# timweiland/GaussianMarkovRandomFields.jl

Hardware: AMD Instinct MI355X
Metric: factor+solve(64 RHS) throughput (higher is better)
Workload: dtype f64; 1 GPU; cfg2: 1000x1000-node jittered P1 mesh, 2-D Matern nu=1 (alpha=2), refactorize + 64-RHS solve + logdet per step, inputs resident in HBM; n=1000000, nnz_Q=18960020, nnz_L=178441686, nnz_L_stored=193749782, nrhs=64, parallelism=1 GPU, ordering=own geometric nested dissection

## Files before the change

### gaussianmarkovrandomfields.jl_amd/csrc/device.cpp

```cpp
#include "device.h"

#include <algorithm>
#include <atomic>
#include <chrono>
#include <cstdio>
#include <climits>
#include <cstdlib>
#include <cstring>
#include <exception>
#include <functional>
#include <stdexcept>
#include <thread>
#include <type_traits>

#include "kernels.h"

namespace gmrfx {

void hip_check(hipError_t e, const char *what) {
    if (e != hipSuccess) throw std::runtime_error(std::string("HIP error in ") + what + ": " + hipGetErrorString(e));
}
#define HC(x) hip_check((x), #x)

static constexpr size_t kPairSlackBytes = 16;
static constexpr size_t kChunkSlack = 16 * 320;
template <class T> T *Device::dalloc(size_t count) {
    void *p = nullptr;
    const size_t bytes = std::max<size_t>(count, 1) * sizeof(T) + kPairSlackBytes;
    HC(hipMalloc(&p, bytes));
    allocs_.push_back(p);
    bytes_total += (double)bytes;
    return (T *)p;
}

template <class T> static void regrow(DevBuf<T> &buf, size_t count, double *ledger) {
    DevBuf<T> fresh;
    fresh.alloc(count, ledger);
    if (buf) HC(hipDeviceSynchronize());
    buf = std::move(fresh);
}

Device::~Device() {
    if (stream) { (void)hipStreamSynchronize(stream); }
    for (void *p : allocs_) (void)hipFree(p);
}

void Device::set_external_stream(hipStream_t s, bool use, bool async) {
    HC(hipSetDevice(device));
    HC(hipStreamSynchronize(stream));
    stream = use ? s : own_stream_;
    async_phases_ = use && async;
}

void Device::init(const Symbolic &S, int dev) {
    int count = 0;
    hipError_t e = hipGetDeviceCount(&count);
    if (e != hipSuccess || count <= 0) throw std::runtime_error("no HIP device available (libgmrfx has no CPU fallback)");
    if (dev < 0) HC(hipGetDevice(&dev));
    if (dev >= count) throw std::runtime_error("HIP device ordinal out of range");
    device = dev;
    HC(hipSetDevice(device));
    {
        int lo = 0, hi = 0;
        HC(hipDeviceGetStreamPriorityRange(&lo, &hi));
        own_stream_.create(hipStreamNonBlocking, hi);
        stream = own_stream_;
        stream2.create(hipStreamNonBlocking, lo);
        stream3.create(hipStreamNonBlocking, hi);
    }
    env_ = read_env_knobs();
    inv_cap_ = env_.inv_cap;
    ev_fact_.create(hipEventDisableTiming);
    ev_inv_.create(hipEventDisableTiming);
    for (auto &ev : ev_) ev.create();
    for (auto &l : ev_lane_) for (auto &ev : l) ev.create();
    h_info_.alloc(2);
    h_info_[0] = INT_MAX;
    h_info_[1] = 0;
    ev_ready_.create(hipEventDisableTiming);
    ev_ready2_.create(hipEventDisableTiming);
    ev_done1_.create(hipEventDisableTiming);
    upload(S);
}

void Device::upload(const Symbolic &S) {
    S_ = &S;
    const DevicePlan P = build_device_plan(S, PlanOptions{env_.syrk_xcd});
    auto up = [&](const auto &host) {
        using T = typename std::decay_t<decltype(host)>::value_type;
        using D = std::conditional_t<std::is_same<T, i64>::value, long long, T>;
        static_assert(sizeof(D) == sizeof(T), "a device array holds the same bytes as its host vector");
        D *p = dalloc<D>(host.size());
        if (!host.empty()) HC(hipMemcpyAsync(p, host.data(), host.size() * sizeof(T), hipMemcpyHostToDevice, stream));
        return p;
    };
    levels_ = P.levels; swlevels_ = P.swlevels; sel_max_cols_ = P.sel_max_cols; sel_max_trail_ = P.sel_max_trail;
    inv_maxc_ = P.inv_maxc; inv_nact_ = P.inv_nact; inv_lvl_first_ = P.inv_lvl_first; inv_lvl_maxc_ = P.inv_lvl_maxc; inv_lvl_nact_ = P.inv_lvl_nact;
    fc_levelptr_ = P.fc_levelptr; fc_maxtrail_ = P.fc_maxtrail;
    std::copy_n(P.wave_first, kWaveClasses, wave_first_); std::copy_n(P.wave_count, kWaveClasses, wave_count_); std::copy_n(P.nsub_cls, 3, nsub_cls_);
    bottom_top_level_ = P.bottom_top_level; fused_gate_level_ = P.fused_gate_level; first_multiblock_level_ = P.first_multiblock_level;
    syrk_flops = P.syrk_flops; sum_trail_ = P.sum_trail; l_size_ = P.l_size; nq_ = P.nq; nswt_ = P.nswt; nswc_ = P.nswc;

    ds_.n = (int)S.n;
    ds_.nsuper = S.nsuper;
    ds_.sfirst = up(S.sfirst); ds_.rowptr = up(S.rowptr); ds_.rows = up(S.rows); ds_.rel = up(S.rel);
    ds_.panelptr = up(S.panelptr); ds_.ld = up(S.ld); ds_.cbptr = up(S.cbptr);
    d_zbptr_ = up(S.zbptr);
    d_selrec_ = up(P.selrec);
    ds_.childptr = up(S.childptr); ds_.children = up(S.children); ds_.sparent = up(S.sparent);
    ds_.qptr = up(S.qptr); ds_.qsrc = up(P.qsrc); ds_.qdst = up(P.qdst); ds_.qcol = up(P.qcol); ds_.qcolptr = up(P.qcolptr);
    d_nzp_ = dalloc<double>((size_t)std::max<long long>(nq_, 1));
    ev_nzp_.create(hipEventDisableTiming);
    ev_nzp0_.create(hipEventDisableTiming);
    ds_.wptr = up(S.wptr);
    ds_.edge = up(P.edge); ds_.etile = up(P.etile); ds_.erow = up(P.erow);
    ds_.diagoff = up(S.diagoff); ds_.perm = up(S.perm);
    d_iperm_ = up(S.iperm);
    if (S.shard_plan) {
        d_owncol_ = up(P.owncol);
        ds_.foreign_parent = up(P.foreign_parent);
        d_fchild_ = up(P.fchild);
    }
    ds_.lrow = up(S.lrow);
    d_sw_levellist_ = up(S.sw_levellist);
    if (nswc_ > 0) {
        d_swc_fwd_ = up(S.swc_fwd); d_swc_bwd_ = up(S.swc_bwd);
        d_swc_listf_ = up(P.swc_listf); d_swc_listb_ = up(P.swc_listb);
        d_dtile_ = dalloc<double>((size_t)nswc_ * 256);
    }
    d_swt_ = up(P.swt);
    d_wave_order_ = up(P.wave_order);
    d_levellist_ = up(S.levellist); d_levellist2_ = up(P.levellist2);
    d_sub_first_ = up(S.sub_first); d_sub_last_ = up(S.sub_last);
    d_sel_levellist_ = up(S.sel_levellist);
    d_frec_ = up(P.frec); d_sel_frec_ = up(P.sel_frec); d_frec2_ = up(P.frec2);
    d_invlist_ = up(P.invlist);
    for (const auto &off : P.inv_toff) d_inv_toff_.push_back(up(off));
    d_invT_ = dalloc<double>((size_t)std::max<long long>(P.inv_tsize, 1));
    if (!P.inv_lvl_list.empty()) d_inv_lvl_list_ = up(P.inv_lvl_list);
    for (const auto &off : P.inv_lvl_toff) d_inv_lvl_toff_.push_back(up(off));
    d_syrk_recs_ = up(P.syrk_recs); d_fwd_recs_ = up(P.fwd_recs); d_arec_ = up(P.arec);
    ev_syrk_.resize(2 * (size_t)S.nlevels);
    for (auto &e : ev_syrk_) e.create();

    static_assert(kPairSlackBytes >= sizeof(double), "pair loads read one element past the end");
    d_L_ = dalloc<double>((size_t)l_size_ + kChunkSlack);
    d_cb_ = dalloc<double>((size_t)S.cb_arena);
    d_nz_ = dalloc<double>((size_t)S.nnz_in);
    d_info_ = dalloc<int>(2);
    d_part_ = dalloc<double>(1024 + 8);
    HC(hipMemsetAsync(d_L_, 0, ((size_t)l_size_ + kChunkSlack) * sizeof(double) + kPairSlackBytes, stream));
    HC(hipStreamSynchronize(stream));
}

void Device::clone_from(const Device &o, const Symbolic &S) {
    init(S, o.device);
    inv_cap_ = o.inv_cap_;
    inv_cap_decided_ = o.inv_cap_decided_;
    ms_inv_decide = o.ms_inv_decide;
    if (o.factorized) {
        HC(hipMemcpyAsync(d_L_, o.d_L_, (size_t)l_size_ * sizeof(double), hipMemcpyDeviceToDevice, stream));
        HC(hipMemcpyAsync(d_info_, o.d_info_, sizeof(int), hipMemcpyDeviceToDevice, stream));
        HC(hipStreamSynchronize(stream));
        factorized = true;
        inverse_pending = true;
    }
}

static bool host_ptr_is_pinned(const void *p) {
    hipPointerAttribute_t a;
    if (hipPointerGetAttributes(&a, p) != hipSuccess) { (void)hipGetLastError(); return false; }
    return a.type == hipMemoryTypeHost || a.type == hipMemoryTypeDevice || a.type == hipMemoryTypeManaged;
}
static int host_io_threads() {
    static const int nt = [] {
        const unsigned hc = std::thread::hardware_concurrency();
        return (int)std::min<unsigned>(8, std::max<unsigned>(1, hc / 2));
    }();
    return nt;
}
static constexpr long long kIoSliceBytes = 16ll << 20;
static constexpr int kIoRing = 8;

static void parallel_memcpy(double *dst, const double *src, long long count) {
    const int T = (int)std::min<long long>(host_io_threads(), std::max<long long>(1, count >> 18));
    if (T <= 1) { std::memcpy(dst, src, (size_t)count * sizeof(double)); return; }
    std::vector<std::thread> th;
    const long long per = (count + T - 1) / T;
    for (int t = 1; t < T; t++) {
        const long long a = t * per, e = std::min(count, a + per);
        if (a < e) th.emplace_back([=] { std::memcpy(dst + a, src + a, (size_t)(e - a) * sizeof(double)); });
    }
    std::memcpy(dst, src, (size_t)std::min(per, count) * sizeof(double));
    for (auto &x : th) x.join();
}

HostIoPlan host_io_plan(long long n, long long nrhs, long long slice_bytes) {
    HostIoPlan p;
    const long long slice_doubles = std::max<long long>(1, slice_bytes / (long long)sizeof(double));
    n = std::max<long long>(n, 1);
    if (n <= slice_doubles) {
        p.cols_per = slice_doubles / n; p.ppc = 1; p.rows_per = n;
        p.slot_doubles = p.cols_per * n;
        p.nsl = (nrhs + p.cols_per - 1) / p.cols_per;
    } else {
        p.cols_per = 1; p.ppc = (n + slice_doubles - 1) / slice_doubles; p.rows_per = (n + p.ppc - 1) / p.ppc;
        p.slot_doubles = p.rows_per;
        p.nsl = nrhs * p.ppc;
    }
    p.reserve = std::min<long long>(p.nsl, kIoRing) * p.slot_doubles;
    return p;
}
HostIoPlan host_io_plan_dir(long long n, long long nrhs, int download) { return host_io_plan(n, nrhs, download ? kIoSliceBytes / 2 : kIoSliceBytes); }
static inline void host_io_slice(const HostIoPlan &p, long long k, long long n, long long nrhs, long long &j0, long long &nc, long long &r0, long long &nr) {
    if (p.ppc == 1) { j0 = k * p.cols_per; nc = std::min(p.cols_per, nrhs - j0); r0 = 0; nr = n; }
    else { j0 = k / p.ppc; nc = 1; r0 = (k % p.ppc) * p.rows_per; nr = std::max<long long>(0, std::min(p.rows_per, n - r0)); }
}

void Device::host_io_reserve(long long count) {
    if (!stream_io_) {
        stream_io_.create(hipStreamNonBlocking);
        ev_up_.create(hipEventDisableTiming);
        ev_x_.create(hipEventDisableTiming);
    }
    if (count <= h_stage_.cap()) return;
    if (h_stage_) HC(hipStreamSynchronize(stream_io_));
    h_stage_.alloc(count);
}

void Device::host_upload_values(const double *nzval) {
    const long long cnt = S_->nnz_in;
    if (host_ptr_is_pinned(nzval)) {
        HC(hipMemcpyAsync(d_nz_, nzval, (size_t)cnt * sizeof(double), hipMemcpyDefault, stream));
        return;
    }
    if (!h_nzstage_) h_nzstage_.alloc(cnt);
    HC(hipStreamSynchronize(stream));
    parallel_memcpy(h_nzstage_, nzval, cnt);
    HC(hipMemcpyAsync(d_nz_, h_nzstage_, (size_t)cnt * sizeof(double), hipMemcpyHostToDevice, stream));
}

void Device::host_upload(const double *B, long long ldb, long long nrhs, double *d_dst) {
    const long long n = S_->n;
    host_io_reserve(0);
    if (host_ptr_is_pinned(B)) {
        if (ldb == n) HC(hipMemcpyAsync(d_dst, B, (size_t)(n * nrhs) * sizeof(double), hipMemcpyDefault, stream_io_));
        else HC(hipMemcpy2DAsync(d_dst, n * sizeof(double), B, ldb * sizeof(double), n * sizeof(double), nrhs, hipMemcpyDefault, stream_io_));
        HC(hipEventRecord(ev_up_, stream_io_));
        return;
    }
    const HostIoPlan pl = host_io_plan(n, nrhs, kIoSliceBytes);
    const long long slot_doubles = pl.slot_doubles, nsl = pl.nsl;
// ... 21 lines not shown
                double *st = h_stage_ + slot * slot_doubles;
                for (long long j = 0; j < nc; j++)
                    std::memcpy(st + j * nr, B + (j0 + j) * ldb + r0, (size_t)nr * sizeof(double));
                if (nc * nr > 0) HC(hipMemcpyAsync(d_dst + j0 * n + r0, st, (size_t)(nc * nr) * sizeof(double), hipMemcpyHostToDevice, stream_io_));
                HC(hipEventRecord(ev_ring_[slot], stream_io_));
                posted[(size_t)k].store(1, std::memory_order_release);
            }
        } catch (...) {
            if (!failed.exchange(true)) err = std::current_exception();
        }
    };
    for (int t = 1; t < T; t++) th.emplace_back(work, t);
    work(0);
    for (auto &x : th) x.join();
    if (err) std::rethrow_exception(err);
    HC(hipEventRecord(ev_up_, stream_io_));
}

void Device::host_download(const double *d_src, long long nrhs, double *X, long long ldx, hipStream_t after) {
    const long long n = S_->n;
    host_io_reserve(0);
    HC(hipStreamSynchronize(after));
    if (host_ptr_is_pinned(X)) {
        if (ldx == n) HC(hipMemcpyAsync(X, d_src, (size_t)(n * nrhs) * sizeof(double), hipMemcpyDefault, stream_io_));
        else HC(hipMemcpy2DAsync(X, ldx * sizeof(double), d_src, n * sizeof(double), n * sizeof(double), nrhs, hipMemcpyDefault, stream_io_));
        HC(hipStreamSynchronize(stream_io_));
        return;
    }
    const HostIoPlan pl = host_io_plan(n, nrhs, kIoSliceBytes / 2);
    const long long slot_doubles = pl.slot_doubles, nsl = pl.nsl;
    host_io_reserve(pl.reserve);
    while ((int)ev_ring_.size() < kIoRing) { Event e; e.create(hipEventDisableTiming); ev_ring_.push_back(std::move(e)); }
    std::vector<std::atomic<int>> done((size_t)nsl);
    for (auto &a : done) a.store(0);
    const int T = (int)std::min<long long>(std::min<long long>(host_io_threads(), kIoRing), nsl);
    std::vector<std::thread> th;
    std::exception_ptr err;
    std::atomic<bool> failed{false};
    const int dev = device;
    auto work = [&](int t) {
        try {
            HC(hipSetDevice(dev));
            for (long long k = t; k < nsl && !failed.load(); k += T) {
                long long j0, nc, r0, nr;
                host_io_slice(pl, k, n, nrhs, j0, nc, r0, nr);
                const int slot = (int)(k % kIoRing);
                if ((slot + 1) * slot_doubles > h_stage_.cap() || nc * nr > slot_doubles) throw std::runtime_error("host_download: slice leaves the staging ring");
                if (k >= kIoRing)
                    while (!done[(size_t)(k - kIoRing)].load(std::memory_order_acquire)) { if (failed.load()) return; std::this_thread::yield(); }
                double *st = h_stage_ + slot * slot_doubles;
                if (nc * nr > 0) HC(hipMemcpyAsync(st, d_src + j0 * n + r0, (size_t)(nc * nr) * sizeof(double), hipMemcpyDeviceToHost, stream_io_));
                HC(hipEventRecord(ev_ring_[slot], stream_io_));
                HC(hipEventSynchronize(ev_ring_[slot]));
                for (long long j = 0; j < nc; j++)
                    std::memcpy(X + (j0 + j) * ldx + r0, st + j * nr, (size_t)nr * sizeof(double));
                done[(size_t)k].store(1, std::memory_order_release);
            }
        } catch (...) {
            if (!failed.exchange(true)) err = std::current_exception();
        }
    };
    for (int t = 1; t < T; t++) th.emplace_back(work, t);
    work(0);
    for (auto &x : th) x.join();
    if (err) std::rethrow_exception(err);
}

static const int kClsRows[4] = {48, 64, 96, 128};
static const int OBK = 4;
static const FrontArg kNoFront{0, 0, 0, 0, 0, 0, 0};

bool Device::factor_small_fronts(const LevelInfo &L) {
    const int nf = L.nbig();
    int ncls_used = 0, widest = -1;
    for (int k = 0; k < 4; k++) if (L.ncls[k] > 0) { ncls_used++; widest = k; }
    const bool split_small = L.nsmall > 0 && (nf > 0 || ncls_used > 1);
    if (split_small) {
        HC(hipEventRecord(ev_ready_, stream));
        HC(hipStreamWaitEvent(stream3, ev_ready_, 0));
    }
    for (int k = 0, off = 0; k < 4; off += L.ncls[k], k++) {
        hipStream_t st_small = !split_small ? stream : (nf > 0 || k != widest) ? stream3 : stream;
        launch_factor_small(st_small, ds_, d_levellist_ + L.first + off, L.ncls[k], kClsRows[k], nz_src_, d_L_, d_cb_, d_info_);
    }
    return split_small;
}

struct Device::PanelChain {
    hipStream_t st;
    const FrontView *views;
    int half;
    FrontArg f1;
    int of(int a) const { return half < 0 ? a : half == 0 ? (a + 1) / 2 : a / 2; }
    int count(const LevelInfo &L, int b) const { return of(L.wider_than(b * NB)); }
    const FrontArg &arg(int active) const { return active == 1 ? f1 : kNoFront; }
};

void Device::panel_block(const PanelChain &ch, const LevelInfo &L, int b) {
    const int n = ch.count(L, b), kb = b * NB;
    if (n <= 0) return;
    hipStream_t st = ch.st;
    const FrontView *hl = ch.views;
    if (b == 0 && n > 1) {
        const int cut[5] = {0, ch.of(L.wider[0]), ch.of(L.wider[1]), ch.of(L.wider[2]), n};
        const int wcls[4] = {64, 48, 32, 16};
        for (int q = 0; q < 4; q++)
            if (cut[q + 1] > cut[q])
                launch_potrf64(st, ds_, hl + cut[q], cut[q + 1] - cut[q], kb, d_L_, d_info_, kNoFront, std::min(wcls[q], L.max_cols));
    } else
        launch_potrf64(st, ds_, hl, n, kb, d_L_, d_info_, ch.arg(n), std::min(NB, L.max_cols - kb));
    {
        constexpr int narrow_min = 256;
        const int cut32 = b == 0 ? ch.of(L.wider[1]) : n;
        const int nnarrow = n - cut32;
        if (b == 0 && narrow_min > 0 && nnarrow >= narrow_min) {
            if (cut32 > 0) launch_trsm(st, ds_, hl, cut32, kb, 0, L.max_rows - kb - 1, d_L_, nullptr, nullptr, kNoFront);
            launch_trsm_narrow(st, hl + cut32, nnarrow, kb, L.max_rows - kb - 1, d_L_);
        } else
            launch_trsm(st, ds_, hl, n, kb, 0, L.max_rows - kb - 1, d_L_, nullptr, nullptr, ch.arg(n));
    }
    const int J1 = (b / OBK + 1) * OBK;
    const int nnext = ch.count(L, b + 1), nouter = ch.count(L, J1);
    if (b + 1 < J1 && nnext > 0)
        launch_gemm_nt(st, ds_, hl, nnext, kb, NB, kb + NB, J1 * NB, L.max_rows - kb - NB,
                       std::min(J1 * NB, L.max_cols) - kb - NB, d_L_, ch.arg(nnext));
    if (b + 1 == J1 && nouter > 0)
        launch_gemm_nt(st, ds_, hl, nouter, (J1 - OBK) * NB, OBK * NB, J1 * NB, INT_MAX,
                       L.max_rows - J1 * NB, L.max_cols - J1 * NB, d_L_, ch.arg(nouter));
}

bool Device::factor_panel_chains(const LevelInfo &L) {
    const int nf = L.nbig(), nblk = L.nblk(), base = L.first + L.nsmall;
    const bool two = nf >= 2 && nblk >= 4 && !sharded();
    if (two) {
        HC(hipEventRecord(ev_ready2_, stream));
        HC(hipStreamWaitEvent(stream3, ev_ready2_, 0));
    }
    auto front_at = [&](int pos) {
        if (pos >= nf) return kNoFront;
        const i32 s = S_->levellist[base + pos];
        return FrontArg{1, (int)s, S_->ncols(s), S_->nrows(s), (int)S_->ld[s], (int)S_->sfirst[s], (long long)S_->panelptr[s]};
    };
    const PanelChain ch[2] = {{stream, two ? d_frec2_ + base : d_frec_ + base, two ? 0 : -1, front_at(0)},
                              {stream3, d_frec2_ + base + (nf + 1) / 2, 1, front_at(1)}};
    for (int b = 0; b < nblk; b++)
        for (int h = 0; h < (two ? 2 : 1); h++) panel_block(ch[h], L, b);
    if (two) {
        HC(hipEventRecord(ev_done1_, stream3));
        HC(hipStreamWaitEvent(stream, ev_done1_, 0));
    }
    return two;
}

void Device::factor_contribution_blocks(const LevelInfo &L, int slot) {
    const int *list = d_levellist_ + L.first + L.nsmall;
    const int nf = L.nbig();
    HC(hipEventRecord(ev_syrk_[2 * slot], stream));
    const bool huge = env_.syrk_xcd && !sharded() && L.max_trail >= 4096 && L.max_cols >= 1024;
    if (env_.syrk_xcd) launch_syrk_cb_recs(stream, ds_, d_syrk_recs_ + L.syrk_off, L.syrk_split, L.syrk_per, d_L_, d_cb_, huge ? 1 : 0, L.max_cols >= env_.syrk_piped_min);
    else launch_syrk_cb(stream, ds_, list, nf, L.max_trail, d_L_, d_cb_);
    if (huge) launch_syrk_big(stream, ds_, list, nf, L.max_trail, d_L_, d_cb_);
    HC(hipEventRecord(ev_syrk_[2 * slot + 1], stream));
}

void Device::factor_levels(int lo, int hi, bool record_level_events) {
    if (lo == 0) {
        const int big = INT_MAX;
        HC(hipMemcpyAsync(d_info_, &big, sizeof(int), hipMemcpyHostToDevice, stream));
        syrk_launches = 0;
        for (int k = 0, off = 0; k < 3; off += nsub_cls_[k], k++)
            launch_subtree(stream, ds_, 0, d_sub_first_ + off, d_sub_last_ + off, nsub_cls_[k], kClsRows[k], nz_src_, d_L_, d_cb_,
                           d_info_, nullptr, nullptr, 0, 0);
    }
    if (lo == 0) {
        HC(hipEventRecord(ev_nzp0_, stream));
        HC(hipStreamWaitEvent(stream3, ev_nzp0_, 0));
        launch_gather_values(stream3, nz_src_, ds_.qsrc, d_nzp_, nq_);
        HC(hipEventRecord(ev_nzp_, stream3));
        nzp_pending_ = true;
    }
    int nsy = (int)syrk_launches;
    for (int lev = lo; lev < hi; lev++) {
        const LevelInfo &L = levels_[lev];
        if (env_.level_mark) { launch_level_mark(stream, 3, lev); level_event(stream, 0, lev); }
        const int nf = L.nbig();
        const bool split_small = factor_small_fronts(L);
        if (nf > 0 && nzp_pending_) { HC(hipStreamWaitEvent(stream, ev_nzp_, 0)); nzp_pending_ = false; }
        launch_assemble(stream, ds_, d_levellist_ + L.first + L.nsmall, d_arec_ + L.first + L.nsmall, d_nzp_, nf, L.max_cols, L.max_rows, nz_src_, d_L_, d_cb_);
        const bool two = factor_panel_chains(L);
        if (nf > 0 && L.max_trail > 0) factor_contribution_blocks(L, nsy++);
        if (split_small && !two) {
            HC(hipEventRecord(ev_done1_, stream3));
            HC(hipStreamWaitEvent(stream, ev_done1_, 0));
        }
        if (record_level_events) HC(hipEventRecord(ev_flevel_[lev], stream));
    }
    syrk_launches = nsy;
    if (lo == 0 && nzp_pending_) { HC(hipStreamWaitEvent(stream, ev_nzp_, 0)); nzp_pending_ = false; }
    if (env_.level_mark) level_event(stream, 0, hi);
}

void Device::start_inverse_async() {
    if (!inverse_pending) return;
    if (!fact_event_valid_) HC(hipEventRecord(ev_fact_, stream));
    fact_event_valid_ = false;
    HC(hipStreamWaitEvent(stream2, ev_fact_, 0));
    invert_diag_blocks(stream2, NB, inv_cap_);
    HC(hipEventRecord(ev_inv_, stream2));
    inverse_pending = false;
    inverse_full_ = inv_maxc_ <= inv_cap_;
}
void Device::wait_inverse(hipStream_t st) { HC(hipStreamWaitEvent(st, ev_inv_, 0)); }

void Device::decide_inverse_cap() {
    if (inv_cap_decided_ || sharded() || *h_info_ != INT_MAX) return;
    inv_cap_decided_ = true;
    const int nf = inv_nact_.empty() ? 0 : inv_nact_[0];
    if (nf <= 0 || inv_cap_ <= NB) return;
    const auto t0 = std::chrono::steady_clock::now();
    const size_t cnt = (size_t)nf * (size_t)((inv_maxc_ + 255) / 256);
    if (!d_pivgrowth_) d_pivgrowth_ = dalloc<double>(cnt);
    launch_pivot_growth(stream, ds_, d_invlist_, nf, inv_maxc_, d_L_, d_pivgrowth_);
    std::vector<double> r(cnt);
    HC(hipMemcpyAsync(r.data(), d_pivgrowth_, cnt * sizeof(double), hipMemcpyDeviceToHost, stream));
    HC(hipStreamSynchronize(stream));
    ms_inv_decide = std::chrono::duration<double, std::milli>(std::chrono::steady_clock::now() - t0).count();
    for (double v : r)
        if (!(v <= kInvGrowthMax)) {
            inv_cap_ = NB;
            break;
        }
}

void Device::invert_diag_blocks(hipStream_t stream, int b_from, int b_to) {
    int stage = 0;
    for (int B = NB; B < std::min(inv_maxc_, b_to); B *= 2, stage++) {
        if (B < b_from) continue;
        const int na = inv_nact_[stage];
        if (na <= 0) break;
        launch_inv_stage(stream, ds_, d_invlist_, na, B, inv_maxc_, 1, d_L_, d_invT_, d_inv_toff_[stage]);
        launch_inv_stage(stream, ds_, d_invlist_, na, B, inv_maxc_, 2, d_L_, d_invT_, d_inv_toff_[stage]);
    }
}

void Device::invert_level(hipStream_t st, int lev) {
    if (inv_lvl_first_.empty() || inv_lvl_maxc_[lev] <= NB) return;
    int stage = 0;
    for (int B = NB; B < std::min(inv_lvl_maxc_[lev], inv_cap_); B *= 2, stage++) {
        const int na = inv_lvl_nact_[lev][stage];
        if (na <= 0) break;
        launch_inv_stage(st, ds_, d_inv_lvl_list_ + inv_lvl_first_[lev], na, B, inv_lvl_maxc_[lev], 1, d_L_, d_invT_, d_inv_lvl_toff_[stage] + inv_lvl_first_[lev]);
        launch_inv_stage(st, ds_, d_inv_lvl_list_ + inv_lvl_first_[lev], na, B, inv_lvl_maxc_[lev], 2, d_L_, d_invT_, d_inv_lvl_toff_[stage] + inv_lvl_first_[lev]);
    }
}

void Device::refactorize_solve(const double *nzval, bool nz_on_device, const double *B, long long ldb, long long nrhs, double *X, long long ldx_out,
                               bool b_on_device) {
    HC(hipSetDevice(device));
    if (sharded()) throw std::invalid_argument("sharded handle: use the phase entry points (gmrfx/shard.py)");
    if (nrhs <= 0 || stream != own_stream_ || !inv_cap_decided_) {
        refactorize(nzval, nz_on_device);
        if (nrhs > 0) solve(B, ldb, nrhs, X, ldx_out, b_on_device, 0);
        return;
    }
    const long long n = S_->n;
    const int nl = (int)levels_.size();
    const double *src = nzval;
    if (!nz_on_device) {
        host_upload_values(nzval);
        src = d_nz_;
    }
    ensure_rhs_capacity(nrhs);
    const double *dB = B;
    double *dXo = X;
    long long ldin = ldb, ldout = ldx_out;
    if (!b_on_device) {
        ensure_io(n * nrhs);
        dB = d_io_; dXo = d_io_; ldin = n; ldout = n;
    }
    while ((int)ev_flevel_.size() < nl + 1) { Event e; e.create(hipEventDisableTiming); ev_flevel_.push_back(std::move(e)); }
    if (!b_on_device) {
        host_upload(B, ldb, nrhs, d_io_);
        HC(hipStreamWaitEvent(stream, ev_up_, 0));
    }
    begin_factor(src);
    HC(hipEventRecord(ev_ready_, stream));
    factor_levels(0, nl, true);
    enqueue_factor_tail();
    const int PW = pass_width(nrhs);
    const int nr = (int)std::min<long long>(PW, nrhs), ldx = nr;
    const Event *ev = ev_lane_[0];
    const SweepLane ln0 = lane(0), side{stream2, ln0.X, ln0.X2, ln0.W};
    HC(hipStreamWaitEvent(side.st, ev_ready_, 0));
    if (!b_on_device) HC(hipStreamWaitEvent(side.st, ev_up_, 0));
    HC(hipEventRecord(ev[0], side.st));
    launch_permute(side.st, d_iperm_, (int)n, const_cast<double *>(dB), ldin, side.X, nr, ldx, 0);
    HC(hipEventRecord(ev[1], side.st));
    forward(side, nr, ldx, 0, nl, true);
    HC(hipEventRecord(ev_inv_, side.st));
    HC(hipEventRecord(ev[2], side.st));
    inverse_pending = false;
    inverse_full_ = inv_maxc_ <= inv_cap_;
    enqueue_logdet(stream2, false);
    HC(hipStreamWaitEvent(stream, ev[2], 0));
    backward(ln0, nr, ldx, true, nl, 0);
    HC(hipEventRecord(ev[3], stream));
    launch_permute(stream, d_iperm_, (int)n, dXo, ldout, ln0.X, nr, ldx, 1);
    HC(hipEventRecord(ev[4], stream));
    for (long long j0 = PW; j0 < nrhs; j0 += PW)
        sweep_pass(ln0, nullptr, dB + j0 * ldin, ldin, dXo + j0 * ldout, ldout, (int)std::min<long long>(PW, nrhs - j0), 0, nullptr);
    HC(hipEventRecord(ev_lane_[1][0], stream));
    if (!b_on_device) host_download(d_io_, nrhs, X, ldx_out, stream);
    HC(hipStreamSynchronize(stream));
    finish_factor();
    float a = 0, b = 0, c = 0, d = 0, tail = 0;
    HC(hipEventElapsedTime(&a, ev[0], ev[1]));
    HC(hipEventElapsedTime(&b, ev_[1], ev[2]));
    HC(hipEventElapsedTime(&c, ev[2], ev[3]));
    HC(hipEventElapsedTime(&d, ev[3], ev[4]));
    HC(hipEventElapsedTime(&tail, ev_[1], ev_lane_[1][0]));
    ms_perm = a + d; ms_fwd = std::max(b, 0.0f); ms_bwd = b >= 0 ? c : c + b;
    ms_solve = tail;
    last_nrhs = nrhs;
}

void Device::begin_factor(const double *d_src) {
    nz_src_ = d_src;
    nz_held_ = (d_src == d_nz_);
    factor_serial_++;
    HC(hipEventRecord(ev_[0], stream));
}
void Device::enqueue_factor_tail() {
    HC(hipEventRecord(ev_[1], stream));
    HC(hipEventRecord(ev_fact_, stream));
    fact_event_valid_ = true;
    HC(hipMemcpyAsync(h_info_, d_info_, sizeof(int), hipMemcpyDeviceToHost, stream));
}
void Device::finish_factor() {
    info_cached_ = true;
    HC(hipGetLastError());
    decide_inverse_cap();
    float ms = 0;
    HC(hipEventElapsedTime(&ms, ev_[0], ev_[1]));
    ms_factor = ms;
    syrk_times_pending_ = true;
    factorized = true;
    selinv_valid = false;
}

void Device::refactorize(const double *nzval, bool on_device) {
    HC(hipSetDevice(device));
    if (sharded()) throw std::invalid_argument("sharded handle: use gmrfx_refactorize_phase (two phases with an exchange in between)");
    const double *src = nzval;
    if (!on_device) {
        HC(hipMemcpyAsync(d_nz_, nzval, (size_t)S_->nnz_in * sizeof(double), hipMemcpyHostToDevice, stream));
        src = d_nz_;
    }
    begin_factor(src);
    factor_levels(0, (int)levels_.size(), false);
    enqueue_factor_tail();
    inverse_pending = true;
    HC(hipStreamSynchronize(stream));
    finish_factor();
}

void Device::refactorize_phase(const double *d_nzval, int phase) {
    HC(hipSetDevice(device));
    if (!sharded()) throw std::invalid_argument("gmrfx_refactorize_phase needs a sharded handle (shard_world > 1, or shard_min_top > 0)");
    const int nl = (int)levels_.size();
    const int split = std::min<int>(S_->shard_level, nl);
    info_cached_ = false;
    fact_event_valid_ = false;
    factor_serial_++;
    HC(hipEventRecord(ev_[0], stream));
    if (phase == 0) {
        nz_src_ = d_nzval;
        nz_held_ = false;
        factorized = false;
        factor_levels(0, split, false);
    } else {
        const int lev = split + phase - 1;
        if (lev >= nl) throw std::invalid_argument("refactorize phase beyond the last level");
        factor_levels(lev, lev + 1, false);
    }
    HC(hipEventRecord(ev_[1], stream));
    if (!async_phases_) {
        HC(hipStreamSynchronize(stream));
        HC(hipGetLastError());
        float ms = 0;
        HC(hipEventElapsedTime(&ms, ev_[0], ev_[1]));
        ms_factor = phase == 0 ? ms : ms_factor + ms;
    }
    selinv_begun_ = false;
    if (split + phase >= nl) { factorized = true; selinv_valid = false; inverse_pending = true; }
}

void Device::dist_front_phase(const double *d_nzval, int front, int what, int block) {
    HC(hipSetDevice(device));
    if (front < 0 || front >= S_->nsuper || !S_->is_dist(front)) throw std::invalid_argument("not a distributed front of this handle");
    const i32 R = front;
    const int g = S_->group_size(R), me = S_->group_pos(R, S_->shard_rank);
    if (me < 0) return;
    const int c = S_->ncols(R), r = S_->nrows(R);
    const int nob = S_->panel_blocks(R);
    const FrontArg fa{1, (int)R, c, r, (int)S_->ld[R], (int)S_->sfirst[R], (long long)S_->panelptr[R]};
    const bool compact = S_->compact_here(R);
    const long long ldR = S_->ld[R], ppl = S_->panelptr[R];
    auto blk_pp = [&](int b) -> long long { return compact ? ppl - 256LL * (b - b / g) * ldR : ppl; };
    auto a_pp = [&](int b) -> long long {
        if (!compact) return kNoPpa;
        return b % g == me ? blk_pp(b) : ppl + S_->compact_window(R, b & 1) - 256LL * b * ldR;
    };
    if (!d_dist_list_) {
        d_dist_list_ = dalloc<int>(S_->dist_fronts.size());
        HC(hipMemcpyAsync(d_dist_list_, S_->dist_fronts.data(), S_->dist_fronts.size() * sizeof(int), hipMemcpyHostToDevice, stream));
    }
    const int *list = d_dist_list_ + S_->dist_index[R];
    if (what == 0) {
        if (!d_nzval) throw std::invalid_argument("d_nzval is null");
        launch_assemble_cyclic(stream, ds_, list, c, d_nzval, d_L_, d_cb_, g, me, compact);
    } else if (what == 1) {
        if (block < 0 || block >= nob) throw std::invalid_argument("distributed front: block out of range");
        if (block % g != me) return;
        FrontArg fb = fa;
        fb.pp = blk_pp(block);
        const int b0 = block * OBK, b1 = std::min(b0 + OBK, (c + NB - 1) / NB);
        for (int b = b0; b < b1; b++) {
            const int kb = b * NB;
            launch_potrf64(stream, ds_, nullptr, 1, kb, d_L_, d_info_, fb);
            launch_trsm(stream, ds_, nullptr, 1, kb, 0, r - kb - 1, d_L_, nullptr, nullptr, fb);
            if (b + 1 < b1)
                launch_gemm_nt(stream, ds_, nullptr, 1, kb, NB, kb + NB, b1 * NB, r - kb - NB, std::min(b1 * NB, c) - kb - NB, d_L_, fb);
        }
    } else if (what == 2 || what == 4 || what == 5) {
        if (block < 0 || block >= nob) throw std::invalid_argument("distributed front: block out of range");
        const int k0 = block * 256, K = std::min(256, c - k0);
        const int jlo = what == 5 ? block + 2 : block + 1, jhi = what == 4 ? std::min(block + 2, nob) : nob;
        for (int j = jlo; j < jhi; j++) {
            if (j % g != me) continue;
            const int c0 = j * 256;
            FrontArg fj = fa;
            fj.pp = blk_pp(j);
            fj.ppa = a_pp(block);
            launch_gemm_nt(stream, ds_, nullptr, 1, k0, K, c0, c0 + 256, r - c0, std::min(256, c - c0), d_L_, fj);
        }
    } else if (what == 3) {
        if (r > c) launch_syrk_cb_cyclic(stream, ds_, list, r - c, d_L_, d_cb_, g, me, nob);
    } else throw std::invalid_argument("distributed front phase must be 0 (assemble), 1 (factor block), 2 / 4 / 5 (apply block: all / next / rest) or 3 (contribution block)");
    if (!async_phases_) HC(hipStreamSynchronize(stream));
    HC(hipGetLastError());
}

void Device::set_prior(const double *prior_nzval, const long long *map, long long cnt) {
    HC(hipSetDevice(device));
    const long long nnz = S_->nnz_in;
    for (long long k = 0; k < cnt; k++)
        if (map[k] < 0 || map[k] >= nnz) throw std::invalid_argument("Hessian index map points outside the stored pattern of Q");
    if (!d_prior_) d_prior_ = dalloc<double>((size_t)nnz);
    HC(hipMemcpyAsync(d_prior_, prior_nzval, (size_t)nnz * sizeof(double), hipMemcpyHostToDevice, stream));
    if (cnt > hmap_cap_ || !d_hmap_ || !d_h_) {
        hmap_cap_ = 0;
        regrow(d_hmap_, (size_t)cnt, &bytes_total);
        regrow(d_h_, (size_t)cnt, &bytes_total);
        hmap_cap_ = cnt;
    }
    hmap_cnt_ = cnt;
    if (cnt > 0) HC(hipMemcpyAsync(d_hmap_, map, (size_t)cnt * sizeof(long long), hipMemcpyHostToDevice, stream));
    HC(hipStreamSynchronize(stream));
}
void Device::newton_values(const double *h, bool on_device) {
    if (!d_prior_) throw std::invalid_argument("gmrfx_set_prior has not been called");
    const double *dh = h;
    if (!on_device && hmap_cnt_ > 0) {
        HC(hipMemcpyAsync(d_h_, h, (size_t)hmap_cnt_ * sizeof(double), hipMemcpyHostToDevice, stream));
        dh = d_h_;
    }
    launch_newton_update(stream, d_prior_, d_nz_, S_->nnz_in, d_hmap_, dh, hmap_cnt_);
}
void Device::refactorize_update(const double *h, bool on_device) {
    HC(hipSetDevice(device));
    newton_values(h, on_device);
    refactorize(d_nz_, true);
}

void Device::refactorize_update_solve(const double *h, bool h_on_device, const double *B, long long ldb, long long nrhs, double *X, long long ldx,
                                      bool b_on_device) {
    HC(hipSetDevice(device));
    newton_values(h, h_on_device);
    refactorize_solve(d_nz_, true, B, ldb, nrhs, X, ldx, b_on_device);
}

double Device::syrk_ms() {
    if (syrk_times_pending_) {
        HC(hipSetDevice(device));
        ms_syrk = 0;
        for (long long k = 0; k < syrk_launches; k++) {
            float t = 0;
            HC(hipEventElapsedTime(&t, ev_syrk_[2 * k], ev_syrk_[2 * k + 1]));
            ms_syrk += t;
        }
        syrk_times_pending_ = false;
    }
    return ms_syrk;
}

long long Device::fail_col() {
    int v = INT_MAX;
    if (info_cached_) v = *h_info_;
    else {
        HC(hipStreamSynchronize(stream));
        HC(hipMemcpy(&v, d_info_, sizeof(int), hipMemcpyDeviceToHost));
    }
    return v == INT_MAX ? -1 : v;
}

void Device::ensure_rhs_capacity(long long nrhs) {
    const long long chunk = std::min<long long>(nrhs, 64);
    if (chunk > rhs_cap_) {
        d_X_ = dalloc<double>((size_t)S_->n * 64);
        d_X2_ = dalloc<double>((size_t)S_->n * 64);
        d_W_ = dalloc<double>((size_t)std::max<long long>(sum_trail_, 1) * 64);
        rhs_cap_ = 64;
    }
    if (pass_width(nrhs) < nrhs && !d_Xb_ && !sharded()) {
        d_Xb_ = dalloc<double>((size_t)S_->n * 64);
        d_X2b_ = dalloc<double>((size_t)S_->n * 64);
        d_Wb_ = dalloc<double>((size_t)std::max<long long>(sum_trail_, 1) * 64);
    }
}

void Device::ensure_io(long long need) {
    if (need <= io_cap_) return;
    const long long cap = std::max(need, 2 * io_cap_);
    regrow(d_io_, (size_t)cap, &bytes_total);
    io_cap_ = cap;
}

void Device::sweep_tasks(const SweepLane &ln, int phase, int nr, int ldx, bool follows_factor) {
    if (nr > env_.wave_max_nr) {
        constexpr int pad_kb = 16;
        const size_t extra = (follows_factor && phase == 1) ? (size_t)pad_kb * 1024 : 0;
        ensure_dtile(ln.st);
        launch_sweep_chunks(ln.st, ds_, phase, d_swt_, nswt_, d_swc_fwd_, d_swc_bwd_, d_swc_listf_, d_swc_listb_, d_dtile_, d_L_, ln.X,
                            phase == 1 ? ln.W : nullptr, nr, ldx, extra);
        return;
    }
    ensure_rdiag(ln.st);
    if (nr <= 4) {
        launch_wave_tasks(ln.st, ds_, phase, d_swt_, d_wave_order_ + nswt_, nswt_, kWaveRows[kWaveClasses - 1], d_L_, d_rdiag_, d_rdiag_ + S_->n, ln.X,
                          ln.W, nr, ldx);
        return;
    }
    for (int k = kWaveClasses - 1; k >= 0; k--)
        launch_wave_tasks(ln.st, ds_, phase, d_swt_, d_wave_order_ + wave_first_[k], wave_count_[k], kWaveRows[k], d_L_, d_rdiag_,
                          d_rdiag_ + S_->n, ln.X, ln.W, nr, ldx);
}

void Device::ensure_rdiag(hipStream_t st) {
    if (env_.wave_max_nr <= 0 || nswt_ <= 0) return;
    if (!d_rdiag_) { d_rdiag_ = dalloc<double>((size_t)S_->n + 2); rdiag_for_ = 0; }
    if (rdiag_for_ == factor_serial_) return;
    launch_rdiag(st, d_L_, ds_.diagoff, (int)S_->n, d_rdiag_);
    HC(hipMemsetAsync(d_rdiag_ + S_->n, 0, 2 * sizeof(double), st));
    rdiag_for_ = factor_serial_;
}

void Device::ensure_dtile(hipStream_t st) {
    if (nswc_ <= 0 || dtile_for_ == factor_serial_) return;
    launch_pack_diag(st, d_swc_bwd_, nswc_, d_L_, d_dtile_);
    dtile_for_ = factor_serial_;
}

SweepKnobs Device::sweep_knobs() const {
    return SweepKnobs{inv_cap_, env_.fwd_front_min, env_.bwd_front_min, env_.syrk_xcd, kNarrowPassMax, kNarrowPassMaxBwd,
                      kFrontMaxCols, kWaveSplitCols, kWaveSplitRows};
}

void Device::forward(const SweepLane &ln, int nr, int ldx, int lo, int hi, bool follows_factor) {
    const SweepKnobs knobs = sweep_knobs();
    if (env_.level_mark && lo == 0) { launch_level_mark(ln.st, 1, -1); level_event(ln.st, 1, 0); }
    if (follows_factor) {
        HC(hipStreamWaitEvent(ln.st, ev_flevel_[fused_gate_level_], 0));
        if (nr <= env_.wave_max_nr && nswt_ > 0) rdiag_for_ = 0;
        dtile_for_ = 0;
    }
    if (lo == 0) sweep_tasks(ln, 1, nr, ldx, follows_factor);
    if (lo == 0)
        for (int k = 0, off = 0; k < 3; off += nsub_cls_[k], k++)
            launch_subtree(ln.st, ds_, 1, d_sub_first_ + off, d_sub_last_ + off, nsub_cls_[k], kClsRows[k], nullptr, d_L_, nullptr,
                           nullptr, ln.X, ln.W, nr, ldx);
    for (int lev = lo; lev < hi; lev++) {
        const LevelInfo &L = swlevels_[lev];
        if (env_.level_mark) { launch_level_mark(ln.st, 1, lev); level_event(ln.st, 1, 1 + lev); }
        if (follows_factor) {
            if (lev > fused_gate_level_) HC(hipStreamWaitEvent(ln.st, ev_flevel_[lev], 0));
            invert_level(ln.st, lev);
        } else if (lev == std::max(lo, first_multiblock_level_)) wait_inverse(ln.st);
        for (int k = 0, off = 0; k < 4; off += L.ncls[k], k++)
            launch_fwd_small(ln.st, ds_, d_sw_levellist_ + L.first + off, L.ncls[k], kClsRows[k], d_L_, ln.X, ln.W, nr, ldx);
        const int *list = d_sw_levellist_ + L.first + L.nsmall;
        const FwdLevelPlan p = plan_forward_level(L, nr, knobs);
        if (p.ntail > 0) {
            launch_fwd_front(ln.st, ds_, list + p.nf, p.ntail, d_L_, ln.X, ln.X2, ln.W, nr, ldx);
            if (p.nf == 0) continue;
        }
        launch_fwd_assemble(ln.st, ds_, list, p.nf, L.max_cols, ln.X, ln.W, nr, ldx);
        for (int j = 0; j < p.nbk; j++) {
            launch_xmul(ln.st, ds_, list, p.xmul_fronts(j), L.max_cols, 0, d_L_, ln.X, ln.X2, nr, ldx, j, inv_cap_);
            if (j + 1 < p.nbk) launch_fwd_own_update(ln.st, ds_, list, p.own_fronts(j), L.max_cols, d_L_, ln.X2, ln.X, nr, ldx, j, inv_cap_);
        }
        if (p.wave) launch_fwd_update_wave(ln.st, ds_, d_fwd_recs_ + L.fwd_off, L.fwd_split, L.fwd_per, d_L_, ln.X2, ln.W, nr, ldx, p.cmin, p.wave_split_k);
        if (p.update == FwdLevelPlan::kRecords)
            launch_fwd_update_recs(ln.st, ds_, d_fwd_recs_ + L.fwd_off, L.fwd_split, L.fwd_per, d_L_, ln.X2, ln.W, nr, ldx, p.cmin);
        else if (p.update == FwdLevelPlan::kGrid)
            launch_fwd_update(ln.st, ds_, list, p.nf, L.max_trail, d_L_, ln.X2, ln.W, nr, ldx, p.cmin);
    }
    if (env_.level_mark) level_event(ln.st, 1, 1 + hi);
}

void Device::backward(const SweepLane &ln, int nr, int ldx, bool y_in_x2, int hi, int lo) {
    const SweepKnobs knobs = sweep_knobs();
    double *const Xt = y_in_x2 ? ln.X2 : ln.X, *const Xx = y_in_x2 ? ln.X : ln.X2;
    wait_inverse(ln.st);
    for (int l = hi - 1; l >= lo; l--) {
        const LevelInfo &L = swlevels_[l];
        if (env_.level_mark) { launch_level_mark(ln.st, 2, l); level_event(ln.st, 2, (int)levels_.size() - 1 - l); }
        const int *list = d_sw_levellist_ + L.first + L.nsmall;
        for (int k = 0, off = 0; k < 4; off += L.ncls[k], k++)
            launch_bwd_small(ln.st, ds_, d_sw_levellist_ + L.first + off, L.ncls[k], kClsRows[k], d_L_, ln.X, nr, ldx);
        const BwdLevelPlan p = plan_backward_level(L, nr, knobs);
        if (p.ntail > 0) {
            launch_bwd_front(ln.st, ds_, list + p.nf, p.ntail, d_L_, ln.X, Xt, ln.X, nr, ldx);
            if (p.nf == 0) continue;
        }
        if (p.wave) launch_bwd_wave(ln.st, ds_, list, p.nf, L.max_cols, d_L_, ln.X, Xt, nr, ldx, p.mmin, p.wave_split_k);
        if (p.gemm) launch_bwd_gemm(ln.st, ds_, list, p.nf, L.max_cols, d_L_, ln.X, Xt, nr, ldx, -1, 1 << 30, p.mmin);
        for (int j = p.nbk - 1; j >= 0; j--) {
            if (j + 1 < p.nbk) launch_bwd_gemm(ln.st, ds_, list, p.own_fronts(j), L.max_cols, d_L_, ln.X, Xt, nr, ldx, j, inv_cap_);
            launch_xmul(ln.st, ds_, list, p.xmul_fronts(j), L.max_cols, 1, d_L_, Xt, Xx, nr, ldx, j, inv_cap_);
            if (!y_in_x2) launch_copy_own(ln.st, ds_, list, p.xmul_fronts(j), L.max_cols, ln.X2, ln.X, nr, ldx, j, inv_cap_);
        }
    }
    if (env_.level_mark && lo == 0) { launch_level_mark(ln.st, 2, -1); level_event(ln.st, 2, (int)levels_.size()); }
    if (lo == 0)
        for (int k = 0, off = 0; k < 3; off += nsub_cls_[k], k++)
            launch_subtree(ln.st, ds_, 2, d_sub_first_ + off, d_sub_last_ + off, nsub_cls_[k], kClsRows[k], nullptr, d_L_, nullptr,
                           nullptr, ln.X, nullptr, nr, ldx);
    if (lo == 0) sweep_tasks(ln, 2, nr, ldx, false);
    if (env_.level_mark && lo == 0) level_event(ln.st, 2, (int)levels_.size() + 1);
}

void Device::level_event(hipStream_t st, int phase, int slot) {
    auto &v = ev_level_[phase];
    while ((int)v.size() <= slot) { Event e; e.create(); v.push_back(std::move(e)); }
    HC(hipEventRecord(v[slot], st));
    level_slots_[phase] = std::max(level_slots_[phase], slot + 1);
}
int Device::level_times(int phase, double *out, int cap) {
    HC(hipSetDevice(device));
    const int nl = (int)levels_.size();
    if (!env_.level_mark || phase < 0 || phase > 2 || level_slots_[phase] < (phase == 0 ? nl + 1 : nl + 2)) return 0;
    HC(hipDeviceSynchronize());
    auto &v = ev_level_[phase];
    auto dt = [&](int a, int b) { float ms = 0; HC(hipEventElapsedTime(&ms, v[a], v[b])); return (double)ms; };
    for (int k = 0; k <= nl && k < cap; k++) {
        if (phase == 0) out[k] = k == 0 ? 0.0 : dt(k - 1, k);
        else if (phase == 1) out[k] = dt(k, k + 1);
        else out[k] = k == 0 ? dt(nl, nl + 1) : dt(nl - k, nl - k + 1);
    }
    return std::min(nl + 1, cap);
}

void Device::solve_phase(const double *d_B, long long ldb, long long nrhs, double *d_Xout, long long ldx_out, int phase) {
    HC(hipSetDevice(device));
    if (!sharded()) throw std::invalid_argument("gmrfx_solve_phase needs a sharded handle (shard_world > 1, or shard_min_top > 0)");
    if (nrhs <= 0 || nrhs > 64) throw std::invalid_argument("sharded solves take 1..64 right-hand sides per call");
    const int nr = (int)nrhs, ldx = nr, nl = (int)levels_.size();
    const int split = std::min<int>(S_->shard_level, nl);
    const long long n = S_->n;
    HC(hipEventRecord(ev_[0], stream));
    if (phase == 0 || phase == 10) ensure_rhs_capacity(nrhs);
    const SweepLane ln = lane(0);
    if (phase == 0) {
        start_inverse_async();
        ensure_rdiag(stream);
        ensure_dtile(stream);
        launch_permute(stream, d_iperm_, (int)n, const_cast<double *>(d_B), ldb, ln.X, nr, ldx, 0);
        forward(ln, nr, ldx, 0, split, false);
    } else if (phase >= 100 && phase < 100 + (nl - split)) {
        const int lev = split + phase - 100;
        forward(ln, nr, ldx, lev, lev + 1, false);
    } else if (phase >= 200 && phase < 200 + (nl - split)) {
        const int lev = split + phase - 200;
        backward(ln, nr, ldx, true, lev + 1, lev);
    } else if (phase == 2) {
        backward(ln, nr, ldx, true, split, 0);
    } else if (phase == 10) {
        start_inverse_async();
        ensure_rdiag(stream);
        ensure_dtile(stream);
        launch_permute(stream, nullptr, (int)n, const_cast<double *>(d_B), ldb, ln.X, nr, ldx, 0);
    } else if (phase >= 300 && phase < 300 + (nl - split)) {
        const int lev = split + phase - 300;
        backward(ln, nr, ldx, false, lev + 1, lev);
    } else if (phase == 12) {
        backward(ln, nr, ldx, false, split, 0);
    } else if (phase == 3) {
        launch_permute(stream, d_iperm_, (int)n, d_Xout, ldx_out, ln.X, nr, ldx, 1);
    } else throw std::invalid_argument("solve phase must be 0, 2, 3, 10, 12, 100 + k, 200 + k or 300 + k (k = top level)");
    HC(hipEventRecord(ev_[1], stream));
    if (!async_phases_) {
        HC(hipStreamSynchronize(stream));
        HC(hipGetLastError());
        float ms = 0;
        HC(hipEventElapsedTime(&ms, ev_[0], ev_[1]));
        ms_solve = (phase == 0 || phase == 10) ? ms : ms_solve + ms;
    }
    last_nrhs = nrhs;
}

void Device::sweep_pass(const SweepLane &ln, const Event *ev, const double *dB, long long ldin, double *dXo, long long ldout, int nr, int mode,
                        const MemberLayout *ml) {
    const int n = (int)S_->n, ldx = nr, nl = (int)levels_.size();
    auto mark = [&](int k) { if (ev) HC(hipEventRecord(ev[k], ln.st)); };
    mark(0);
    if (ml) launch_batch_permute(ln.st, mode == 0 ? d_iperm_ : nullptr, n, (int)ml->n_member, const_cast<double *>(dB), ldin, ml->sin, ln.X, nr, ldx, 0);
    else launch_permute(ln.st, mode == 0 ? d_iperm_ : nullptr, n, const_cast<double *>(dB), ldin, ln.X, nr, ldx, 0);
    mark(1);
    if (mode == 0) forward(ln, nr, ldx, 0, nl, false);
    mark(2);
    backward(ln, nr, ldx, mode == 0, nl, 0);
    mark(3);
    if (ml) launch_batch_permute(ln.st, d_iperm_, n, (int)ml->n_member, dXo, ldout, ml->sout, ln.X, nr, ldx, 1);
    else launch_permute(ln.st, d_iperm_, n, dXo, ldout, ln.X, nr, ldx, 1);
    mark(4);
}

void Device::solve(const double *B, long long ldb, long long nrhs, double *X, long long ldx_out, bool on_device, int mode,
                   const MemberLayout *ml) {
    HC(hipSetDevice(device));
    if (sharded()) throw std::invalid_argument("sharded handle: use gmrfx_solve_phase (phases with exchanges in between, gmrfx/shard.py)");
    if (ml && !on_device) throw std::invalid_argument("member-strided solves take device arrays");
    if (nrhs <= 0) return;
    const long long n = S_->n;
    ensure_rhs_capacity(nrhs);
    start_inverse_async();
    ensure_rdiag(stream);
    ensure_dtile(stream);
    const double *dB = B;
    double *dXo = X;
    long long ldin = ldb, ldout = ldx_out;
    if (!on_device) {
        const long long need = n * nrhs;
        ensure_io(need);
        if (ldb == n) HC(hipMemcpyAsync(d_io_, B, (size_t)need * sizeof(double), hipMemcpyHostToDevice, stream));
        else HC(hipMemcpy2DAsync(d_io_, n * sizeof(double), B, ldb * sizeof(double), n * sizeof(double), nrhs, hipMemcpyHostToDevice, stream));
        dB = d_io_; dXo = d_io_; ldin = n; ldout = n;
    }
    double t_perm = 0, t_fwd = 0, t_bwd = 0;
    const int PW = pass_width(nrhs);
    const bool two = nrhs > PW && d_Xb_ != nullptr;
    const SweepLane lanes[2] = {lane(0), lane(1)};
    if (two) {
        HC(hipEventRecord(ev_ready_, stream));
        HC(hipStreamWaitEvent(stream3, ev_ready_, 0));
    }
    bool busy[2] = {false, false};
    auto collect = [&](int ln) {
        if (!busy[ln]) return;
        HC(hipEventSynchronize(ev_lane_[ln][4]));
        float a, b, c, d;
        HC(hipEventElapsedTime(&a, ev_lane_[ln][0], ev_lane_[ln][1]));
        HC(hipEventElapsedTime(&b, ev_lane_[ln][1], ev_lane_[ln][2]));
        HC(hipEventElapsedTime(&c, ev_lane_[ln][2], ev_lane_[ln][3]));
        HC(hipEventElapsedTime(&d, ev_lane_[ln][3], ev_lane_[ln][4]));
        t_perm += a + d; t_fwd += b; t_bwd += c;
        busy[ln] = false;
    };
    HC(hipEventRecord(ev_[0], stream));
    int pass = 0;
    for (long long j0 = 0; j0 < nrhs; j0 += PW, pass++) {
        const int ln = two ? (pass & 1) : 0;
        collect(ln);
        sweep_pass(lanes[ln], ev_lane_[ln], dB + j0 * ldin, ldin, dXo + j0 * ldout, ldout, (int)std::min<long long>(PW, nrhs - j0), mode, ml);
        busy[ln] = true;
    }
    if (two) {
        HC(hipEventRecord(ev_done1_, stream3));
        HC(hipStreamWaitEvent(stream, ev_done1_, 0));
    }
    HC(hipEventRecord(ev_[1], stream));
    collect(0);
    collect(1);
    HC(hipStreamSynchronize(stream));
    float wall = 0;
    HC(hipEventElapsedTime(&wall, ev_[0], ev_[1]));
    HC(hipGetLastError());
    if (!on_device) {
        const long long need = n * nrhs;
        if (ldx_out == n) HC(hipMemcpyAsync(X, d_io_, (size_t)need * sizeof(double), hipMemcpyDeviceToHost, stream));
        else HC(hipMemcpy2DAsync(X, ldx_out * sizeof(double), d_io_, n * sizeof(double), n * sizeof(double), nrhs, hipMemcpyDeviceToHost, stream));
        HC(hipStreamSynchronize(stream));
    }
    ms_perm = t_perm; ms_fwd = t_fwd; ms_bwd = t_bwd;
    if (mode == 0) ms_solve = two ? wall : t_perm + t_fwd + t_bwd; else ms_bsolve = two ? wall : t_perm + t_bwd;
    last_nrhs = nrhs;
}

void Device::enqueue_logdet(hipStream_t st, bool timed) {
    if (!h_logdet_) {
        h_logdet_.alloc(1);
        ev_logdet_.create(hipEventDisableTiming);
    }
    const int nparts = (int)std::min<long long>(1024, std::max<long long>(1, (S_->n + 255) / 256));
    if (timed) HC(hipEventRecord(ev_[0], st));
    launch_logdet(st, d_L_, ds_.diagoff, d_owncol_, (int)S_->n, d_part_, nparts, d_part_ + 1024);
    if (timed) HC(hipEventRecord(ev_[1], st));
    HC(hipMemcpyAsync(h_logdet_, d_part_ + 1024, sizeof(double), hipMemcpyDeviceToHost, st));
    HC(hipEventRecord(ev_logdet_, st));
    logdet_for_ = factor_serial_;
}
double Device::logdet() {
    HC(hipSetDevice(device));
    if (logdet_for_ != factor_serial_ || !h_logdet_) {
        enqueue_logdet(stream, true);
        HC(hipEventSynchronize(ev_logdet_));
        float ms; HC(hipEventElapsedTime(&ms, ev_[0], ev_[1])); ms_logdet = ms;
    } else HC(hipEventSynchronize(ev_logdet_));
    return *h_logdet_;
}

void Device::prepare_quadform(long long nvec) {
    const Symbolic &S = *S_;
    if (!d_in_colptr_) {
        d_in_colptr_ = dalloc<long long>(S.in_colptr.size());
        d_in_row_ = dalloc<int>(std::max<size_t>(S.in_row.size(), 1));
        HC(hipMemcpyAsync(d_in_colptr_, S.in_colptr.data(), S.in_colptr.size() * sizeof(long long), hipMemcpyHostToDevice, stream));
        HC(hipMemcpyAsync(d_in_row_, S.in_row.data(), S.in_row.size() * sizeof(int), hipMemcpyHostToDevice, stream));
        HC(hipStreamSynchronize(stream));
    }
    const int nblk = quadform_blocks((int)S.n);
    if (nvec > qf_cap_) {
        const long long cap = std::max<long long>(nvec, 2 * qf_cap_);
        qf_cap_ = 0;
        regrow(d_qf_part_, (size_t)cap * nblk, &bytes_total);
        regrow(d_qf_out_, (size_t)cap, &bytes_total);
        qf_cap_ = cap;
    }
}

void Device::refactorize_logpdf(const double *d_nz, const double *d_X, long long ldx, long long nvec, const double *d_mu, double *quad_out,
                                double *logdet_out) {
    HC(hipSetDevice(device));
    const Symbolic &S = *S_;
    if (sharded()) throw std::invalid_argument("sharded handle: use the phase entry points (gmrfx/shard.py)");
    if (nvec < 0 || nvec > 65535) throw std::invalid_argument("refactorize_logpdf: 0..65535 vectors per call");
    if (nvec > 0 && ldx < S.n) throw std::invalid_argument("refactorize_logpdf: ldx < n");
    if (stream != own_stream_) throw std::invalid_argument("refactorize_logpdf: not on a caller's stream");
    if (nvec > 0) {
        prepare_quadform(nvec);
        h_qf_.grow(nvec, 16);
        HC(hipEventRecord(ev_ready_, stream));
        HC(hipStreamWaitEvent(stream2, ev_ready_, 0));
        launch_quadform(stream2, (int)S.n, d_in_colptr_, d_in_row_, d_nz, S.in_use, d_X, ldx, (int)nvec, d_mu, d_qf_part_, d_qf_out_);
        HC(hipMemcpyAsync(h_qf_, d_qf_out_, (size_t)nvec * sizeof(double), hipMemcpyDeviceToHost, stream2));
        ev_qf_.ensure(hipEventDisableTiming);
        HC(hipEventRecord(ev_qf_, stream2));
    }
    begin_factor(d_nz);
    factor_levels(0, (int)levels_.size(), false);
    enqueue_factor_tail();
    inverse_pending = true;
    enqueue_logdet(stream, false);
    if (nvec > 0) HC(hipStreamWaitEvent(stream, ev_qf_, 0));
    HC(hipStreamSynchronize(stream));
    finish_factor();
    for (long long k = 0; k < nvec; k++) quad_out[k] = h_qf_[k];
    if (logdet_out) *logdet_out = *h_logdet_;
}

void Device::quadform(const double *d_nz, const double *d_X, long long ldx, long long nvec, const double *d_mu, double *out_host) {
    HC(hipSetDevice(device));
    const Symbolic &S = *S_;
    if (nvec <= 0) return;
    if (nvec > 65535) throw std::invalid_argument("quadform: at most 65535 vectors per call");
    if (ldx < S.n) throw std::invalid_argument("quadform: ldx < n");
    if (!d_nz) {
        if (!nz_held_) throw std::invalid_argument("quadform: the handle does not hold Q's values (last refactorisation read a caller device buffer): pass them");
        d_nz = d_nz_;
    }
    prepare_quadform(nvec);
    HC(hipEventRecord(ev_[0], stream));
    launch_quadform(stream, (int)S.n, d_in_colptr_, d_in_row_, d_nz, S.in_use, d_X, ldx, (int)nvec, d_mu, d_qf_part_, d_qf_out_);
    HC(hipEventRecord(ev_[1], stream));
    HC(hipMemcpyAsync(out_host, d_qf_out_, (size_t)nvec * sizeof(double), hipMemcpyDeviceToHost, stream));
    HC(hipStreamSynchronize(stream));
    float ms; HC(hipEventElapsedTime(&ms, ev_[0], ev_[1])); ms_quadform = ms;
}

void Device::selinv_begin() {
    const Symbolic &S = *S_;
    start_inverse_async();
    wait_inverse(stream);
    if (!inverse_full_) {
        invert_diag_blocks(stream, inv_cap_, 1 << 30);
        inverse_full_ = true;
    }
    if (!d_Z_) d_Z_ = dalloc<double>((size_t)l_size_);
    if (!d_yoff_) {
        std::vector<long long> yoff(S.nsuper, 0);
        long long mx = 0;
        for (i32 l = 0; l < S.nlevels; l++) {
            long long off = 0;
            const i64 lf = S.sel_levelptr[l], cnt = S.sel_levelptr[l + 1] - lf;
            for (i64 k = 0; k < cnt; k++) {
                i32 s = S.sel_levellist[lf + k];
                yoff[s] = off;
                off += k < S.sel_level_nsmall[l] ? (long long)S.nrows(s) * NB : 2LL * (S.nrows(s) - S.ncols(s)) * S.ncols(s);
            }
            mx = std::max(mx, off);
        }
        if (mx > tmp_cap_) { regrow(d_tmp_, (size_t)mx, &bytes_total); tmp_cap_ = mx; }
        d_yoff_ = dalloc<long long>(std::max<size_t>(yoff.size(), 1));
        HC(hipMemcpyAsync(d_yoff_, yoff.data(), yoff.size() * sizeof(long long), hipMemcpyHostToDevice, stream));
        HC(hipStreamSynchronize(stream));
    }
    HC(hipMemsetAsync(d_Z_, 0, (size_t)l_size_ * sizeof(double) + kPairSlackBytes, stream));
}

void Device::selinv_levels(int hi, int lo) {
    const Symbolic &S = *S_;
    DevSym dsz = ds_;
    dsz.cbptr = d_zbptr_;
    for (int l = hi - 1; l >= lo; l--) {
        const int sfirst = (int)S.sel_levelptr[l], scount = (int)(S.sel_levelptr[l + 1] - S.sel_levelptr[l]);
        const int snsmall = S.sel_level_nsmall[l];
        const int *list = d_sel_levellist_ + sfirst + snsmall;
        const int nf = scount - snsmall;
        if (env_.level_mark) launch_level_mark(stream, 4, l);
        launch_sel_gather(stream, d_selrec_, dsz, list, nf, sel_max_trail_[l], d_Z_, d_cb_);
        for (int phase = 0; phase < 3; phase++)
            launch_sel_dense(stream, dsz, list, nf, phase, sel_max_cols_[l], sel_max_trail_[l], d_L_, d_Z_, d_cb_, d_tmp_,
                             d_tmp_, d_yoff_);
        if (snsmall > 0) {
            const int *sl = d_sel_levellist_ + sfirst;
            launch_sel_gather(stream, d_selrec_, dsz, sl, snsmall, 128, d_Z_, d_cb_);
            launch_trsm(stream, dsz, d_sel_frec_ + sfirst, snsmall, 0, 1, 128, d_L_, d_tmp_, d_yoff_, FrontArg{0, 0, 0, 0, 0, 0, 0});
            launch_sel_symm(stream, dsz, sl, snsmall, 0, 128, d_Z_, d_cb_, d_tmp_, d_yoff_);
            launch_sel_diag(stream, dsz, sl, snsmall, 0, d_L_, d_Z_, d_tmp_, d_yoff_);
        }
    }
}

void Device::selinv_compute() {
    HC(hipSetDevice(device));
    if (selinv_valid) return;
    if (sharded()) throw std::invalid_argument("sharded handle: the selected inversion runs in phases with exchanges in between (gmrfx_selinv_phase, gmrfx/shard.py)");
    selinv_begin();
    HC(hipEventRecord(ev_[0], stream));
    selinv_levels((int)levels_.size(), 0);
    HC(hipEventRecord(ev_[1], stream));
    HC(hipStreamSynchronize(stream));
    HC(hipGetLastError());
    float ms; HC(hipEventElapsedTime(&ms, ev_[0], ev_[1])); ms_selinv = ms;
    selinv_valid = true;
}

void Device::selinv_phase(int what, int hi, int lo) {
    HC(hipSetDevice(device));
    if (!sharded()) throw std::invalid_argument("gmrfx_selinv_phase needs a sharded handle (shard_world > 1, or shard_min_top > 0)");
    const int nl = (int)levels_.size();
    if (what != 0 && !selinv_begun_)
        throw std::invalid_argument("selinv phase 1, 2 or 3 before phase 0 (begin) since the last refactorisation");
    if (what == 0) {
        if (!factorized) throw std::invalid_argument("selinv phase 0 before the factorisation has finished");
        selinv_valid = false;
        selinv_begin();
        selinv_begun_ = true;
        ms_selinv = 0;
    } else if (what == 1) {
        if (hi < 0 || hi >= nl) throw std::invalid_argument("selinv phase: level out of range");
        DevSym dsz = ds_;
        dsz.cbptr = d_zbptr_;
        const int a = fc_levelptr_[hi], b = fc_levelptr_[hi + 1];
        launch_sel_gather(stream, d_selrec_, dsz, d_fchild_ + a, b - a, fc_maxtrail_[hi], d_Z_, d_cb_);
    } else if (what == 2) {
        if (lo < 0 || hi > nl || lo > hi) throw std::invalid_argument("selinv phase: level range out of bounds");
        HC(hipEventRecord(ev_[0], stream));
        selinv_levels(hi, lo);
        HC(hipEventRecord(ev_[1], stream));
        if (!async_phases_) {
            HC(hipStreamSynchronize(stream));
            float ms; HC(hipEventElapsedTime(&ms, ev_[0], ev_[1])); ms_selinv += ms;
        }
    } else if (what == 3) {
        selinv_valid = true;
    } else throw std::invalid_argument("selinv phase must be 0 (begin), 1 (gather for other ranks), 2 (own levels) or 3 (end)");
    if (!async_phases_) HC(hipStreamSynchronize(stream));
    HC(hipGetLastError());
}

void Device::selinv_diag(double *out_host) {
    HC(hipSetDevice(device));
    const long long n = S_->n;
    if (n > io_cap_) { regrow(d_io_, (size_t)n, &bytes_total); io_cap_ = n; }
    launch_gather_diag(stream, d_Z_, ds_.diagoff, ds_.perm, (int)n, d_io_);
    HC(hipMemcpyAsync(out_host, d_io_, (size_t)n * sizeof(double), hipMemcpyDeviceToHost, stream));
    HC(hipStreamSynchronize(stream));
}

void Device::gather_z(const long long *offsets_host, long long cnt, double *out_host) {
    HC(hipSetDevice(device));
    if (cnt <= 0) return;
    DevBuf<long long> d_off;
    DevBuf<double> d_out;
    d_off.alloc((size_t)cnt);
    d_out.alloc((size_t)cnt);
    HC(hipMemcpyAsync(d_off, offsets_host, (size_t)cnt * sizeof(long long), hipMemcpyHostToDevice, stream));
    launch_gather(stream, d_Z_, d_off, cnt, d_out);
    HC(hipMemcpyAsync(out_host, d_out, (size_t)cnt * sizeof(double), hipMemcpyDeviceToHost, stream));
    HC(hipStreamSynchronize(stream));
}

// ... 18 lines not shown
}

long long Device::rowdiag_plan_create(const long long *segptr_host, long long nseg, const long long *off_host, const int *p_host,
                                      const int *q_host, long long nvals) {
    HC(hipSetDevice(device));
    if (nseg > 0x7fffffffLL) throw std::invalid_argument("too many rows");
    RowDiagPlan P;
    P.nseg = nseg; P.cnt = nseg > 0 ? segptr_host[nseg] : 0; P.nvals = nvals;
    P.seg.alloc((size_t)nseg + 1);
    P.off.alloc((size_t)P.cnt);
    P.p.alloc((size_t)P.cnt);
    P.q.alloc((size_t)P.cnt);
    P.vals.alloc((size_t)nvals);
    P.out.alloc((size_t)nseg);
    HC(hipMemcpyAsync(P.seg, segptr_host, (size_t)(nseg + 1) * sizeof(long long), hipMemcpyHostToDevice, stream));
    HC(hipMemcpyAsync(P.off, off_host, (size_t)P.cnt * sizeof(long long), hipMemcpyHostToDevice, stream));
    HC(hipMemcpyAsync(P.p, p_host, (size_t)P.cnt * sizeof(int), hipMemcpyHostToDevice, stream));
    HC(hipMemcpyAsync(P.q, q_host, (size_t)P.cnt * sizeof(int), hipMemcpyHostToDevice, stream));
    HC(hipStreamSynchronize(stream));
    for (size_t k = 0; k < rd_plans_.size(); k++)
        if (!rd_plans_[k].seg) { rd_plans_[k] = std::move(P); return (long long)k; }
    rd_plans_.push_back(std::move(P));
    return (long long)rd_plans_.size() - 1;
}

void Device::rowdiag_plan_apply(long long id, const double *values_host, double *out_host) {
    HC(hipSetDevice(device));
    if (id < 0 || id >= (long long)rd_plans_.size() || !rd_plans_[id].seg) throw std::invalid_argument("unknown row-diag plan");
    const RowDiagPlan &P = rd_plans_[id];
    if (P.nseg <= 0) return;
    HC(hipMemcpyAsync(P.vals, values_host, (size_t)P.nvals * sizeof(double), hipMemcpyHostToDevice, stream));
    launch_seg_wsum_pairs(stream, d_Z_, P.seg, P.nseg, P.off, P.p, P.q, P.vals, P.out);
    HC(hipMemcpyAsync(out_host, P.out, (size_t)P.nseg * sizeof(double), hipMemcpyDeviceToHost, stream));
    HC(hipStreamSynchronize(stream));
}

void Device::rowdiag_plan_free(long long id) {
    if (id < 0 || id >= (long long)rd_plans_.size() || !rd_plans_[id].seg) return;
    rd_plans_[id] = RowDiagPlan{};
}

void Device::dense_apply(const double *d_D, const double *d_T, double *d_R, long long n1, long long n2) {
    HC(hipSetDevice(device));
    launch_dense_apply(stream, d_D, d_T, d_R, (int)n1, n2);
    HC(hipGetLastError());
    HC(hipStreamSynchronize(stream));
}
void Device::transpose(const double *d_src, double *d_dst, long long rows, long long cols) {
    HC(hipSetDevice(device));
    launch_transpose(stream, d_src, d_dst, rows, cols);
    HC(hipGetLastError());
    HC(hipStreamSynchronize(stream));
}

void Device::copy_factor(double *out_host) {
    HC(hipSetDevice(device));
    HC(hipMemcpy(out_host, d_L_, (size_t)l_size_ * sizeof(double), hipMemcpyDeviceToHost));
}

void Device::set_batch(int nbatch, long long n_member, long long nnz_member) {
    HC(hipSetDevice(device));
    const Symbolic &S = *S_;
    if (nbatch < 1 || n_member * nbatch != S.n || nnz_member * nbatch != S.nnz_in) throw std::invalid_argument("set_batch: sizes do not match the forest");
    nbatch_ = nbatch; nmember_ = n_member; nnz_member_ = nnz_member;
    d_bpsum_ = dalloc<double>((size_t)nbatch * batch_diag_parts((int)n_member));
    d_bpbad_ = dalloc<int>((size_t)nbatch * batch_diag_parts((int)n_member));
    d_bdiag_ = dalloc<double>(2 * (size_t)nbatch);
    h_bdiag_.alloc(2 * (long long)nbatch);
    ev_bdiag_.create(hipEventDisableTiming);
    d_bin_colptr_ = dalloc<long long>((size_t)n_member + 1);
    d_bin_row_ = dalloc<int>((size_t)std::max<long long>(nnz_member, 1));
    HC(hipMemcpyAsync(d_bin_colptr_, S.in_colptr.data(), ((size_t)n_member + 1) * sizeof(long long), hipMemcpyHostToDevice, stream));
    if (nnz_member > 0) HC(hipMemcpyAsync(d_bin_row_, S.in_row.data(), (size_t)nnz_member * sizeof(int), hipMemcpyHostToDevice, stream));
    HC(hipStreamSynchronize(stream));
}

void Device::enqueue_batch_diag(hipStream_t st) {
    double *ld = d_bdiag_;
    long long *info = reinterpret_cast<long long *>(d_bdiag_ + nbatch_);
    launch_batch_diag(st, d_L_, ds_.diagoff, (int)nmember_, nbatch_, d_bpsum_, d_bpbad_, ld, info);
    HC(hipMemcpyAsync(h_bdiag_, d_bdiag_, 2 * (size_t)nbatch_ * sizeof(double), hipMemcpyDeviceToHost, st));
    HC(hipEventRecord(ev_bdiag_, st));
    bdiag_for_ = factor_serial_;
}

void Device::batch_diag(double *logdet_out, long long *info_out) {
    HC(hipSetDevice(device));
    if (!h_bdiag_) throw std::invalid_argument("not a batched handle");
    if (bdiag_for_ != factor_serial_) enqueue_batch_diag(stream);
    HC(hipEventSynchronize(ev_bdiag_));
    HC(hipGetLastError());
    read_batch_diag(logdet_out, info_out);
}
void Device::read_batch_diag(double *logdet_out, long long *info_out) const {
    const long long *hi = reinterpret_cast<const long long *>(h_bdiag_ + nbatch_);
    for (int k = 0; k < nbatch_; k++) {
        if (logdet_out) logdet_out[k] = h_bdiag_[k];
        if (info_out) info_out[k] = hi[k];
    }
}

void Device::prepare_batch_quadform(long long npairs) {
    const long long nblk = batch_quadform_blocks((int)nmember_);
    if (npairs > bqf_cap_) {
        const long long cap = std::max<long long>(npairs, 2 * bqf_cap_);
        bqf_cap_ = 0;
        regrow(d_bqf_part_, (size_t)(cap * nblk), &bytes_total);
        regrow(d_bqf_out_, (size_t)cap, &bytes_total);
        bqf_cap_ = cap;
    }
    h_bqf_.grow(npairs, 64);
}

void Device::enqueue_batch_quadform(hipStream_t st, const double *d_nz, const double *d_X, long long ldx, long long sx, long long nvec,
                                    const double *d_mu) {
    launch_batch_quadform(st, (int)nmember_, d_bin_colptr_, d_bin_row_, d_nz, nnz_member_, S_->in_use, d_X, ldx, sx, (int)nvec, nbatch_, d_mu,
                          d_bqf_part_, d_bqf_out_);
    HC(hipMemcpyAsync(h_bqf_, d_bqf_out_, (size_t)(nvec * nbatch_) * sizeof(double), hipMemcpyDeviceToHost, st));
}

void Device::batch_quadform(const double *d_nz, const double *d_X, long long ldx, long long sx, long long nvec, const double *d_mu,
                            double *quad_out) {
    HC(hipSetDevice(device));
    if (!h_bdiag_) throw std::invalid_argument("not a batched handle");
    if (nvec <= 0) return;
    if (!d_nz) {
        if (!nz_held_) throw std::invalid_argument("batch_quadform: the handle does not hold Q's values (last refactorisation read a caller device buffer): pass them");
        d_nz = d_nz_;
    }
    prepare_batch_quadform(nvec * nbatch_);
    HC(hipEventRecord(ev_[0], stream));
    enqueue_batch_quadform(stream, d_nz, d_X, ldx, sx, nvec, d_mu);
    HC(hipEventRecord(ev_[1], stream));
    HC(hipStreamSynchronize(stream));
    HC(hipGetLastError());
    float ms; HC(hipEventElapsedTime(&ms, ev_[0], ev_[1])); ms_quadform = ms;
    for (long long k = 0; k < nvec * nbatch_; k++) quad_out[k] = h_bqf_[k];
}

void Device::batch_refactorize_logpdf(const double *d_nz, const double *d_X, long long ldx, long long sx, long long nvec, const double *d_mu,
                                      double *quad_out, double *logdet_out, long long *info_out) {
    HC(hipSetDevice(device));
    if (!h_bdiag_) throw std::invalid_argument("not a batched handle");
    if (stream != own_stream_) throw std::invalid_argument("batch_refactorize_logpdf: not on a caller's stream");
    if (nvec > 0) {
        prepare_batch_quadform(nvec * nbatch_);
        HC(hipEventRecord(ev_ready_, stream));
        HC(hipStreamWaitEvent(stream2, ev_ready_, 0));
        enqueue_batch_quadform(stream2, d_nz, d_X, ldx, sx, nvec, d_mu);
        ev_qf_.ensure(hipEventDisableTiming);
        HC(hipEventRecord(ev_qf_, stream2));
    }
    begin_factor(d_nz);
    factor_levels(0, (int)levels_.size(), false);
    enqueue_factor_tail();
    inverse_pending = true;
    enqueue_batch_diag(stream);
    if (nvec > 0) HC(hipStreamWaitEvent(stream, ev_qf_, 0));
    HC(hipStreamSynchronize(stream));
    finish_factor();
    for (long long k = 0; k < nvec * nbatch_; k++) quad_out[k] = h_bqf_[k];
    read_batch_diag(logdet_out, info_out);
}

}
```

### gaussianmarkovrandomfields.jl_amd/csrc/device.h

```cpp
#pragma once
#include <hip/hip_runtime.h>

#include <functional>
#include <string>
#include <vector>

#include "device_plan.h"
#include "rbmc_plan.h"
#include "resource.h"

namespace gmrfx {

struct DevSym {
    int n, nsuper;
    const int *sfirst;
    const long long *rowptr;
    const int *rows;
    const int *rel;
    const long long *panelptr;
    const int *ld;
    const long long *cbptr;
    const long long *childptr;
    const int *children;
    const int *sparent;
    const long long *qptr;
    const int *qsrc;
    const int *qdst;
    const int *qcol;
    const int *qcolptr;
    const int *erow;
    const long long *wptr;
    const long long *diagoff;
    const int *perm;
    const EdgeRec *edge;
    const int *etile;
    const int *lrow;
    const unsigned char *foreign_parent;
};

struct ConHost {
    int m = 0;
    std::vector<long long> rowptr;
    std::vector<int> col;
    std::vector<double> val, e;
    double logdet_AAt = 0;
};

constexpr long long kNoPpa = (long long)0x8000000000000000ull;
struct FrontArg { int on, s, c, r, ld, first; long long pp; long long ppa = kNoPpa; };
struct SweepLane { hipStream_t st; double *X, *X2, *W; };
constexpr size_t kTableMinBytes = 8;
class Device {
public:
    Device() = default;
    ~Device();
    Device(const Device &) = delete;
    Device &operator=(const Device &) = delete;

    void init(const Symbolic &S, int device);
    void clone_from(const Device &o, const Symbolic &S);

    void refactorize(const double *nzval, bool on_device);
    void refactorize_solve(const double *nzval, bool nz_on_device, const double *B, long long ldb, long long nrhs, double *X, long long ldx,
                           bool b_on_device);
    void refactorize_logpdf(const double *d_nz, const double *d_X, long long ldx, long long nvec, const double *d_mu, double *quad_out,
                            double *logdet_out);
    void refactorize_update_solve(const double *h, bool h_on_device, const double *B, long long ldb, long long nrhs, double *X, long long ldx,
                                  bool b_on_device);
    void set_prior(const double *prior_nzval, const long long *map, long long cnt);
    void refactorize_update(const double *h, bool on_device);
    void refactorize_phase(const double *d_nzval, int phase);
    void solve_phase(const double *d_B, long long ldb, long long nrhs, double *d_X, long long ldx, int phase);
    double *rhs_x() { return d_X_; }
    double *rhs_w() { return d_W_; }
    void ensure_rhs(long long nrhs) { ensure_rhs_capacity(nrhs); }
    static int pass_width(long long) { return 64; }
    double *cb_arena() { return d_cb_; }
    double *factor_panels() { return d_L_; }
    bool sharded() const { return S_ && S_->shard_plan; }
    struct MemberLayout { long long n_member, sin, sout; };
    void solve(const double *B, long long ldb, long long nrhs, double *X, long long ldx, bool on_device, int mode,
               const MemberLayout *ml = nullptr);
    void set_batch(int nbatch, long long n_member, long long nnz_member);
    bool batched() const { return (bool)h_bdiag_; }
    void batch_diag(double *logdet_out, long long *info_out);
    void batch_quadform(const double *d_nz, const double *d_X, long long ldx, long long sx, long long nvec, const double *d_mu, double *quad_out);
    void batch_refactorize_logpdf(const double *d_nz, const double *d_X, long long ldx, long long sx, long long nvec, const double *d_mu,
                                  double *quad_out, double *logdet_out, long long *info_out);
    double logdet();
    void quadform(const double *d_nz, const double *d_X, long long ldx, long long nvec, const double *d_mu, double *out_host);
    void selinv_compute();
    void selinv_phase(int what, int hi, int lo);
    void selinv_diag(double *out_host);
    void gather_z(const long long *offsets_host, long long cnt, double *out_host);
    void weighted_z_sums(const long long *segptr_host, long long nseg, const long long *off_host, const double *w_host, double *out_host);
    long long rowdiag_plan_create(const long long *segptr_host, long long nseg, const long long *off_host, const int *p_host,
                                  const int *q_host, long long nvals);
    void rowdiag_plan_apply(long long id, const double *values_host, double *out_host);
    void rowdiag_plan_free(long long id);
    void copy_factor(double *out_host);
    void dense_apply(const double *d_D, const double *d_T, double *d_R, long long n1, long long n2);
    void transpose(const double *d_src, double *d_dst, long long rows, long long cols);
    long long fail_col();
    void con_set(const ConHost &c);
    int con_m() const { return con_.m; }
    bool con_prepare();
    double con_logdet_w() const { return con_.logdet_w; }
    double con_ms() const { return con_.ms; }
    void con_get(double *At_host, long long ld, double *W_host);
    void con_correct(double *d_X, long long ldx, long long nvec, const double *d_mu);
    double ms_con_correct = 0;
    void con_residual(double *out_host);
    const std::vector<double> &con_linv() const { return con_.h_linv; }
    void con_var(double *out_host);
    void bcon_set(const ConHost &c);
    int bcon_m() const { return bcon_.m; }
    bool bcon_prepare();
    const std::vector<double> &bcon_logdet_w() const { return bcon_.h_logdet; }
    const std::vector<long long> &bcon_cinfo() const { return bcon_.h_cinfo; }
    double bcon_ms() const { return bcon_.ms; }
    void bcon_get(int member, double *At_host, long long ld, double *W_host);
    void bcon_correct(double *d_X, long long ldx, long long sx, long long nvec, const double *d_mu);
    void bcon_quad(const double *d_x, double *quad_host);
    void bcon_var(double *out_host);

    void rbmc_var(const RbmcSym &sym, const RbmcPlan *plan, const double *d_nz, const double *Z, long long ldz, bool z_on_device, long long k,
                  double *out, bool out_on_device);
    double ms_rbmc = 0, ms_rbmc_bsolve = 0;

    bool factorized = false, selinv_valid = false;
    bool inverse_pending = false;
    double ms_factor = 0, ms_solve = 0, ms_fwd = 0, ms_bwd = 0, ms_perm = 0, ms_bsolve = 0, ms_logdet = 0, ms_selinv = 0;
    long long last_nrhs = 0;
    double ms_quadform = 0;
    double ms_inv_decide = 0;
    int inv_cap() const { return inv_cap_; }
    bool syrk_times_pending_ = false;
    double syrk_ms();
    double ms_syrk = 0, syrk_flops = 0;
    long long syrk_launches = 0;
    double bytes_total = 0;
    int device = 0;
    hipStream_t stream = nullptr;
    Stream own_stream_;
    bool async_phases_ = false;
    Stream stream2;
    Stream stream3;

private:
    void upload(const Symbolic &S);
    void ensure_rhs_capacity(long long nrhs);
    void factor_levels(int lo, int hi, bool record_level_events);
    struct PanelChain;
    bool factor_small_fronts(const LevelInfo &L);
    bool factor_panel_chains(const LevelInfo &L);
    void panel_block(const PanelChain &ch, const LevelInfo &L, int b);
    void factor_contribution_blocks(const LevelInfo &L, int slot);
    SweepKnobs sweep_knobs() const;
    void forward(const SweepLane &ln, int nr, int ldx, int lo, int hi, bool follows_factor);
    void backward(const SweepLane &ln, int nr, int ldx, bool y_in_x2, int hi, int lo);
    void sweep_pass(const SweepLane &ln, const Event *ev, const double *dB, long long ldin, double *dXo, long long ldout, int nr, int mode,
                    const MemberLayout *ml);
    SweepLane lane(int k) const { return k == 0 ? SweepLane{stream, d_X_, d_X2_, d_W_} : SweepLane{stream3, d_Xb_, d_X2b_, d_Wb_}; }
    void begin_factor(const double *d_src);
    void enqueue_factor_tail();
    void finish_factor();
    void newton_values(const double *h, bool on_device);
    void ensure_io(long long need);
    void read_batch_diag(double *logdet_out, long long *info_out) const;
    Stream stream_io_;
    Event ev_fact_, ev_inv_;
    template <class T> T *dalloc(size_t count);
    std::vector<void *> allocs_;

    const Symbolic *S_ = nullptr;
    const SelRec *d_selrec_ = nullptr;
    DevSym ds_{};
    std::vector<LevelInfo> levels_;
    std::vector<LevelInfo> swlevels_;
    int *d_sw_levellist_ = nullptr;
    SweepTask *d_swt_ = nullptr;
    int nswt_ = 0;
    const unsigned char *d_owncol_ = nullptr;
    const long long *d_zbptr_ = nullptr;
    const int *d_iperm_ = nullptr;
    int *d_levellist_ = nullptr;
    FwdTile *d_fwd_recs_ = nullptr;
    double *d_nzp_ = nullptr;
    long long nq_ = 0;
    Event ev_nzp_, ev_nzp0_;
    AsmRec *d_arec_ = nullptr;
    SyrkTile *d_syrk_recs_ = nullptr;
    EnvKnobs env_;
    FrontView *d_frec_ = nullptr, *d_frec2_ = nullptr, *d_sel_frec_ = nullptr;
    int *d_levellist2_ = nullptr;
    const int *d_wave_order_ = nullptr;
    int wave_first_[kWaveClasses] = {0, 0}, wave_count_[kWaveClasses] = {0, 0};
    void sweep_tasks(const SweepLane &ln, int phase, int nr, int ldx, bool follows_factor);
public:
    void set_external_stream(hipStream_t s, bool use, bool async);
    int level_times(int phase, double *out, int cap);
    void dist_front_phase(const double *d_nzval, int front, int what, int block);
private:
    void ensure_rdiag(hipStream_t st);
    bool nzp_pending_ = false;
    void ensure_dtile(hipStream_t st);
    Symbolic::SwChunk *d_swc_fwd_ = nullptr, *d_swc_bwd_ = nullptr;
    int *d_swc_listf_ = nullptr, *d_swc_listb_ = nullptr;
    double *d_dtile_ = nullptr;
    int nswc_ = 0;
    unsigned long long dtile_for_ = 0;
    double *d_rdiag_ = nullptr;
    unsigned long long factor_serial_ = 1, rdiag_for_ = 0;
    std::vector<int> sel_max_cols_, sel_max_trail_;
    int *d_dist_list_ = nullptr;
    bool selinv_begun_ = false;
    std::vector<Event> ev_level_[3];
    int level_slots_[3] = {0, 0, 0};
    void level_event(hipStream_t st, int phase, int slot);
    int *d_sub_first_ = nullptr, *d_sub_last_ = nullptr, *d_sel_levellist_ = nullptr;
    int nsub_cls_[3] = {0, 0, 0};
    double *d_L_ = nullptr, *d_Z_ = nullptr, *d_cb_ = nullptr, *d_nz_ = nullptr;
    const double *nz_src_ = nullptr;
    double *d_prior_ = nullptr;
    DevBuf<double> d_h_;
    DevBuf<long long> d_hmap_;
    long long hmap_cnt_ = 0, hmap_cap_ = 0;
    double *d_X_ = nullptr, *d_X2_ = nullptr, *d_W_ = nullptr, *d_part_ = nullptr;
    DevBuf<double> d_io_, d_tmp_;
    int *d_invlist_ = nullptr;
    std::vector<int> inv_nact_;
    std::vector<long long *> d_inv_toff_;
    double *d_invT_ = nullptr;
    int inv_maxc_ = 0;
    int inv_cap_ = EnvKnobs{}.inv_cap;
    static constexpr double kInvGrowthMax = 1e4;
    bool inv_cap_decided_ = false;
    double *d_pivgrowth_ = nullptr;
    void decide_inverse_cap();
    bool inverse_full_ = false;
    std::vector<Event> ev_flevel_;
    int bottom_top_level_ = 0, fused_gate_level_ = 0;
    int *d_inv_lvl_list_ = nullptr;
    std::vector<int> inv_lvl_first_, inv_lvl_maxc_;
    std::vector<std::vector<int>> inv_lvl_nact_;
    std::vector<long long *> d_inv_lvl_toff_;
    void invert_level(hipStream_t st, int lev);
    bool fact_event_valid_ = false;
    PinnedBuf<int> h_info_;
    PinnedBuf<double> h_qf_;
    Event ev_qf_;
    void prepare_quadform(long long nvec);
    PinnedBuf<double> h_logdet_;
    unsigned long long logdet_for_ = 0;
    Event ev_logdet_;
    void enqueue_logdet(hipStream_t st, bool timed);
    bool info_cached_ = false;
    void invert_diag_blocks(hipStream_t st, int b_from, int b_to);
    void start_inverse_async();
    void wait_inverse(hipStream_t st);
    int first_multiblock_level_ = 0;
    long long rhs_cap_ = 0, io_cap_ = 0, tmp_cap_ = 0;
    long long *d_yoff_ = nullptr;
    int *d_fchild_ = nullptr;
    std::vector<int> fc_levelptr_, fc_maxtrail_;
    void selinv_begin();
    void selinv_levels(int hi, int lo);
    double *d_Xb_ = nullptr, *d_X2b_ = nullptr, *d_Wb_ = nullptr;
    Event ev_lane_[2][5];
    Event ev_ready_, ev_ready2_, ev_done1_;
    int *d_info_ = nullptr;
    PinnedBuf<double> h_stage_, h_nzstage_;
    void host_upload_values(const double *nzval);
    Event ev_up_, ev_x_;
    std::vector<Event> ev_ring_;
    void host_io_reserve(long long count);
    void host_upload(const double *B, long long ldb, long long nrhs, double *d_dst);
    void host_download(const double *d_src, long long nrhs, double *X, long long ldx, hipStream_t after);
    struct RowDiagPlan { long long nseg = 0, cnt = 0, nvals = 0; DevBuf<long long> seg, off; DevBuf<int> p, q; DevBuf<double> vals, out; };
    std::vector<RowDiagPlan> rd_plans_;
    long long *d_in_colptr_ = nullptr;
    int *d_in_row_ = nullptr;
    DevBuf<double> d_qf_part_, d_qf_out_;
    long long qf_cap_ = 0;
    bool nz_held_ = false;
    Event ev_[8];
    std::vector<Event> ev_syrk_;
    long long l_size_ = 0, sum_trail_ = 0;
    int nbatch_ = 1;
    long long nmember_ = 0, nnz_member_ = 0;
    double *d_bpsum_ = nullptr, *d_bdiag_ = nullptr;
    PinnedBuf<double> h_bdiag_;
    int *d_bpbad_ = nullptr;
    unsigned long long bdiag_for_ = 0;
    Event ev_bdiag_;
    long long *d_bin_colptr_ = nullptr;
    int *d_bin_row_ = nullptr;
    DevBuf<double> d_bqf_part_, d_bqf_out_;
    PinnedBuf<double> h_bqf_;
    long long bqf_cap_ = 0;
    void enqueue_batch_diag(hipStream_t st);
    struct ConRows {
        int m = 0, maxchunks = 0;
        long long nnz = 0, maxlen = 0, totchunks = 0, colcap = 0;
        DevBuf<long long> rowptr;
        DevBuf<int> col, choff;
        DevBuf<double> val, e, R, part;
    };
    ConRows con_rows_upload(const ConHost &c);
    void con_reserve_cols(ConRows &a, long long cols, int members);
    struct ConDev : ConRows {
        DevBuf<double> At, B, Linv, amu, sig;
        std::vector<double> h_w, h_linv;
        double logdet_w = 0, ms = 0;
        unsigned long long serial = 0;
    } con_;
    struct BConDev : ConRows {
        long long piece = 0;
        DevBuf<long long> cinfo;
        DevBuf<double> At, B, W, Linv, amu, sig, stat;
        std::vector<double> h_logdet;
        std::vector<long long> h_cinfo;
        double ms = 0;
        bool ok = false;
        unsigned long long serial = 0;
    } bcon_;
    Event con_ev_[2], bcon_ev_[2], rb_ev_[2];
    struct RbmcSymDev {
        DevBuf<long long> rp;
        DevBuf<int> col, pos, dpos;
        DevBuf<double> Xc, Xt, mean, m2, base, out;
    };
    struct RbmcPlanDev {
        DevBuf<long long> bptr, eptr;
        DevBuf<int> rows, ns, loc, order[kRbmcClasses];
        DevBuf<unsigned char> owner;
        int cnt[kRbmcClasses] = {};
        DevBuf<double> scrM, scrR;
        int enclosure = -2;
        unsigned long long serial = 0;
    };
    struct RbmcState { RbmcSymDev sym; RbmcPlanDev plan; } rb_;
    void rbmc_upload_sym(const RbmcSym &sym);
    void rbmc_upload_plan(const RbmcPlan &plan);
    void con_drop();
    void prepare_batch_quadform(long long npairs);
    void enqueue_batch_quadform(hipStream_t st, const double *d_nz, const double *d_X, long long ldx, long long sx, long long nvec,
                                const double *d_mu);
};

void hip_check(hipError_t e, const char *what);

struct HostIoPlan { long long cols_per = 1, ppc = 1, rows_per = 0, slot_doubles = 0, nsl = 0, reserve = 0; };
HostIoPlan host_io_plan(long long n, long long nrhs, long long slice_bytes);
HostIoPlan host_io_plan_dir(long long n, long long nrhs, int download);

}
```

### gaussianmarkovrandomfields.jl_amd/csrc/device_plan.cpp

```cpp
#include "device_plan.h"

#include <algorithm>
#include <climits>
#include <cstdlib>
#include <stdexcept>
#include <string>

namespace gmrfx {

static std::vector<FrontView> front_views(const Symbolic &S, const std::vector<i32> &lst) {
    std::vector<FrontView> v(lst.size());
    for (size_t k = 0; k < lst.size(); k++) {
        const i32 s = lst[k];
        v[k] = FrontView{(int)s, S.ncols(s), S.nrows(s), (int)S.ld[s], (int)S.sfirst[s], 0, (long long)S.panelptr[s]};
    }
    return v;
}

static std::vector<int> even_odd_levellist(const Symbolic &S) {
    std::vector<int> l2(S.levellist.begin(), S.levellist.end());
    for (i32 l = 0; l < S.nlevels; l++) {
        const i64 f = S.levelptr[l] + S.level_nsmall[l], e = S.levelptr[l + 1];
        i64 w = f;
        for (i64 k = f; k < e; k += 2) l2[w++] = S.levellist[k];
// ... 300 lines not shown
        std::vector<int> &ord = P.wave_order;
        for (int k = 0; k < kWaveClasses; k++) {
            P.wave_first[k] = (int)ord.size();
            for (int t = 0; t < P.nswt; t++) {
                const int rows = tk[t].nt + tk[t].mroot;
                if (rows <= kWaveRows[k] && (k == 0 || rows > kWaveRows[k - 1])) ord.push_back(t);
            }
            P.wave_count[k] = (int)ord.size() - P.wave_first[k];
        }
        if ((int)ord.size() != P.nswt) throw std::runtime_error("internal: a sweep task exceeds the largest wave-task class");
        for (int t = 0; t < P.nswt; t++) ord.push_back(t);
    }
    P.levellist2 = even_odd_levellist(S);
    for (int k = 0; k < 3; k++) P.nsub_cls[k] = S.nsub_cls[k];
    P.frec = front_views(S, S.levellist);
    P.sel_frec = front_views(S, S.sel_levellist);
    P.frec2 = front_views(S, P.levellist2);

    P.sel_max_cols.assign(S.nlevels, 0);
    P.sel_max_trail.assign(S.nlevels, 0);
    for (i32 l = 0; l < S.nlevels; l++)
        for (i64 k = S.sel_levelptr[l] + S.sel_level_nsmall[l]; k < S.sel_levelptr[l + 1]; k++) {
            const i32 s = S.sel_levellist[k];
            P.sel_max_cols[l] = std::max(P.sel_max_cols[l], (int)S.ncols(s));
            P.sel_max_trail[l] = std::max(P.sel_max_trail[l], (int)(S.nrows(s) - S.ncols(s)));
        }
    P.levels = level_infos(S, S.levelptr, S.levellist, S.level_nsmall, S.level_ncls, &P.syrk_flops);
    P.swlevels = level_infos(S, S.sw_levelptr, S.sw_levellist, S.sw_level_nsmall, S.sw_level_ncls, nullptr);

    {
        std::vector<int> &il = P.invlist;
        for (i32 s = 0; s < ns; s++) {
            const bool mine = !S.shard_plan || S.owner[s] == S.shard_rank;
            if (S.ncols(s) > NB && mine) il.push_back(s);
        }
        std::sort(il.begin(), il.end(), [&](int a, int b) { return S.ncols(a) != S.ncols(b) ? S.ncols(a) > S.ncols(b) : a < b; });
        P.inv_maxc = il.empty() ? 0 : S.ncols(il[0]);
        for (int B = NB; B < P.inv_maxc; B *= 2) {
            long long acc = 0;
            P.inv_toff.push_back(stage_offsets(S, il, B, &acc));
            P.inv_nact.push_back((int)P.inv_toff.back().size());
            P.inv_tsize = std::max(P.inv_tsize, acc);
        }
        std::vector<int> &cat = P.inv_lvl_list;
        P.inv_lvl_first.assign(S.nlevels + 1, 0); P.inv_lvl_maxc.assign(S.nlevels, 0); P.inv_lvl_nact.assign(S.nlevels, {});
        std::vector<std::vector<int>> per(S.nlevels);
        for (int s : il) per[S.level[s]].push_back(s);
        for (i32 l = 0; l < S.nlevels; l++) {
            P.inv_lvl_first[l] = (int)cat.size();
            P.inv_lvl_maxc[l] = per[l].empty() ? 0 : S.ncols(per[l][0]);
            cat.insert(cat.end(), per[l].begin(), per[l].end());
        }
        P.inv_lvl_first[S.nlevels] = (int)cat.size();
        for (int B = NB; !cat.empty() && B < P.inv_maxc; B *= 2) {
            std::vector<long long> off(cat.size(), 0);
            for (i32 l = 0; l < S.nlevels; l++) {
                long long acc = 0;
                const std::vector<long long> lo = stage_offsets(S, per[l], B, &acc);
                std::copy(lo.begin(), lo.end(), off.begin() + P.inv_lvl_first[l]);
                P.inv_lvl_nact[l].push_back((int)lo.size());
            }
            P.inv_lvl_toff.push_back(off);
        }
    }
    {
        int &btl = P.bottom_top_level;
        for (size_t t = 0; t < S.swt_last.size(); t++) btl = std::max<int>(btl, S.level[S.swt_last[t]]);
        for (i32 s = 0; s < ns; s++) if (S.in_subtree[s]) btl = std::max<int>(btl, S.level[s]);
        btl = std::min<int>(btl, std::max<int>(S.nlevels - 1, 0));
        int gate = S.nlevels - 1;
        while (gate > 0 && P.levels[gate - 1].count <= 32) gate--;
        P.fused_gate_level = std::min<int>(std::max(gate, btl), std::max<int>(S.nlevels - 1, 0));
    }

    std::vector<double> cost;
    constexpr int SQ = 8;
    for (i32 l = 0; l < S.nlevels; l++) {
        LevelInfo &L = P.levels[l];
        cost.clear();
        L.syrk_off = (long long)P.syrk_recs.size();
        for (int k = L.nsmall; o.syrk_xcd && k < L.count; k++) {
            const i32 s = S.levellist[L.first + k];
            const int c = S.ncols(s), m = S.nrows(s) - c;
            const int T = (m + 63) / 64, nT = (m + 31) / 32;
            const i64 ch0 = S.childptr[s];
            const int nch = (int)(S.childptr[s + 1] - ch0);
            for (int I = 0; I < T; I += SQ)
                for (int J = 0; J <= I; J += SQ)
                    for (int bi = I; bi < std::min(I + SQ, T); bi++)
                        for (int bj = J; bj < std::min(J + SQ, bi + 1); bj++) {
                            cost.push_back((double)(c + 48) * (bi == bj ? 3 : 4));
                            SyrkTile t{};
                            t.pa = (long long)S.panelptr[s] + c;
                            t.cb = (long long)S.cbptr[s];
                            t.ch0 = (long long)ch0;
                            t.c = c; t.m = m; t.ld = (int)S.ld[s]; t.nch = nch;
                            t.bi = bi; t.bj = bj;
                            for (int q = 0; q < std::min(nch, 2); q++) {
                                const EdgeRec &e = P.edge[ch0 + q];
                                const int *et = P.etile.data() + e.tptr;
                                t.reloff[q] = e.reloff; t.cboff[q] = e.cboff; t.md[q] = e.md;
                                t.a0[q] = et[2 * bi]; t.a1[q] = et[std::min(2 * bi + 2, nT)];
                                t.b0[q] = et[2 * bj]; t.b1[q] = et[std::min(2 * bj + 2, nT)];
                            }
                            P.syrk_recs.push_back(t);
                        }
        }
        cut_xcd_runs(cost, L.syrk_split, &L.syrk_per, "contribution-block");
    }
    if (P.syrk_recs.empty()) P.syrk_recs.push_back(SyrkTile{});
    for (i32 l = 0; l < S.nlevels; l++) {
        LevelInfo &L = P.swlevels[l];
        cost.clear();
        L.fwd_off = (long long)P.fwd_recs.size();
        for (int k = L.nsmall; o.syrk_xcd && k < L.count; k++) {
            const i32 s = S.sw_levellist[L.first + k];
            const int c = S.ncols(s), r = S.nrows(s), m = r - c;
            const i64 ch0 = S.childptr[s];
            const int nch = (int)(S.childptr[s + 1] - ch0);
            for (int T = 0; T * 32 < m; T++) {
                FwdTile t{};
                t.pp = (long long)S.panelptr[s]; t.xoff = S.sfirst[s]; t.woff = S.wptr[s]; t.ch0 = (long long)ch0;
                t.c = c; t.r = r; t.ld = (int)S.ld[s]; t.i0 = c + 32 * T; t.nch = nch; t.tile = T;
                for (int q = 0; q < std::min(nch, 2); q++) {
                    const EdgeRec &e = P.edge[ch0 + q];
                    t.md[q] = e.md; t.reloff[q] = e.reloff; t.cwoff[q] = e.woff;
                    t.a0[q] = P.etile[(size_t)e.tptr + T]; t.a1[q] = P.etile[(size_t)e.tptr + T + 1];
                }
                P.fwd_recs.push_back(t);
                cost.push_back((double)(c + 64));
            }
        }
        cut_xcd_runs(cost, L.fwd_split, &L.fwd_per, "update-vector");
    }
    if (P.fwd_recs.empty()) P.fwd_recs.push_back(FwdTile{});
    P.arec.resize(S.levellist.size());
    for (size_t k = 0; k < S.levellist.size(); k++) {
        const i32 s = S.levellist[k];
        AsmRec a{};
        a.pp = (long long)S.panelptr[s];
        a.ch0 = (long long)S.childptr[s];
        a.c = S.ncols(s); a.ld = (int)S.ld[s]; a.first = (int)S.sfirst[s];
        a.nch = (int)(S.childptr[s + 1] - S.childptr[s]);
        for (int q = 0; q < std::min(a.nch, 2); q++) {
            const EdgeRec &e = P.edge[a.ch0 + q];
            a.reloff[q] = e.reloff; a.cboff[q] = e.cboff; a.eoff[q] = e.eoff; a.md[q] = e.md;
        }
        P.arec[k] = a;
    }
    if (P.arec.empty()) P.arec.push_back(AsmRec{});

    P.first_multiblock_level = S.nlevels;
    for (i32 l = 0; l < S.nlevels; l++) if (P.swlevels[l].max_cols > NB) { P.first_multiblock_level = l; break; }
    P.l_size = S.panelptr[ns];
    return P;
}

}
```

### gaussianmarkovrandomfields.jl_amd/csrc/device_plan.h

```cpp
#pragma once
#include <algorithm>
#include <utility>
#include <vector>

#include "symbolic.h"

namespace gmrfx {

constexpr int NB = 64;
constexpr int kChunkNc = 16;
constexpr int kChunkSpareRow = 288;
constexpr int kWaveClasses = 2;
constexpr int kWaveRows[kWaveClasses] = {160, 288};

struct EdgeRec {
    int d, md;
    int tptr;
    int nown;
    long long reloff;
    long long woff;
    long long cboff;
    long long eoff;
};

// ... 27 lines not shown
    long long pa;
    long long cb;
    long long ch0;
    int c, m, ld, nch;
    int bi, bj, pad0, pad1;
    long long reloff[2], cboff[2];
    int md[2];
    int a0[2], a1[2], b0[2], b1[2];
};
static_assert(sizeof(SyrkTile) == 128, "SyrkTile is one 128-byte record");

struct FwdTile {
    long long pp;
    long long xoff;
    long long woff;
    long long ch0;
    int c, r, ld, i0;
    int nch, tile;
    int md[2], a0[2], a1[2];
    int pad[4];
    long long reloff[2], cwoff[2];
};
static_assert(sizeof(FwdTile) == 128, "FwdTile is one 128-byte record");

struct SelRec {
    long long rel;
    long long zp;
    long long zbp;
    long long out;
    int m, cp, mp, ldp;
    int p, foreign, pad[2];
};
static_assert(sizeof(SelRec) == 64, "SelRec is 64 bytes");

struct LevelInfo {
    int first;
    int count;
    int nsmall;
    int ncls[4];
    int max_rows;
    int max_cols;
    int max_trail = 0;
    int min_trail = 0;
    int wider[3] = {0, 0, 0};
    long long syrk_off = 0;
    SyrkSplit syrk_split{};
    int syrk_per = 0;
    long long fwd_off = 0;
    SyrkSplit fwd_split{};
    int fwd_per = 0;

    int nbig() const { return count - nsmall; }
    int nblk() const { return (max_cols + NB - 1) / NB; }
    int wider_than(int cols) const { const size_t k = (size_t)cols / NB; return k < wider_blk_.size() ? wider_blk_[k] : 0; }
    void set_block_counts(std::vector<int> counts) { wider_blk_ = std::move(counts); }
private:
    std::vector<int> wider_blk_;
};

constexpr int kSyrkPipedMinCols = 128;
struct EnvKnobs {
    int inv_cap = 2048;
    int wave_max_nr = 16;
    bool level_mark = false;
    int fwd_front_min = 384;
    int bwd_front_min = 192;
    bool syrk_xcd = true;
    int syrk_piped_min = kSyrkPipedMinCols;
};
EnvKnobs read_env_knobs();

constexpr int kFwdWaveCols = 1024;
constexpr int kBwdWaveRows = 4096;

struct SweepKnobs {
    int inv_cap;
    int fwd_front_min, bwd_front_min;
    bool tile_records;
    int narrow_pass_max, narrow_pass_max_bwd;
    int front_max_cols;
    int wave_split_cols, wave_split_rows;
};

struct LevelBlocks {
    const LevelInfo *L;
    int inv_cap;
    int ntail;
    int nf;
    int nbk;
    int xmul_fronts(int j) const { return std::min(nf, L->wider_than(j * inv_cap)); }
    int own_fronts(int j) const { return std::min(nf, L->wider_than((j + 1) * inv_cap)); }
};
struct FwdLevelPlan : LevelBlocks {
    int cmin;
    bool wave;
    bool wave_split_k;
    enum Update { kNone, kRecords, kGrid } update;
};
struct BwdLevelPlan : LevelBlocks {
    int mmin;
    bool wave;
    bool wave_split_k;
    bool gemm;
};
FwdLevelPlan plan_forward_level(const LevelInfo &L, int nr, const SweepKnobs &k);
BwdLevelPlan plan_backward_level(const LevelInfo &L, int nr, const SweepKnobs &k);

constexpr int ASM_CW = 4;
constexpr int FWD_RB = 32;
constexpr int kAsmLdsWaveMaxRows = 1280, kAsmLdsWgMaxRows = 16384;
constexpr int kAsmHbmWgMaxGroups = 2200;
constexpr int kTrsmSplitMaxTiles = 128;
constexpr int kGemmBigKStep = 16, kGemmBigMinK = 256, kGemmBigMinM = 4096, kGemmBigMinN = 512;
constexpr int kGemmSmallTileMax = 256;
constexpr int kFwdUpdate16MaxTiles = 128;
constexpr int kBwdGemmWide8Min = 384, kBwdGemm8Max = 768;
constexpr int kPermuteNarrowMaxNr = 8;
constexpr int kNarrowPassMax = 32, kNarrowPassMaxBwd = 16;
constexpr int kWaveSplitCols = 128, kWaveSplitRows = 256;
constexpr int kFrontMaxCols = 128;

inline int cdiv(int a, int b) { return (a + b - 1) / b; }
inline unsigned odd(int v) { return (unsigned)(v | 1); }
inline int asm_ldmax(int max_rows) { return (max_rows + 1) & ~1; }

enum KernelVariant {
    kNoLaunch,
    kAssembleLdsWave, kAssembleLdsWg, kAssembleHbmWg, kAssembleHbmWave,
    kTrsmSplit, kTrsmWhole,
    kGemmNtBig, kGemmNt32, kGemmNt64,
    kFwdUpdate16, kFwdUpdate32,
    kBwdGemm16x8, kBwdGemm32x8, kBwdGemm32x4,
    kPermuteNarrow, kPermuteTiles,
    kWaveWhole, kWaveSplitK,
    kFwdOwnUpdate,
    kVariantCount
};
struct Launch {
    KernelVariant variant = kNoLaunch;
    unsigned gx = 0, gy = 1, gz = 1, block = 0;
    size_t lds = 0;
    bool raised_lds = false;
};
Launch choose_assemble(int nfronts, int max_cols, int max_rows);
Launch choose_assemble_hbm(int nfronts, int max_cols);
Launch choose_trsm(int nactive, int max_rows_below);
Launch choose_gemm_nt(int nactive, int K, int maxM, int maxN);
Launch choose_fwd_update(int nfronts, int max_trail);
Launch choose_fwd_update_wave(int per_xcd, int nr, bool split_k);
Launch choose_fwd_own_update(int nfronts, int max_cols, int blk, int cap);
Launch choose_bwd_gemm(int nfronts, int max_cols, int blk, int cap);
Launch choose_bwd_wave(int nfronts, int max_cols, int nr, bool split_k);
Launch choose_permute(int n, int nr);

struct PlanOptions {
    bool syrk_xcd = true;
    int chunk_nc = kChunkNc, chunk_spare_row = kChunkSpareRow;
};

struct DevicePlan {
    std::vector<SelRec> selrec;
    std::vector<int> qsrc, qdst, qcol, qcolptr;
    std::vector<EdgeRec> edge;
    std::vector<int> etile, erow;
    std::vector<unsigned char> owncol, foreign_parent;
    std::vector<int> fchild;
    std::vector<SweepTask> swt;
    std::vector<int> swc_listf, swc_listb;
    std::vector<int> wave_order;
    std::vector<int> levellist2;
    std::vector<FrontView> frec, frec2, sel_frec;
    std::vector<int> invlist;
    std::vector<std::vector<long long>> inv_toff;
    std::vector<int> inv_lvl_list;
    std::vector<std::vector<long long>> inv_lvl_toff;
    std::vector<SyrkTile> syrk_recs;
    std::vector<FwdTile> fwd_recs;
    std::vector<AsmRec> arec;
    std::vector<LevelInfo> levels, swlevels;
    std::vector<int> sel_max_cols, sel_max_trail;
    int inv_maxc = 0;
    long long inv_tsize = 0;
    std::vector<int> inv_nact, inv_lvl_first, inv_lvl_maxc;
    std::vector<std::vector<int>> inv_lvl_nact;
    std::vector<int> fc_levelptr, fc_maxtrail;
    int wave_first[kWaveClasses] = {}, wave_count[kWaveClasses] = {};
    int nsub_cls[3] = {};
    int bottom_top_level = 0, fused_gate_level = 0, first_multiblock_level = 0;
    double syrk_flops = 0;
    long long sum_trail = 0, l_size = 0, nq = 0;
    int nswt = 0, nswc = 0;
};

DevicePlan build_device_plan(const Symbolic &S, const PlanOptions &o);

}
```

### gaussianmarkovrandomfields.jl_amd/csrc/gmrfx_api.cpp

```cpp
#include "../../include/gmrfx.h"

#include <algorithm>
#include <chrono>
#include <climits>
#include <cmath>
#include <cstdlib>
#include <cstring>
#include <memory>
#include <stdexcept>
#include <string>
#include <system_error>
#include <thread>
#include <vector>

#include "device.h"
#include "symbolic.h"

using namespace gmrfx;

struct gmrfx_handle {
    Symbolic S;
    std::unique_ptr<Device> D;
    gmrfx_opts opts{};
    std::string err;
// ... 119 lines not shown
    if (so.coords && so.coord_dim != 2 && so.coord_dim != 3) throw std::invalid_argument("coord_dim must be 2 or 3");
    if (const char *e = std::getenv("GMRFX_SMALL_ROWS")) so.small_front_rows = std::atoi(e);
    if (const char *e = std::getenv("GMRFX_SUBTREE_MAX")) so.subtree_max = std::atoi(e);
    if (const char *e = std::getenv("GMRFX_SWEEP_TASK_ROWS")) so.sweep_task_rows = std::atoi(e);
    if (const char *e = std::getenv("GMRFX_MERGE_WIDE")) so.merge_wide = std::atoi(e);
    if (const char *e = std::getenv("GMRFX_TOP_BY_DEPTH")) so.top_by_depth = std::atoi(e);
    if (o.shard_world > 1 || (o.shard_world == 1 && o.shard_min_top > 0)) {
        so.shard_min_top = std::max(0, o.shard_min_top);
        if (o.shard_rank < 0 || o.shard_rank >= o.shard_world) throw std::invalid_argument("shard_rank out of range");
        so.shard_rank = o.shard_rank;
        so.shard_world = o.shard_world;
        if (const char *e = std::getenv("GMRFX_DIST_MIN")) so.dist_min_cols = std::atoi(e);
        so.subtree_max = 0;
    }
}

extern "C" int32_t gmrfx_create(int64_t n, const int64_t *colptr, const int64_t *rowval, int32_t index_base,
                                const int64_t *perm, const gmrfx_opts *opts, gmrfx_handle **out) {
    if (!out) { g_create_err = "out is null"; return GMRFX_ERR_INVALID_ARG; }
    *out = nullptr;
    if (!colptr || !rowval) { g_create_err = "colptr/rowval is null"; return GMRFX_ERR_INVALID_ARG; }
    std::unique_ptr<gmrfx_handle> h(new gmrfx_handle());
    if (!read_opts(opts, h->opts)) return GMRFX_ERR_INVALID_ARG;
    if (int32_t e = create_guarded(true, [&]() -> int32_t {
            SymOptions so;
            sym_options(h->opts, so);
            analyze(n, colptr, rowval, index_base, perm, so, h->S);
            h->opts.coords = nullptr;
            h->n_member = h->S.n; h->nnz_member = h->S.nnz_in;
            return GMRFX_OK;
        })) return e;
    if (int32_t e = attach_device(h.get(), false)) return e;
    *out = h.release();
    return GMRFX_OK;
}

extern "C" void gmrfx_destroy(gmrfx_handle *h) { delete h; }

extern "C" int32_t gmrfx_clone(const gmrfx_handle *h, gmrfx_handle **out) {
    if (!h || !out) return GMRFX_ERR_INVALID_ARG;
    *out = nullptr;
    std::unique_ptr<gmrfx_handle> c(new gmrfx_handle());
    try {
        c->S = h->S;
        c->opts = h->opts;
        c->nbatch = h->nbatch; c->n_member = h->n_member; c->nnz_member = h->nnz_member;
        if (h->D) {
            c->D.reset(new Device());
            c->D->clone_from(*h->D, c->S);
            if (h->D->batched()) c->D->set_batch((int)c->nbatch, c->n_member, c->nnz_member);
        }
        c->con = h->con;
        if (c->D && c->con.m > 0) c->D->con_set(c->con);
        c->bcon = h->bcon;
        if (c->D && c->bcon.m > 0) c->D->bcon_set(c->bcon);
    } catch (const std::exception &e) {
        g_create_err = e.what();
        return GMRFX_ERR_HIP;
    }
    *out = c.release();
    return GMRFX_OK;
}

static int32_t refactorize_impl(gmrfx_handle *h, const double *nz, int64_t *info, bool dev) {
    return guarded(h, [&]() -> int32_t {
        if (int32_t e = need_device(h, false)) return e;
        if (!nz) throw std::invalid_argument("nzval is null");
        h->D->refactorize(nz, dev);
        return pivot_status(h, info);
    });
}
extern "C" int32_t gmrfx_refactorize(gmrfx_handle *h, const double *nzval, int64_t *info) { return refactorize_impl(h, nzval, info, false); }

static int32_t refactorize_solve_impl(gmrfx_handle *h, const double *nz, const double *B, int64_t ldb, int64_t nrhs, double *X, int64_t ldx,
                                      int64_t *info, bool dev) {
    return guarded(h, [&]() -> int32_t {
        if (int32_t e = need_device(h, false)) return e;
        if (!nz) throw std::invalid_argument("nzval is null");
        check_rhs(h, B, ldb, X, ldx, nrhs, "B/X");
        h->D->refactorize_solve(nz, dev, B, ldb, nrhs, X, ldx, dev);
        return pivot_status(h, info);
    });
}
extern "C" int32_t gmrfx_refactorize_solve(gmrfx_handle *h, const double *nzval, const double *B, int64_t ldb, int64_t nrhs, double *X,
                                           int64_t ldx, int64_t *info) { return refactorize_solve_impl(h, nzval, B, ldb, nrhs, X, ldx, info, false); }
extern "C" int32_t gmrfx_refactorize_solve_dev(gmrfx_handle *h, const double *d_nzval, const double *d_B, int64_t ldb, int64_t nrhs, double *d_X,
                                               int64_t ldx, int64_t *info) { return refactorize_solve_impl(h, d_nzval, d_B, ldb, nrhs, d_X, ldx, info, true); }

extern "C" int32_t gmrfx_set_prior(gmrfx_handle *h, const double *prior_nzval, const int64_t *map, int64_t cnt, int32_t index_base) {
    return guarded(h, [&]() -> int32_t {
        if (int32_t e = need_device(h, false)) return e;
        if (!prior_nzval || (cnt > 0 && !map) || cnt < 0) throw std::invalid_argument("prior_nzval / map is null");
        std::vector<long long> m((size_t)cnt);
        for (int64_t k = 0; k < cnt; k++) m[k] = map[k] - index_base;
        h->D->set_prior(prior_nzval, m.data(), cnt);
        return GMRFX_OK;
    });
}
static int32_t refactorize_update_impl(gmrfx_handle *h, const double *hv, int64_t *info, bool dev) {
    return guarded(h, [&]() -> int32_t {
        if (int32_t e = need_device(h, false)) return e;
        h->D->refactorize_update(hv, dev);
        return pivot_status(h, info);
    });
}
extern "C" int32_t gmrfx_refactorize_logpdf_dev(gmrfx_handle *h, const double *d_nzval, const double *d_X, int64_t ldx, int64_t nvec,
                                                const double *d_mu, double *quad, double *logdet, int64_t *info) {
    return guarded(h, [&]() -> int32_t {
        if (int32_t e = need_device(h, false)) return e;
        if (!d_nzval) throw std::invalid_argument("nzval is null");
        if (nvec > 0 && (!d_X || !quad)) throw std::invalid_argument("X / quad is null");
        h->D->refactorize_logpdf(d_nzval, d_X, ldx, nvec, d_mu, quad, logdet);
        return pivot_status(h, info);
    });
}
static int32_t refactorize_update_solve_impl(gmrfx_handle *h, const double *hv, const double *B, int64_t ldb, int64_t nrhs, double *X, int64_t ldx,
                                             int64_t *info, bool dev) {
    return guarded(h, [&]() -> int32_t {
        if (int32_t e = need_device(h, false)) return e;
        check_rhs(h, B, ldb, X, ldx, nrhs, "B/X");
        h->D->refactorize_update_solve(hv, dev, B, ldb, nrhs, X, ldx, dev);
        return pivot_status(h, info);
    });
}
extern "C" int32_t gmrfx_refactorize_update_solve(gmrfx_handle *h, const double *hvals, const double *B, int64_t ldb, int64_t nrhs, double *X,
                                                  int64_t ldx, int64_t *info) { return refactorize_update_solve_impl(h, hvals, B, ldb, nrhs, X, ldx, info, false); }
extern "C" int32_t gmrfx_refactorize_update_solve_dev(gmrfx_handle *h, const double *d_hvals, const double *d_B, int64_t ldb, int64_t nrhs,
                                                      double *d_X, int64_t ldx, int64_t *info) { return refactorize_update_solve_impl(h, d_hvals, d_B, ldb, nrhs, d_X, ldx, info, true); }
extern "C" int32_t gmrfx_refactorize_update(gmrfx_handle *h, const double *hvals, int64_t *info) { return refactorize_update_impl(h, hvals, info, false); }
extern "C" int32_t gmrfx_refactorize_update_dev(gmrfx_handle *h, const double *d_hvals, int64_t *info) { return refactorize_update_impl(h, d_hvals, info, true); }

extern "C" int32_t gmrfx_refactorize_phase(gmrfx_handle *h, const double *d_nzval, int32_t phase) {
    return guarded(h, [&]() -> int32_t {
        if (int32_t e = need_device(h, false)) return e;
        if (phase == 0 && !d_nzval) throw std::invalid_argument("d_nzval is null");
        if (phase < 0 || phase > h->S.nlevels - h->S.shard_level) throw std::invalid_argument("phase must be 0 (own subtrees) or 1 + k (top level k)");
        h->D->refactorize_phase(d_nzval, phase);
        return GMRFX_OK;
    });
}
extern "C" int32_t gmrfx_level_times(gmrfx_handle *h, int32_t which, double *ms, int64_t cap, int64_t *count) {
    return guarded(h, [&]() -> int32_t {
        if (int32_t e = need_device(h, false)) return e;
        if (!ms || !count) throw std::invalid_argument("null output");
        *count = h->D->level_times(which, ms, (int)cap);
        return GMRFX_OK;
    });
}
extern "C" int32_t gmrfx_host_io_plan(int64_t n, int64_t nrhs, int32_t download, int64_t *plan) {
    if (!plan || n < 0 || nrhs < 0) return GMRFX_ERR_INVALID_ARG;
    const gmrfx::HostIoPlan p = gmrfx::host_io_plan_dir(n, nrhs, download);
    plan[0] = p.cols_per; plan[1] = p.ppc; plan[2] = p.rows_per; plan[3] = p.slot_doubles; plan[4] = p.nsl; plan[5] = p.reserve;
    return GMRFX_OK;
}
extern "C" int32_t gmrfx_set_stream(gmrfx_handle *h, void *hip_stream, int32_t use_external, int32_t async_phases) {
    return guarded(h, [&]() -> int32_t {
        if (int32_t e = need_device(h, false)) return e;
        h->D->set_external_stream((hipStream_t)hip_stream, use_external != 0, async_phases != 0);
        return GMRFX_OK;
    });
}
extern "C" int32_t gmrfx_shard_info(const gmrfx_handle *h, int64_t *n_edges, int64_t *n_top_fronts, int64_t *shard_level) {
    if (!h) return GMRFX_ERR_INVALID_ARG;
    const Symbolic &S = h->S;
    int64_t ntop = 0;
    for (i32 s = 0; s < S.nsuper; s++) ntop += S.is_top[s];
    if (n_edges) *n_edges = (int64_t)S.shard_edges.size();
    if (n_top_fronts) *n_top_fronts = ntop;
    if (shard_level) *shard_level = S.shard_level;
    return GMRFX_OK;
}
extern "C" int32_t gmrfx_shard_edges(const gmrfx_handle *h, int64_t *child, int64_t *src, int64_t *dst, int64_t *level,
                                     int64_t *cb_offset, int64_t *cb_count, int64_t *w_row0, int64_t *w_nrows, int64_t *zb_offset,
                                     int64_t *child_level) {
    if (!h || !child || !src || !dst || !level || !cb_offset || !cb_count || !w_row0 || !w_nrows) return GMRFX_ERR_INVALID_ARG;
    const Symbolic &S = h->S;
    const std::vector<i64> &wptr = S.wptr;
    for (size_t k = 0; k < S.shard_edges.size(); k++) {
        const i32 d = S.shard_edges[k], p = S.sparent[d];
        const int64_t m = S.nrows(d) - S.ncols(d);
        child[k] = d; src[k] = S.owner[d]; dst[k] = S.owner[p]; level[k] = S.level[p];
        const bool end = S.owner[d] == S.shard_rank || S.owner[p] == S.shard_rank;
        cb_offset[k] = end ? S.cbptr[d] : -1; cb_count[k] = m * m;
        w_row0[k] = wptr[d]; w_nrows[k] = m;
        if (zb_offset) zb_offset[k] = end ? S.zbptr[d] : -1;
        if (child_level) child_level[k] = S.level[d];
    }
    return GMRFX_OK;
}
extern "C" int32_t gmrfx_shard_dist_fronts(const gmrfx_handle *h, int64_t *counts, int64_t *front, int64_t *cols, int64_t *rows,
                                           int64_t *panel_offset, int64_t *panel_ld, int64_t *level, int64_t *gptr, int64_t *grank) {
    if (!h || !counts) return GMRFX_ERR_INVALID_ARG;
    const Symbolic &S = h->S;
    const size_t nf = S.dist_fronts.size();
    counts[0] = (int64_t)nf; counts[1] = (int64_t)S.dist_grank.size(); counts[2] = (int64_t)S.xf_child.size(); counts[3] = S.shard_world;
    for (size_t k = 0; k < nf; k++) {
        const i32 s = S.dist_fronts[k];
        if (front) front[k] = s;
        if (cols) cols[k] = S.ncols(s);
        if (rows) rows[k] = S.nrows(s);
        if (panel_offset) panel_offset[k] = S.panelptr[s];
        if (panel_ld) panel_ld[k] = S.ld[s];
        if (level) level[k] = S.level[s];
    }
    if (gptr) for (size_t k = 0; k < S.dist_gptr.size(); k++) gptr[k] = S.dist_gptr[k];
    if (grank) for (size_t k = 0; k < S.dist_grank.size(); k++) grank[k] = S.dist_grank[k];
    return GMRFX_OK;
}
extern "C" int32_t gmrfx_dist_front_block(const gmrfx_handle *h, int32_t front, int32_t block, int64_t *offset, int64_t *count) {
    if (!h || !offset || !count) return GMRFX_ERR_INVALID_ARG;
    const Symbolic &S = h->S;
    if (front < 0 || front >= S.nsuper || !S.is_dist(front) || block < 0 || block >= S.panel_blocks(front)) return GMRFX_ERR_INVALID_ARG;
    const i32 g = S.group_size(front), me = S.group_pos(front, S.shard_rank);
    *offset = -1; *count = 0;
    if (me < 0) return GMRFX_OK;
    const i64 ld = S.ld[front];
    *count = (i64)std::min<i64>(256, S.ncols(front) - 256 * (i64)block) * ld;
    if (!S.compact_here(front)) *offset = S.panelptr[front] + 256 * (i64)block * ld;
    else if (block % g == me) *offset = S.panelptr[front] + (i64)(block / g) * 256 * ld;
    else *offset = S.panelptr[front] + S.compact_window(front, block & 1);
    return GMRFX_OK;
}
extern "C" int32_t gmrfx_shard_transfers(const gmrfx_handle *h, int64_t *child, int64_t *src, int64_t *dst, int64_t *level,
                                         int64_t *offset, int64_t *count, int64_t *col0) {
    if (!h) return GMRFX_ERR_INVALID_ARG;
    const Symbolic &S = h->S;
    for (size_t k = 0; k < S.xf_child.size(); k++) {
        if (child) child[k] = S.xf_child[k];
        if (src) src[k] = S.xf_src[k];
        if (dst) dst[k] = S.xf_dst[k];
        if (level) level[k] = S.xf_level[k];
        if (offset) offset[k] = S.xf_off[k];
        if (count) count[k] = S.xf_cnt[k];
        if (col0) col0[k] = S.xf_col0[k];
    }
    return GMRFX_OK;
}
extern "C" int32_t gmrfx_dist_front_phase(gmrfx_handle *h, const double *d_nzval, int32_t front, int32_t what, int32_t block) {
    return guarded(h, [&]() -> int32_t {
        if (int32_t e = need_device(h, false)) return e;
        h->D->dist_front_phase(d_nzval, front, what, block);
        return GMRFX_OK;
    });
}
extern "C" int32_t gmrfx_shard_owner(const gmrfx_handle *h, int64_t *owner, int64_t *is_top) {
    if (!h || !owner) return GMRFX_ERR_INVALID_ARG;
    for (i32 s = 0; s < h->S.nsuper; s++) { owner[s] = h->S.owner[s]; if (is_top) is_top[s] = h->S.is_top[s]; }
    return GMRFX_OK;
}
extern "C" void *gmrfx_device_ptr(gmrfx_handle *h, int32_t which) {
    if (!h || !h->D) return nullptr;
    try {
        if (which == 2 || which == 3) h->D->ensure_rhs(64);
    } catch (...) { return nullptr; }
    switch (which) {
        case 0: return h->D->cb_arena();
        case 1: return h->D->factor_panels();
        case 2: return h->D->rhs_x();
        case 3: return h->D->rhs_w();
        default: return nullptr;
    }
}
extern "C" int32_t gmrfx_solve_phase(gmrfx_handle *h, const double *d_B, int64_t ldb, int64_t nrhs, double *d_X, int64_t ldx, int32_t phase) {
    return guarded(h, [&]() -> int32_t {
        if (int32_t e = need_device(h, true)) return e;
        if (phase == 0 && !d_B) throw std::invalid_argument("d_B is null");
        if (phase == 0 && ldb < h->S.n) throw std::invalid_argument("ldb < n");
        if (phase == 3 && (!d_X || ldx < h->S.n)) throw std::invalid_argument("d_X is null or ldx < n");
        h->D->solve_phase(d_B, ldb, nrhs, d_X, ldx, phase);
        return GMRFX_OK;
    });
}
extern "C" int32_t gmrfx_shard_rows(const gmrfx_handle *h, int32_t kind, int64_t *nblocks, int64_t *owner, int64_t *row0, int64_t *nrows,
                                    int64_t *level) {
    if (!h || !nblocks) return GMRFX_ERR_INVALID_ARG;
    const Symbolic &S = h->S;
    std::vector<int64_t> o, a, c, l;
    if (kind == 2) {
        for (i32 s = 0; s < S.nsuper; s++) if (S.is_top[s]) { o.push_back(S.owner[s]); a.push_back(S.sfirst[s]); c.push_back(S.ncols(s)); l.push_back(S.level[s]); }
    } else if (kind == 3) {
        for (size_t k = 0; k < S.shard_sub_root.size(); k++) {
            const i32 t = S.shard_sub_root[k];
            o.push_back(S.owner[t]); a.push_back(S.shard_sub_col0[k]); c.push_back(S.sfirst[t + 1] - S.shard_sub_col0[k]); l.push_back(S.level[t]);
        }
    } else return GMRFX_ERR_INVALID_ARG;
    *nblocks = (int64_t)o.size();
    if (owner && row0 && nrows)
        for (size_t k = 0; k < o.size(); k++) { owner[k] = o[k]; row0[k] = a[k]; nrows[k] = c[k]; if (level) level[k] = l[k]; }
    return GMRFX_OK;
}
extern "C" int32_t gmrfx_logdet_partial(gmrfx_handle *h, double *out) {
    return guarded(h, [&]() -> int32_t {
        if (int32_t e = need_device(h, true)) return e;
        if (!out) throw std::invalid_argument("out is null");
        *out = h->D->logdet();
        return GMRFX_OK;
    });
}
extern "C" int32_t gmrfx_refactorize_dev(gmrfx_handle *h, const double *d_nzval, int64_t *info) { return refactorize_impl(h, d_nzval, info, true); }

static int32_t solve_impl(gmrfx_handle *h, const double *B, int64_t ldb, int64_t nrhs, double *X, int64_t ldx, bool dev, int mode) {
    return guarded(h, [&]() -> int32_t {
        if (int32_t e = need_device(h, true)) return e;
        check_rhs(h, B, ldb, X, ldx, nrhs, "B/X");
        if (nrhs == 0) return GMRFX_OK;
        h->D->solve(B, ldb, nrhs, X, ldx, dev, mode);
// ... 1150 lines not shown
```

### gaussianmarkovrandomfields.jl_amd/gmrfx/_lib.py

```python
from __future__ import annotations

import ctypes as C
import os

import numpy as np

_HERE = os.path.dirname(os.path.abspath(__file__))
_LIBPATH = os.environ.get("GMRFX_LIB", os.path.join(os.path.dirname(_HERE), "libgmrfx.so"))

GMRFX_OK = 0
ERR_INVALID_ARG, ERR_NO_DEVICE, ERR_HIP, ERR_NOT_FACTORIZED, ERR_NOT_POSDEF, ERR_ALLOC = 1, 2, 3, 4, 5, 6


class GmrfxOpts(C.Structure):
    _fields_ = [
        ("struct_size", C.c_int32), ("uplo", C.c_int32), ("ordering", C.c_int32), ("device", C.c_int32),
        ("symbolic_only", C.c_int32), ("check_posdef", C.c_int32), ("nd_leaf", C.c_int32),
        ("relax_cols", C.c_int32), ("relax_zeros", C.c_double), ("coord_dim", C.c_int32),
        ("reserved0", C.c_int32), ("coords", C.c_void_p), ("shard_rank", C.c_int32), ("shard_world", C.c_int32),
        ("shard_min_top", C.c_int32), ("reserved1", C.c_int32),
    ]


class GmrfxStats(C.Structure):
    _fields_ = [(k, C.c_int64) for k in (
        "n", "nnz_q_tri", "nnz_l", "nnz_l_stored", "nsuper", "nlevels", "max_cols", "max_rows", "sum_rows",
        "n_small_fronts", "n_big_fronts")] + [(k, C.c_double) for k in (
        "factor_flops", "bytes_factor", "bytes_cb_arena", "bytes_device_total", "ms_symbolic", "ms_factor",
        "ms_solve", "ms_solve_fwd", "ms_solve_bwd", "ms_solve_perm", "ms_backward_solve", "ms_logdet",
        "ms_selinv")] + [("last_nrhs", C.c_int64), ("fail_col", C.c_int64), ("ms_syrk", C.c_double),
                         ("syrk_flops", C.c_double), ("syrk_launches", C.c_int64),
                         ("ms_quadform", C.c_double), ("inv_cap", C.c_int64), ("ms_inv_decide", C.c_double),
                         ("ms_rbmc", C.c_double)]

    def asdict(self):
        return {k: getattr(self, k) for k, _ in self._fields_}


class GmrfxError(RuntimeError):
    def __init__(self, code, msg):
        super().__init__(f"gmrfx error {code}: {msg}")
        self.code = code


class NoDeviceError(GmrfxError):
    pass


class PosDefException(GmrfxError):
    pass


_lib = None
EXPORTS = [
    "gmrfx_last_create_error", "gmrfx_last_error", "gmrfx_create", "gmrfx_destroy", "gmrfx_clone",
    "gmrfx_dense_apply_dev", "gmrfx_transpose_dev",
    "gmrfx_refactorize", "gmrfx_refactorize_dev", "gmrfx_refactorize_solve", "gmrfx_refactorize_solve_dev",
    "gmrfx_refactorize_update_solve", "gmrfx_refactorize_update_solve_dev", "gmrfx_refactorize_logpdf_dev", "gmrfx_solve", "gmrfx_solve_dev", "gmrfx_backward_solve",
    "gmrfx_backward_solve_dev", "gmrfx_logdet", "gmrfx_selinv_compute", "gmrfx_selinv_diag", "gmrfx_selinv_nnz",
    "gmrfx_selinv_csc", "gmrfx_selinv_extract", "gmrfx_get_perm", "gmrfx_get_stats", "gmrfx_symbolic_sizes",
    "gmrfx_symbolic_get", "gmrfx_get_factor_values", "gmrfx_refactorize_phase", "gmrfx_shard_info",
    "gmrfx_shard_edges", "gmrfx_shard_owner", "gmrfx_device_ptr", "gmrfx_set_stream", "gmrfx_level_times", "gmrfx_shard_dist_fronts", "gmrfx_shard_transfers",
    "gmrfx_dist_front_phase", "gmrfx_logdet_partial", "gmrfx_solve_phase",
    "gmrfx_shard_rows", "gmrfx_set_prior", "gmrfx_refactorize_update", "gmrfx_refactorize_update_dev",
    "gmrfx_quadform", "gmrfx_quadform_dev", "gmrfx_selinv_dot", "gmrfx_selinv_row_diag", "gmrfx_kl_cholesky",
    "gmrfx_selinv_row_diag_plan", "gmrfx_selinv_row_diag_apply", "gmrfx_selinv_row_diag_free",
    "gmrfx_symbolic_sweep_tasks", "gmrfx_symbolic_sweep_chunks", "gmrfx_selinv_phase", "gmrfx_host_io_plan", "gmrfx_dist_front_block",
    "gmrfx_create_batched", "gmrfx_batch_size", "gmrfx_batch_refactorize", "gmrfx_batch_refactorize_dev", "gmrfx_batch_logdet",
    "gmrfx_batch_solve", "gmrfx_batch_solve_dev", "gmrfx_batch_backward_solve", "gmrfx_batch_backward_solve_dev",
    "gmrfx_batch_quadform", "gmrfx_batch_quadform_dev", "gmrfx_batch_refactorize_logpdf_dev",
    "gmrfx_constraints_set", "gmrfx_constraints_info", "gmrfx_constraints_get", "gmrfx_constraints_mean",
    "gmrfx_constraints_correct", "gmrfx_constraints_correct_dev", "gmrfx_constraints_var", "gmrfx_sample", "gmrfx_sample_dev",
    "gmrfx_batch_constraints_set", "gmrfx_batch_constraints_info", "gmrfx_batch_constraints_get", "gmrfx_batch_constraints_mean",
    "gmrfx_batch_constraints_correct", "gmrfx_batch_constraints_correct_dev", "gmrfx_batch_constraints_var", "gmrfx_batch_sample",
    "gmrfx_batch_sample_dev", "gmrfx_batch_constrained_logpdf_dev",
    "gmrfx_rbmc_var", "gmrfx_rbmc_var_dev", "gmrfx_rbmc_plan",
]


def source_tree_hash() -> str:
    import glob, hashlib
    h = hashlib.sha256()
    files = sorted(glob.glob(os.path.join(_HERE, "..", "csrc", "*.hip")) + glob.glob(os.path.join(_HERE, "..", "csrc", "*.cpp")) +
                   glob.glob(os.path.join(_HERE, "..", "csrc", "*.h")), key=os.path.basename)
    files.append(os.path.join(_HERE, "..", "..", "include", "gmrfx.h"))
    for f in files:
        h.update(os.path.basename(f).encode())
        with open(f, "rb") as fh:
            h.update(fh.read())
    return h.hexdigest()[:16]


def lib():
    global _lib
    if _lib is None:
        if not os.path.exists(_LIBPATH):
            raise ImportError(f"{_LIBPATH} not found: build it with `make -C {os.path.dirname(_HERE)}` "
                              "(or __graft_entry__.build()); there is no non-HIP fallback")
        if not os.environ.get("GMRFX_NO_TORCH"):
            try:
                import torch
            except Exception:
                pass
        L = C.CDLL(_LIBPATH)
        vp, i64, i32, dbl = C.c_void_p, C.c_int64, C.c_int32, C.c_double
        L.gmrfx_last_create_error.restype = C.c_char_p
        L.gmrfx_last_error.restype = C.c_char_p
        L.gmrfx_last_error.argtypes = [vp]
        L.gmrfx_create.argtypes = [i64, vp, vp, i32, vp, C.POINTER(GmrfxOpts), C.POINTER(vp)]
        L.gmrfx_destroy.argtypes = [vp]
        L.gmrfx_destroy.restype = None
        L.gmrfx_clone.argtypes = [vp, C.POINTER(vp)]
        L.gmrfx_refactorize.argtypes = [vp, vp, C.POINTER(i64)]
        L.gmrfx_refactorize_dev.argtypes = [vp, vp, C.POINTER(i64)]
        L.gmrfx_dense_apply_dev.argtypes = [vp, i64, i64, vp, vp, vp]
        L.gmrfx_transpose_dev.argtypes = [vp, i64, i64, vp, vp]
        L.gmrfx_refactorize_solve.argtypes = [vp, vp, vp, i64, i64, vp, i64, C.POINTER(i64)]
        L.gmrfx_refactorize_solve_dev.argtypes = [vp, vp, vp, i64, i64, vp, i64, C.POINTER(i64)]
        L.gmrfx_refactorize_logpdf_dev.argtypes = [vp, vp, vp, i64, i64, vp, vp, C.POINTER(dbl), C.POINTER(i64)]
        L.gmrfx_refactorize_update_solve.argtypes = [vp, vp, vp, i64, i64, vp, i64, C.POINTER(i64)]
        L.gmrfx_refactorize_update_solve_dev.argtypes = [vp, vp, vp, i64, i64, vp, i64, C.POINTER(i64)]
        for nm in ("gmrfx_solve", "gmrfx_solve_dev", "gmrfx_backward_solve", "gmrfx_backward_solve_dev"):
            getattr(L, nm).argtypes = [vp, vp, i64, i64, vp, i64]
        L.gmrfx_logdet.argtypes = [vp, C.POINTER(dbl)]
        L.gmrfx_selinv_compute.argtypes = [vp]
        L.gmrfx_selinv_diag.argtypes = [vp, vp]
        L.gmrfx_selinv_nnz.argtypes = [vp, C.POINTER(i64)]
        L.gmrfx_selinv_csc.argtypes = [vp, i32, vp, vp, vp]
        L.gmrfx_selinv_extract.argtypes = [vp, i64, vp, vp, i32, vp]
        L.gmrfx_get_perm.argtypes = [vp, i32, vp]
        L.gmrfx_get_stats.argtypes = [vp, C.POINTER(GmrfxStats), i32]
        L.gmrfx_symbolic_sizes.argtypes = [vp, vp]
        L.gmrfx_symbolic_get.argtypes = [vp] + [vp] * 10
        L.gmrfx_symbolic_sweep_tasks.argtypes = [vp, C.POINTER(i64), C.POINTER(i64), vp, vp, vp]
        L.gmrfx_symbolic_sweep_chunks.argtypes = [vp, vp, C.POINTER(i64), vp, vp, vp, vp, vp]
        L.gmrfx_get_factor_values.argtypes = [vp, vp]
        L.gmrfx_refactorize_phase.argtypes = [vp, vp, i32]
        L.gmrfx_shard_info.argtypes = [vp, C.POINTER(i64), C.POINTER(i64), C.POINTER(i64)]
        L.gmrfx_shard_edges.argtypes = [vp] + [vp] * 10
        L.gmrfx_selinv_phase.argtypes = [vp, i32, i32, i32]
        L.gmrfx_shard_owner.argtypes = [vp, vp, vp]
        L.gmrfx_device_ptr.argtypes = [vp, i32]
        L.gmrfx_device_ptr.restype = C.c_void_p
        L.gmrfx_set_stream.argtypes = [vp, vp, i32, i32]
        L.gmrfx_level_times.argtypes = [vp, i32, vp, i64, C.POINTER(i64)]
        L.gmrfx_shard_dist_fronts.argtypes = [vp] + [vp] * 9
        L.gmrfx_shard_transfers.argtypes = [vp] + [vp] * 7
        L.gmrfx_dist_front_phase.argtypes = [vp, vp, i32, i32, i32]
        L.gmrfx_logdet_partial.argtypes = [vp, C.POINTER(dbl)]
        L.gmrfx_solve_phase.argtypes = [vp, vp, i64, i64, vp, i64, i32]
        L.gmrfx_shard_rows.argtypes = [vp, i32, C.POINTER(i64), vp, vp, vp, vp]
        L.gmrfx_set_prior.argtypes = [vp, vp, vp, i64, i32]
        L.gmrfx_refactorize_update.argtypes = [vp, vp, C.POINTER(i64)]
        L.gmrfx_refactorize_update_dev.argtypes = [vp, vp, C.POINTER(i64)]
        L.gmrfx_quadform.argtypes = [vp, vp, vp, i64, i64, vp, vp]
        L.gmrfx_quadform_dev.argtypes = [vp, vp, vp, i64, i64, vp, vp]
        L.gmrfx_selinv_dot.argtypes = [vp, i64, vp, vp, vp, i32, C.POINTER(dbl)]
        L.gmrfx_selinv_row_diag.argtypes = [vp, i64, vp, vp, vp, i32, vp]
        L.gmrfx_kl_cholesky.argtypes = [i64, vp, i64, i32, vp, i64, vp, vp, vp, vp, i32, dbl, i32, vp, C.POINTER(i64)]
        L.gmrfx_selinv_row_diag_plan.argtypes = [vp, i64, vp, vp, i32, C.POINTER(i64)]
        L.gmrfx_selinv_row_diag_apply.argtypes = [vp, i64, vp, vp]
        L.gmrfx_selinv_row_diag_free.argtypes = [vp, i64]
        L.gmrfx_host_io_plan.argtypes = [i64, i64, i32, vp]
        L.gmrfx_dist_front_block.argtypes = [vp, i32, i32, C.POINTER(i64), C.POINTER(i64)]
        L.gmrfx_create_batched.argtypes = [i64, vp, vp, i32, vp, i64, C.POINTER(GmrfxOpts), C.POINTER(vp)]
        L.gmrfx_batch_size.argtypes = [vp, C.POINTER(i64), C.POINTER(i64)]
        L.gmrfx_batch_refactorize.argtypes = [vp, vp, vp]
        L.gmrfx_batch_refactorize_dev.argtypes = [vp, vp, vp]
        L.gmrfx_batch_logdet.argtypes = [vp, vp]
        for nm in ("gmrfx_batch_solve", "gmrfx_batch_solve_dev", "gmrfx_batch_backward_solve", "gmrfx_batch_backward_solve_dev"):
            getattr(L, nm).argtypes = [vp, vp, i64, i64, i64, vp, i64, i64]
        L.gmrfx_batch_quadform.argtypes = [vp, vp, vp, i64, i64, i64, vp, vp]
        L.gmrfx_batch_quadform_dev.argtypes = [vp, vp, vp, i64, i64, i64, vp, vp]
        L.gmrfx_batch_refactorize_logpdf_dev.argtypes = [vp, vp, vp, i64, i64, i64, vp, vp, vp, vp]
        L.gmrfx_constraints_set.argtypes = [vp, i64, vp, vp, vp, i32, vp]
        L.gmrfx_constraints_info.argtypes = [vp, C.POINTER(i64), C.POINTER(dbl), C.POINTER(dbl), C.POINTER(dbl)]
        L.gmrfx_constraints_get.argtypes = [vp, vp, i64, vp]
        L.gmrfx_constraints_mean.argtypes = [vp, vp, vp, C.POINTER(dbl)]
        L.gmrfx_constraints_correct.argtypes = [vp, vp, i64, i64]
        L.gmrfx_constraints_correct_dev.argtypes = [vp, vp, i64, i64]
        L.gmrfx_constraints_var.argtypes = [vp, vp]
        L.gmrfx_sample.argtypes = [vp, vp, i64, i64, vp, vp, i64]
        L.gmrfx_sample_dev.argtypes = [vp, vp, i64, i64, vp, vp, i64]
        L.gmrfx_batch_constraints_set.argtypes = [vp, i64, vp, vp, vp, i32, vp]
        L.gmrfx_batch_constraints_info.argtypes = [vp, C.POINTER(i64), vp, C.POINTER(dbl), vp, C.POINTER(dbl)]
        L.gmrfx_batch_constraints_get.argtypes = [vp, i64, vp, i64, vp]
        L.gmrfx_batch_constraints_mean.argtypes = [vp, vp, vp, vp]
        L.gmrfx_batch_constraints_correct.argtypes = [vp, vp, i64, i64, i64]
        L.gmrfx_batch_constraints_correct_dev.argtypes = [vp, vp, i64, i64, i64]
        L.gmrfx_batch_constraints_var.argtypes = [vp, vp]
        L.gmrfx_batch_sample.argtypes = [vp, vp, i64, i64, i64, vp, vp, i64, i64]
        L.gmrfx_batch_sample_dev.argtypes = [vp, vp, i64, i64, i64, vp, vp, i64, i64]
        L.gmrfx_batch_constrained_logpdf_dev.argtypes = [vp, vp, vp, i64, i64, i64, vp, vp, vp, vp, vp, vp]
        L.gmrfx_rbmc_var.argtypes = [vp, vp, vp, i64, i64, i32, vp]
        L.gmrfx_rbmc_var_dev.argtypes = [vp, vp, vp, i64, i64, i32, vp]
        L.gmrfx_rbmc_plan.argtypes = [vp, i32, i32, vp, vp, vp, vp, vp]
        for nm in EXPORTS[2:]:
            if nm not in ("gmrfx_destroy", "gmrfx_device_ptr"):
                getattr(L, nm).restype = i32
        _lib = L
    return _lib


def ptr(a):
    return None if a is None else a.ctypes.data_as(C.c_void_p)


def check(code, handle=None):
    if code == GMRFX_OK:
        return
    L = lib()
    msg = (L.gmrfx_last_error(handle) if handle else L.gmrfx_last_create_error()) or b""
    msg = msg.decode("utf-8", "replace")
    if code == ERR_INVALID_ARG:
        raise ValueError(f"gmrfx: {msg}")
    if code == ERR_NO_DEVICE:
        raise NoDeviceError(code, msg)
    if code == ERR_NOT_POSDEF:
        raise PosDefException(code, msg)
    raise GmrfxError(code, msg)
```

### include/gmrfx.h

```cpp
#ifndef GMRFX_H
#define GMRFX_H

#include <stdint.h>

#ifdef __cplusplus
extern "C" {
#endif

typedef struct gmrfx_handle gmrfx_handle;

enum {
    GMRFX_OK = 0,
    GMRFX_ERR_INVALID_ARG = 1,
    GMRFX_ERR_NO_DEVICE = 2,
    GMRFX_ERR_HIP = 3,
    GMRFX_ERR_NOT_FACTORIZED = 4,
    GMRFX_ERR_NOT_POSDEF = 5,
    GMRFX_ERR_ALLOC = 6
};

enum { GMRFX_UPLO_UPPER = 0, GMRFX_UPLO_LOWER = 1 };
enum { GMRFX_ORDER_AUTO = 0, GMRFX_ORDER_NATURAL = 1 };

typedef struct gmrfx_opts {
    int32_t struct_size;
    int32_t uplo;
    int32_t ordering;
    int32_t device;
    int32_t symbolic_only;
    int32_t check_posdef;
    int32_t nd_leaf;
    int32_t relax_cols;
    double  relax_zeros;
    int32_t coord_dim;
    int32_t reserved0;
    const double *coords;
    int32_t shard_rank, shard_world;
    int32_t shard_min_top;
    int32_t reserved1;
} gmrfx_opts;

typedef struct gmrfx_stats {
    int64_t n, nnz_q_tri, nnz_l, nnz_l_stored;
    int64_t nsuper, nlevels, max_cols, max_rows, sum_rows;
    int64_t n_small_fronts, n_big_fronts;
    double  factor_flops;
    double  bytes_factor, bytes_cb_arena, bytes_device_total;
    double  ms_symbolic;
    double  ms_factor, ms_solve, ms_solve_fwd, ms_solve_bwd, ms_solve_perm, ms_backward_solve,
            ms_logdet, ms_selinv;
    int64_t last_nrhs;
    int64_t fail_col;
    double  ms_syrk, syrk_flops;
    int64_t syrk_launches;
    double  ms_quadform;
    int64_t inv_cap;
    double  ms_inv_decide;
    double  ms_rbmc;
} gmrfx_stats;

const char *gmrfx_last_create_error(void);
const char *gmrfx_last_error(const gmrfx_handle *h);

int32_t gmrfx_create(int64_t n, const int64_t *colptr, const int64_t *rowval, int32_t index_base,
                     const int64_t *perm, const gmrfx_opts *opts, gmrfx_handle **out);
void    gmrfx_destroy(gmrfx_handle *h);
int32_t gmrfx_clone(const gmrfx_handle *h, gmrfx_handle **out);

int32_t gmrfx_refactorize(gmrfx_handle *h, const double *nzval, int64_t *info);
int32_t gmrfx_refactorize_dev(gmrfx_handle *h, const double *d_nzval, int64_t *info);
int32_t gmrfx_refactorize_solve(gmrfx_handle *h, const double *nzval, const double *B, int64_t ldb, int64_t nrhs, double *X, int64_t ldx,
                                int64_t *info);
int32_t gmrfx_refactorize_solve_dev(gmrfx_handle *h, const double *d_nzval, const double *d_B, int64_t ldb, int64_t nrhs, double *d_X,
                                    int64_t ldx, int64_t *info);

int32_t gmrfx_refactorize_logpdf_dev(gmrfx_handle *h, const double *d_nzval, const double *d_X, int64_t ldx, int64_t nvec,
                                     const double *d_mu, double *quad , double *logdet , int64_t *info);

int32_t gmrfx_set_prior(gmrfx_handle *h, const double *prior_nzval, const int64_t *map, int64_t cnt, int32_t index_base);
int32_t gmrfx_refactorize_update(gmrfx_handle *h, const double *hvals, int64_t *info);
int32_t gmrfx_refactorize_update_dev(gmrfx_handle *h, const double *d_hvals, int64_t *info);
int32_t gmrfx_refactorize_update_solve(gmrfx_handle *h, const double *hvals, const double *B, int64_t ldb, int64_t nrhs, double *X, int64_t ldx,
                                       int64_t *info);
int32_t gmrfx_refactorize_update_solve_dev(gmrfx_handle *h, const double *d_hvals, const double *d_B, int64_t ldb, int64_t nrhs, double *d_X,
                                           int64_t ldx, int64_t *info);

int32_t gmrfx_refactorize_phase(gmrfx_handle *h, const double *d_nzval, int32_t phase);
int32_t gmrfx_shard_info(const gmrfx_handle *h, int64_t *n_edges, int64_t *n_top_fronts, int64_t *shard_level);
int32_t gmrfx_shard_edges(const gmrfx_handle *h, int64_t *child, int64_t *src, int64_t *dst, int64_t *level,
                          int64_t *cb_offset, int64_t *cb_count, int64_t *w_row0, int64_t *w_nrows,
                          int64_t *zb_offset , int64_t *child_level );
int32_t gmrfx_selinv_phase(gmrfx_handle *h, int32_t what, int32_t level_hi, int32_t level_lo);
int32_t gmrfx_shard_owner(const gmrfx_handle *h, int64_t *owner , int64_t *is_top );
void   *gmrfx_device_ptr(gmrfx_handle *h, int32_t which );
int32_t gmrfx_solve_phase(gmrfx_handle *h, const double *d_B, int64_t ldb, int64_t nrhs, double *d_X, int64_t ldx, int32_t phase);
int32_t gmrfx_set_stream(gmrfx_handle *h, void *hip_stream, int32_t use_external, int32_t async_phases);
int32_t gmrfx_shard_dist_fronts(const gmrfx_handle *h, int64_t *counts , int64_t *front, int64_t *cols, int64_t *rows,
                                int64_t *panel_offset, int64_t *panel_ld, int64_t *level, int64_t *gptr, int64_t *grank);
int32_t gmrfx_shard_transfers(const gmrfx_handle *h, int64_t *child, int64_t *src, int64_t *dst, int64_t *level,
                              int64_t *offset, int64_t *count, int64_t *col0);
int32_t gmrfx_dist_front_phase(gmrfx_handle *h, const double *d_nzval, int32_t front, int32_t what, int32_t block);
int32_t gmrfx_dist_front_block(const gmrfx_handle *h, int32_t front, int32_t block, int64_t *offset, int64_t *count);
int32_t gmrfx_level_times(gmrfx_handle *h, int32_t which, double *ms, int64_t cap, int64_t *count);
int32_t gmrfx_shard_rows(const gmrfx_handle *h, int32_t kind, int64_t *nblocks, int64_t *owner, int64_t *row0, int64_t *nrows,
                         int64_t *level);
int32_t gmrfx_logdet_partial(gmrfx_handle *h, double *out);

int32_t gmrfx_host_io_plan(int64_t n, int64_t nrhs, int32_t download, int64_t *plan );

int32_t gmrfx_solve(gmrfx_handle *h, const double *B, int64_t ldb, int64_t nrhs, double *X, int64_t ldx);
int32_t gmrfx_solve_dev(gmrfx_handle *h, const double *d_B, int64_t ldb, int64_t nrhs, double *d_X, int64_t ldx);

int32_t gmrfx_backward_solve(gmrfx_handle *h, const double *Z, int64_t ldz, int64_t nrhs, double *X, int64_t ldx);
int32_t gmrfx_backward_solve_dev(gmrfx_handle *h, const double *d_Z, int64_t ldz, int64_t nrhs, double *d_X, int64_t ldx);

int32_t gmrfx_logdet(gmrfx_handle *h, double *out);

int32_t gmrfx_quadform(gmrfx_handle *h, const double *nzval, const double *X, int64_t ldx, int64_t nvec,
                       const double *mu, double *out);
int32_t gmrfx_quadform_dev(gmrfx_handle *h, const double *d_nzval, const double *d_X, int64_t ldx, int64_t nvec,
                           const double *d_mu, double *out);

int32_t gmrfx_dense_apply_dev(gmrfx_handle *h, int64_t n1, int64_t n2, const double *d_D, const double *d_T, double *d_R);
int32_t gmrfx_transpose_dev(gmrfx_handle *h, int64_t rows, int64_t cols, const double *d_src, double *d_dst);

int32_t gmrfx_selinv_compute(gmrfx_handle *h);
int32_t gmrfx_selinv_diag(gmrfx_handle *h, double *out );
int32_t gmrfx_selinv_nnz(gmrfx_handle *h, int64_t *nnz);
int32_t gmrfx_selinv_csc(gmrfx_handle *h, int32_t index_base, int64_t *colptr, int64_t *rowval, double *nzval);
int32_t gmrfx_selinv_extract(gmrfx_handle *h, int64_t ncol, const int64_t *colptr, const int64_t *rowval,
                             int32_t index_base, double *out_nzval);
int32_t gmrfx_selinv_dot(gmrfx_handle *h, int64_t ncol, const int64_t *colptr, const int64_t *rowval,
                         const double *nzval, int32_t index_base, double *out);
int32_t gmrfx_selinv_row_diag(gmrfx_handle *h, int64_t m, const int64_t *rowptr, const int64_t *colind,
                              const double *values, int32_t index_base, double *out);
int32_t gmrfx_selinv_row_diag_plan(gmrfx_handle *h, int64_t m, const int64_t *rowptr, const int64_t *colind,
                                   int32_t index_base, int64_t *plan);
int32_t gmrfx_selinv_row_diag_apply(gmrfx_handle *h, int64_t plan, const double *values, double *out);
int32_t gmrfx_selinv_row_diag_free(gmrfx_handle *h, int64_t plan);

int32_t gmrfx_get_perm(const gmrfx_handle *h, int32_t index_base, int64_t *perm);
int32_t gmrfx_get_stats(const gmrfx_handle *h, gmrfx_stats *out, int32_t struct_size);

int32_t gmrfx_symbolic_sizes(const gmrfx_handle *h, int64_t *sizes);
int32_t gmrfx_symbolic_get(const gmrfx_handle *h, int64_t *super_first, int64_t *super_parent,
                           int64_t *row_ptr, int64_t *rows, int64_t *rel, int64_t *panel_ptr,
                           int64_t *panel_ld, int64_t *level, int64_t *q_src, int64_t *q_dst);
int32_t gmrfx_symbolic_sweep_tasks(const gmrfx_handle *h, int64_t *ntasks, int64_t *rows_cap, int64_t *first,
                                   int64_t *last, int64_t *lrow);
int32_t gmrfx_symbolic_sweep_chunks(const gmrfx_handle *h, int64_t *nchunks, int64_t *nrows, int64_t *task_ptr,
                                    int64_t *slot, int64_t *fwd, int64_t *bwd, int64_t *rows);
int32_t gmrfx_get_factor_values(gmrfx_handle *h, double *out);

int32_t gmrfx_create_batched(int64_t n, const int64_t *colptr, const int64_t *rowval, int32_t index_base, const int64_t *perm,
                             int64_t nbatch, const gmrfx_opts *opts, gmrfx_handle **out);
int32_t gmrfx_batch_size(const gmrfx_handle *h, int64_t *nbatch, int64_t *n_member);
int32_t gmrfx_batch_refactorize(gmrfx_handle *h, const double *nzval, int64_t *info );
int32_t gmrfx_batch_refactorize_dev(gmrfx_handle *h, const double *d_nzval, int64_t *info );
int32_t gmrfx_batch_logdet(gmrfx_handle *h, double *out );
int32_t gmrfx_batch_solve(gmrfx_handle *h, const double *B, int64_t ldb, int64_t sb, int64_t nrhs, double *X, int64_t ldx, int64_t sx);
int32_t gmrfx_batch_solve_dev(gmrfx_handle *h, const double *d_B, int64_t ldb, int64_t sb, int64_t nrhs, double *d_X, int64_t ldx, int64_t sx);
int32_t gmrfx_batch_backward_solve(gmrfx_handle *h, const double *Z, int64_t ldz, int64_t sz, int64_t nrhs, double *X, int64_t ldx, int64_t sx);
int32_t gmrfx_batch_backward_solve_dev(gmrfx_handle *h, const double *d_Z, int64_t ldz, int64_t sz, int64_t nrhs, double *d_X, int64_t ldx,
                                       int64_t sx);
int32_t gmrfx_batch_quadform(gmrfx_handle *h, const double *nzval, const double *X, int64_t ldx, int64_t sx, int64_t nvec,
                             const double *mu, double *quad);
int32_t gmrfx_batch_quadform_dev(gmrfx_handle *h, const double *d_nzval, const double *d_X, int64_t ldx, int64_t sx, int64_t nvec,
                                 const double *d_mu, double *quad);
int32_t gmrfx_batch_refactorize_logpdf_dev(gmrfx_handle *h, const double *d_nzval, const double *d_X, int64_t ldx, int64_t sx, int64_t nvec,
                                           const double *d_mu, double *quad , double *logdet ,
                                           int64_t *info );

int32_t gmrfx_constraints_set(gmrfx_handle *h, int64_t m, const int64_t *rowptr, const int64_t *colind, const double *values,
                              int32_t index_base, const double *e);
int32_t gmrfx_constraints_info(gmrfx_handle *h, int64_t *m, double *logdet_W, double *logdet_AAt, double *ms);
int32_t gmrfx_constraints_get(gmrfx_handle *h, double *A_tilde_T , int64_t ld, double *W );
int32_t gmrfx_constraints_mean(gmrfx_handle *h, const double *mu , double *mean_c ,
                               double *log_correction );
int32_t gmrfx_constraints_correct(gmrfx_handle *h, double *X, int64_t ldx, int64_t nvec);
int32_t gmrfx_constraints_correct_dev(gmrfx_handle *h, double *d_X, int64_t ldx, int64_t nvec);
int32_t gmrfx_constraints_var(gmrfx_handle *h, double *out );
int32_t gmrfx_sample(gmrfx_handle *h, const double *Z, int64_t ldz, int64_t nrhs, const double *mu , double *X, int64_t ldx);
int32_t gmrfx_sample_dev(gmrfx_handle *h, const double *d_Z, int64_t ldz, int64_t nrhs, const double *d_mu , double *d_X,
                         int64_t ldx);

int32_t gmrfx_batch_constraints_set(gmrfx_handle *h, int64_t m, const int64_t *rowptr, const int64_t *colind, const double *values,
                                    int32_t index_base, const double *e);
int32_t gmrfx_batch_constraints_info(gmrfx_handle *h, int64_t *m, double *logdet_W , double *logdet_AAt,
                                     int64_t *cinfo , double *ms);
int32_t gmrfx_batch_constraints_get(gmrfx_handle *h, int64_t member, double *A_tilde_T , int64_t ld,
                                    double *W );
int32_t gmrfx_batch_constraints_mean(gmrfx_handle *h, const double *mu , double *mean_c ,
                                     double *log_correction );
int32_t gmrfx_batch_constraints_correct(gmrfx_handle *h, double *X, int64_t ldx, int64_t sx, int64_t nvec);
int32_t gmrfx_batch_constraints_correct_dev(gmrfx_handle *h, double *d_X, int64_t ldx, int64_t sx, int64_t nvec);
int32_t gmrfx_batch_constraints_var(gmrfx_handle *h, double *out );
int32_t gmrfx_batch_sample(gmrfx_handle *h, const double *Z, int64_t ldz, int64_t sz, int64_t nrhs, const double *mu ,
                           double *X, int64_t ldx, int64_t sx);
int32_t gmrfx_batch_sample_dev(gmrfx_handle *h, const double *d_Z, int64_t ldz, int64_t sz, int64_t nrhs,
                               const double *d_mu , double *d_X, int64_t ldx, int64_t sx);
int32_t gmrfx_batch_constrained_logpdf_dev(gmrfx_handle *h, const double *d_nzval, const double *d_X, int64_t ldx, int64_t sx, int64_t nvec,
                                           const double *d_mu, double *quad , double *logdet ,
                                           double *log_correction , int64_t *info ,
                                           int64_t *cinfo );

int32_t gmrfx_kl_cholesky(int64_t n, const double *theta, int64_t ldt, int32_t theta_on_device,
                          const int64_t *L_colptr, int64_t ntasks, const int64_t *task_rowptr, const int64_t *task_rows,
                          const int64_t *task_colptr, const int64_t *task_cols, int32_t index_base, double reg,
                          int32_t device, double *nzval, int64_t *info);

int32_t gmrfx_rbmc_var(gmrfx_handle *h, const double *nzval, const double *Z, int64_t ldz, int64_t nsamples,
                       int32_t enclosure_size, double *out );
int32_t gmrfx_rbmc_var_dev(gmrfx_handle *h, const double *d_nzval, const double *d_Z, int64_t ldz, int64_t nsamples,
                           int32_t enclosure_size, double *d_out );
int32_t gmrfx_rbmc_plan(gmrfx_handle *h, int32_t enclosure_size, int32_t index_base, int64_t *counts,
                        int64_t *block_ptr, int64_t *rows, int64_t *n_interior, int64_t *owner);

#ifdef __cplusplus
}
#endif
#endif
```

Before: 82.36 million DoF/s.

## Plan fine-grained release of forward-sweep pieces against factorization progress

Adds a release planner that uses per-level cost estimates to decide, for each forward-sweep piece (dtile, chunked bottom tasks, inverse, assemble, product, update), which factor event it must wait on. Some pieces can start once a level's SYRK begins rather than after the whole level is factored. Bottom sweep tasks are split into ranges so they can begin earlier. The goal is tighter overlap of the fused factor and solve, at the cost of more events and launches and a risk of ordering errors if the plan and the sweep drift out of step.

```diff
diff --git a/gaussianmarkovrandomfields.jl_amd/csrc/device.cpp b/gaussianmarkovrandomfields.jl_amd/csrc/device.cpp
--- a/gaussianmarkovrandomfields.jl_amd/csrc/device.cpp
+++ b/gaussianmarkovrandomfields.jl_amd/csrc/device.cpp
@@ -98,6 +98,7 @@
     inv_maxc_ = P.inv_maxc; inv_nact_ = P.inv_nact; inv_lvl_first_ = P.inv_lvl_first; inv_lvl_maxc_ = P.inv_lvl_maxc; inv_lvl_nact_ = P.inv_lvl_nact;
     fc_levelptr_ = P.fc_levelptr; fc_maxtrail_ = P.fc_maxtrail;
     std::copy_n(P.wave_first, kWaveClasses, wave_first_); std::copy_n(P.wave_count, kWaveClasses, wave_count_); std::copy_n(P.nsub_cls, 3, nsub_cls_);
+    release_base_ = P.release;
     bottom_top_level_ = P.bottom_top_level; fused_gate_level_ = P.fused_gate_level; first_multiblock_level_ = P.first_multiblock_level;
     syrk_flops = P.syrk_flops; sum_trail_ = P.sum_trail; l_size_ = P.l_size; nq_ = P.nq; nswt_ = P.nswt; nswc_ = P.nswc;
 
@@ -425,9 +426,10 @@
     return two;
 }
 
-void Device::factor_contribution_blocks(const LevelInfo &L, int slot) {
+void Device::factor_contribution_blocks(const LevelInfo &L, int slot, const Event *about_to_start) {
     const int *list = d_levellist_ + L.first + L.nsmall;
     const int nf = L.nbig();
+    if (about_to_start) HC(hipEventRecord(*about_to_start, stream));
     HC(hipEventRecord(ev_syrk_[2 * slot], stream));
     const bool huge = env_.syrk_xcd && !sharded() && L.max_trail >= 4096 && L.max_cols >= 1024;
     if (env_.syrk_xcd) launch_syrk_cb_recs(stream, ds_, d_syrk_recs_ + L.syrk_off, L.syrk_split, L.syrk_per, d_L_, d_cb_, huge ? 1 : 0, L.max_cols >= env_.syrk_piped_min);
@@ -436,7 +438,7 @@
     HC(hipEventRecord(ev_syrk_[2 * slot + 1], stream));
 }
 
-void Device::factor_levels(int lo, int hi, bool record_level_events) {
+void Device::factor_levels(int lo, int hi, const ReleasePlan *plan) {
     if (lo == 0) {
         const int big = INT_MAX;
         HC(hipMemcpyAsync(d_info_, &big, sizeof(int), hipMemcpyHostToDevice, stream));
@@ -461,12 +463,12 @@
         if (nf > 0 && nzp_pending_) { HC(hipStreamWaitEvent(stream, ev_nzp_, 0)); nzp_pending_ = false; }
         launch_assemble(stream, ds_, d_levellist_ + L.first + L.nsmall, d_arec_ + L.first + L.nsmall, d_nzp_, nf, L.max_cols, L.max_rows, nz_src_, d_L_, d_cb_);
         const bool two = factor_panel_chains(L);
-        if (nf > 0 && L.max_trail > 0) factor_contribution_blocks(L, nsy++);
+        if (nf > 0 && L.max_trail > 0) factor_contribution_blocks(L, nsy++, plan && plan->record_syrk_start[lev] ? &ev_window_[lev] : nullptr);
         if (split_small && !two) {
             HC(hipEventRecord(ev_done1_, stream3));
             HC(hipStreamWaitEvent(stream, ev_done1_, 0));
         }
-        if (record_level_events) HC(hipEventRecord(ev_flevel_[lev], stream));
+        if (plan && plan->record_factored[lev]) HC(hipEventRecord(ev_flevel_[lev], stream));
     }
     syrk_launches = nsy;
     if (lo == 0 && nzp_pending_) { HC(hipStreamWaitEvent(stream, ev_nzp_, 0)); nzp_pending_ = false; }
@@ -552,16 +554,18 @@
         dB = d_io_; dXo = d_io_; ldin = n; ldout = n;
     }
     while ((int)ev_flevel_.size() < nl + 1) { Event e; e.create(hipEventDisableTiming); ev_flevel_.push_back(std::move(e)); }
+    while ((int)ev_window_.size() < nl + 1) { Event e; e.create(hipEventDisableTiming); ev_window_.push_back(std::move(e)); }
+    const int PW = pass_width(nrhs);
+    const int nr = (int)std::min<long long>(PW, nrhs), ldx = nr;
+    const ReleasePlan &plan = release_plan(nr);
     if (!b_on_device) {
         host_upload(B, ldb, nrhs, d_io_);
         HC(hipStreamWaitEvent(stream, ev_up_, 0));
     }
     begin_factor(src);
     HC(hipEventRecord(ev_ready_, stream));
-    factor_levels(0, nl, true);
+    factor_levels(0, nl, &plan);
     enqueue_factor_tail();
-    const int PW = pass_width(nrhs);
-    const int nr = (int)std::min<long long>(PW, nrhs), ldx = nr;
     const Event *ev = ev_lane_[0];
     const SweepLane ln0 = lane(0), side{stream2, ln0.X, ln0.X2, ln0.W};
     HC(hipStreamWaitEvent(side.st, ev_ready_, 0));
@@ -630,7 +634,7 @@
         src = d_nz_;
     }
     begin_factor(src);
-    factor_levels(0, (int)levels_.size(), false);
+    factor_levels(0, (int)levels_.size(), nullptr);
     enqueue_factor_tail();
     inverse_pending = true;
     HC(hipStreamSynchronize(stream));
@@ -650,11 +654,11 @@
         nz_src_ = d_nzval;
         nz_held_ = false;
         factorized = false;
-        factor_levels(0, split, false);
+        factor_levels(0, split, nullptr);
     } else {
         const int lev = split + phase - 1;
         if (lev >= nl) throw std::invalid_argument("refactorize phase beyond the last level");
-        factor_levels(lev, lev + 1, false);
+        factor_levels(lev, lev + 1, nullptr);
     }
     HC(hipEventRecord(ev_[1], stream));
     if (!async_phases_) {
@@ -809,12 +813,19 @@
     io_cap_ = cap;
 }
 
-void Device::sweep_tasks(const SweepLane &ln, int phase, int nr, int ldx, bool follows_factor) {
+void Device::sweep_tasks(const SweepLane &ln, int phase, int nr, int ldx, bool follows_factor, int t0, int t1, int ranges) {
     if (nr > env_.wave_max_nr) {
         constexpr int pad_kb = 16;
         const size_t extra = (follows_factor && phase == 1) ? (size_t)pad_kb * 1024 : 0;
         ensure_dtile(ln.st);
-        launch_sweep_chunks(ln.st, ds_, phase, d_swt_, nswt_, d_swc_fwd_, d_swc_bwd_, d_swc_listf_, d_swc_listb_, d_dtile_, d_L_, ln.X,
+        if (t1 < 0) {
+            const int per = ((nswt_ + std::max(ranges, 1) - 1) / std::max(ranges, 1) + 7) / 8 * 8;
+            for (int a = 0; a < nswt_; a += std::max(per, 8))
+                launch_sweep_chunks(ln.st, ds_, phase, d_swt_ + a, std::min(per, nswt_ - a), d_swc_fwd_, d_swc_bwd_, d_swc_listf_, d_swc_listb_, d_dtile_,
+                                    d_L_, ln.X, phase == 1 ? ln.W : nullptr, nr, ldx, extra);
+            return;
+        }
+        launch_sweep_chunks(ln.st, ds_, phase, d_swt_ + t0, t1 - t0, d_swc_fwd_, d_swc_bwd_, d_swc_listf_, d_swc_listb_, d_dtile_, d_L_, ln.X,
                             phase == 1 ? ln.W : nullptr, nr, ldx, extra);
         return;
     }
@@ -849,15 +860,38 @@
                       kFrontMaxCols, kWaveSplitCols, kWaveSplitRows};
 }
 
+const ReleasePlan &Device::release_plan(int nr) {
+    if (release_plan_nr_ != nr || release_plan_cap_ != inv_cap_) {
+        ReleaseInput in = release_input(release_base_, nr, nr > env_.wave_max_nr);
+        if (test_force_windows_) for (ReleaseLevel &L : in.levels) L.cost_ratio = 0;
+        release_plan_ = plan_forward_release(in);
+        release_plan_nr_ = nr; release_plan_cap_ = inv_cap_;
+    }
+    return release_plan_;
+}
+
 void Device::forward(const SweepLane &ln, int nr, int ldx, int lo, int hi, bool follows_factor) {
     const SweepKnobs knobs = sweep_knobs();
     if (env_.level_mark && lo == 0) { launch_level_mark(ln.st, 1, -1); level_event(ln.st, 1, 0); }
+    const ReleasePlan *plan = follows_factor ? &release_plan(nr) : nullptr;
+    size_t ip = 1;
+    auto released = [&](int kind, int lev) -> const ReleasePiece & {
+        const ReleasePiece &p = plan->pieces.at(ip++);
+        if (p.kind != kind || (kind >= kRelInverse && p.level != lev)) throw std::logic_error("forward sweep and release plan out of step");
+        if (p.enqueue_wait) HC(hipStreamWaitEvent(ln.st, p.wait == kWaitFactored ? ev_flevel_[p.wait_level] : ev_window_[p.wait_level], 0));
+        return p;
+    };
     if (follows_factor) {
-        HC(hipStreamWaitEvent(ln.st, ev_flevel_[fused_gate_level_], 0));
+        if (lo != 0) throw std::logic_error("the pipelined forward sweep starts at the bottom");
+        released(kRelDtile, 0);
         if (nr <= env_.wave_max_nr && nswt_ > 0) rdiag_for_ = 0;
         dtile_for_ = 0;
-    }
-    if (lo == 0) sweep_tasks(ln, 1, nr, ldx, follows_factor);
+        for (int k = 0; k < plan->task_ranges; k++) {
+            const ReleasePiece &p = released(kRelTasks, 0);
+            if (nr > env_.wave_max_nr) sweep_tasks(ln, 1, nr, ldx, true, p.t0, p.t1);
+            else sweep_tasks(ln, 1, nr, ldx, true);
+        }
+    } else if (lo == 0) sweep_tasks(ln, 1, nr, ldx, false, 0, -1, test_task_ranges_);
     if (lo == 0)
         for (int k = 0, off = 0; k < 3; off += nsub_cls_[k], k++)
             launch_subtree(ln.st, ds_, 1, d_sub_first_ + off, d_sub_last_ + off, nsub_cls_[k], kClsRows[k], nullptr, d_L_, nullptr,
@@ -866,8 +900,9 @@
         const LevelInfo &L = swlevels_[lev];
         if (env_.level_mark) { launch_level_mark(ln.st, 1, lev); level_event(ln.st, 1, 1 + lev); }
         if (follows_factor) {
-            if (lev > fused_gate_level_) HC(hipStreamWaitEvent(ln.st, ev_flevel_[lev], 0));
+            released(kRelInverse, lev);
             invert_level(ln.st, lev);
+            released(kRelAssemble, lev);
         } else if (lev == std::max(lo, first_multiblock_level_)) wait_inverse(ln.st);
         for (int k = 0, off = 0; k < 4; off += L.ncls[k], k++)
             launch_fwd_small(ln.st, ds_, d_sw_levellist_ + L.first + off, L.ncls[k], kClsRows[k], d_L_, ln.X, ln.W, nr, ldx);
@@ -875,13 +910,15 @@
         const FwdLevelPlan p = plan_forward_level(L, nr, knobs);
         if (p.ntail > 0) {
             launch_fwd_front(ln.st, ds_, list + p.nf, p.ntail, d_L_, ln.X, ln.X2, ln.W, nr, ldx);
-            if (p.nf == 0) continue;
+            if (p.nf == 0) { if (follows_factor) ip += 2; continue; }
         }
         launch_fwd_assemble(ln.st, ds_, list, p.nf, L.max_cols, ln.X, ln.W, nr, ldx);
+        if (follows_factor) released(kRelProduct, lev);
         for (int j = 0; j < p.nbk; j++) {
             launch_xmul(ln.st, ds_, list, p.xmul_fronts(j), L.max_cols, 0, d_L_, ln.X, ln.X2, nr, ldx, j, inv_cap_);
             if (j + 1 < p.nbk) launch_fwd_own_update(ln.st, ds_, list, p.own_fronts(j), L.max_cols, d_L_, ln.X2, ln.X, nr, ldx, j, inv_cap_);
         }
+        if (follows_factor) released(kRelUpdate, lev);
         if (p.wave) launch_fwd_update_wave(ln.st, ds_, d_fwd_recs_ + L.fwd_off, L.fwd_split, L.fwd_per, d_L_, ln.X2, ln.W, nr, ldx, p.cmin, p.wave_split_k);
         if (p.update == FwdLevelPlan::kRecords)
             launch_fwd_update_recs(ln.st, ds_, d_fwd_recs_ + L.fwd_off, L.fwd_split, L.fwd_per, d_L_, ln.X2, ln.W, nr, ldx, p.cmin);
@@ -919,7 +956,7 @@
         for (int k = 0, off = 0; k < 3; off += nsub_cls_[k], k++)
             launch_subtree(ln.st, ds_, 2, d_sub_first_ + off, d_sub_last_ + off, nsub_cls_[k], kClsRows[k], nullptr, d_L_, nullptr,
                            nullptr, ln.X, nullptr, nr, ldx);
-    if (lo == 0) sweep_tasks(ln, 2, nr, ldx, false);
+    if (lo == 0) sweep_tasks(ln, 2, nr, ldx, false, 0, -1, test_task_ranges_);
     if (env_.level_mark && lo == 0) level_event(ln.st, 2, (int)levels_.size() + 1);
 }
 
@@ -1141,7 +1178,7 @@
         HC(hipEventRecord(ev_qf_, stream2));
     }
     begin_factor(d_nz);
-    factor_levels(0, (int)levels_.size(), false);
+    factor_levels(0, (int)levels_.size(), nullptr);
     enqueue_factor_tail();
     inverse_pending = true;
     enqueue_logdet(stream, false);
@@ -1466,7 +1503,7 @@
         HC(hipEventRecord(ev_qf_, stream2));
     }
     begin_factor(d_nz);
-    factor_levels(0, (int)levels_.size(), false);
+    factor_levels(0, (int)levels_.size(), nullptr);
     enqueue_factor_tail();
     inverse_pending = true;
     enqueue_batch_diag(stream);
diff --git a/gaussianmarkovrandomfields.jl_amd/csrc/device.h b/gaussianmarkovrandomfields.jl_amd/csrc/device.h
--- a/gaussianmarkovrandomfields.jl_amd/csrc/device.h
+++ b/gaussianmarkovrandomfields.jl_amd/csrc/device.h
@@ -150,12 +150,12 @@
 private:
     void upload(const Symbolic &S);
     void ensure_rhs_capacity(long long nrhs);
-    void factor_levels(int lo, int hi, bool record_level_events);
+    void factor_levels(int lo, int hi, const ReleasePlan *plan);
     struct PanelChain;
     bool factor_small_fronts(const LevelInfo &L);
     bool factor_panel_chains(const LevelInfo &L);
     void panel_block(const PanelChain &ch, const LevelInfo &L, int b);
-    void factor_contribution_blocks(const LevelInfo &L, int slot);
+    void factor_contribution_blocks(const LevelInfo &L, int slot, const Event *about_to_start);
     SweepKnobs sweep_knobs() const;
     void forward(const SweepLane &ln, int nr, int ldx, int lo, int hi, bool follows_factor);
     void backward(const SweepLane &ln, int nr, int ldx, bool y_in_x2, int hi, int lo);
@@ -196,8 +196,12 @@
     int *d_levellist2_ = nullptr;
     const int *d_wave_order_ = nullptr;
     int wave_first_[kWaveClasses] = {0, 0}, wave_count_[kWaveClasses] = {0, 0};
-    void sweep_tasks(const SweepLane &ln, int phase, int nr, int ldx, bool follows_factor);
+    void sweep_tasks(const SweepLane &ln, int phase, int nr, int ldx, bool follows_factor, int t0 = 0, int t1 = -1, int ranges = 1);
+    int test_task_ranges_ = 1;
+    bool test_force_windows_ = false;
 public:
+    void set_test_release(int task_ranges, bool force_windows) { test_task_ranges_ = std::max(task_ranges, 1); test_force_windows_ = force_windows; release_plan_nr_ = -1; }
+    const ReleasePlan &release_plan(int nr);
     void set_external_stream(hipStream_t s, bool use, bool async);
     int level_times(int phase, double *out, int cap);
     void dist_front_phase(const double *d_nzval, int front, int what, int block);
@@ -239,7 +243,10 @@
     double *d_pivgrowth_ = nullptr;
     void decide_inverse_cap();
     bool inverse_full_ = false;
-    std::vector<Event> ev_flevel_;
+    std::vector<Event> ev_flevel_, ev_window_;
+    ReleaseBase release_base_;
+    ReleasePlan release_plan_;
+    int release_plan_nr_ = -1, release_plan_cap_ = -1;
     int bottom_top_level_ = 0, fused_gate_level_ = 0;
     int *d_inv_lvl_list_ = nullptr;
     std::vector<int> inv_lvl_first_, inv_lvl_maxc_;
diff --git a/gaussianmarkovrandomfields.jl_amd/csrc/device_plan.cpp b/gaussianmarkovrandomfields.jl_amd/csrc/device_plan.cpp
--- a/gaussianmarkovrandomfields.jl_amd/csrc/device_plan.cpp
+++ b/gaussianmarkovrandomfields.jl_amd/csrc/device_plan.cpp
@@ -476,8 +476,150 @@
 
     P.first_multiblock_level = S.nlevels;
     for (i32 l = 0; l < S.nlevels; l++) if (P.swlevels[l].max_cols > NB) { P.first_multiblock_level = l; break; }
+    {
+        ReleaseBase &R = P.release;
+        R.levels.resize((size_t)S.nlevels);
+        R.gate_level = P.fused_gate_level; R.task_level = P.bottom_top_level; R.ntasks = P.nswt;
+        for (i32 l = 0; l < S.nlevels; l++) {
+            ReleaseBase::Level &V = R.levels[l];
+            const LevelInfo &L = P.levels[l], &W = P.swlevels[l];
+            V.nbig = L.nbig(); V.max_cols = L.nbig() > 0 ? L.max_cols : 0; V.max_trail = L.nbig() > 0 ? L.max_trail : 0;
+            V.has_syrk = L.nbig() > 0 && L.max_trail > 0;
+            for (int k = L.nsmall; k < L.count; k++) {
+                const i32 s = S.levellist[L.first + k];
+                const double c = S.ncols(s), m = S.nrows(s) - S.ncols(s);
+                V.syrk_flops += m * (m + 1) * c;
+            }
+            for (int k = 0; k < W.count; k++) {
+                const i32 s = S.sw_levellist[W.first + k];
+                const double c = S.ncols(s), m = S.nrows(s) - S.ncols(s);
+                V.rows += c + m;
+                if (k < W.nsmall) { V.upd_doubles += (c + m) * c; continue; }
+                V.prod_doubles += 0.5 * c * c; V.upd_doubles += m * c; V.upd_rows += m;
+                if (c > NB) V.inv_flops += c * c * c / 3.0;
+            }
+        }
+        for (int t = 0; t < P.nswt; t++) {
+            if (t % 8 == 0) { R.task_group_doubles.push_back(0); R.task_group_rows.push_back(0); }
+            R.task_group_doubles.back() += (double)(P.swt[t].p1 - P.swt[t].p0);
+            R.task_group_rows.back() += P.swt[t].nt + P.swt[t].mroot;
+        }
+    }
     P.l_size = S.panelptr[ns];
     return P;
 }
 
-}
+double syrk_window_cost_ratio(int max_cols, int nbig) {
+    (void)nbig;
+    if (max_cols < kSyrkWindowMinCols) return kMidLevelCostRatio;
+    if (max_cols < 300) return 0.60;
+    if (max_cols < 500) return 0.47;
+    return kChainCostRatio;
+}
+bool release_window_eligible(const ReleaseLevel &L) {
+    return L.has_syrk && L.nbig > 0 && L.max_cols >= kSyrkWindowMinCols && L.cost_ratio < kChainCostRatio;
+}
+
+std::vector<ReleasePieceIn> release_piece_list(int nlevels, int task_level, bool tasks, const double *level_us) {
+    std::vector<ReleasePieceIn> v;
+    v.push_back({kRelTransposeIn, -1, 0.0});
+    if (tasks) { v.push_back({kRelDtile, task_level, 0.0}); v.push_back({kRelTasks, task_level, 0.0}); }
+    for (int l = 0; l < nlevels; l++)
+        for (int k = 0; k < 4; k++) v.push_back({kRelInverse + k, l, level_us ? level_us[4 * l + k] : 0.0});
+    return v;
+}
+
+ReleaseInput release_input(const ReleaseBase &b, int nr, bool chunk_tasks) {
+    ReleaseInput in;
+    const int nl = (int)b.levels.size();
+    in.levels.resize((size_t)nl);
+    in.gate_level = b.gate_level;
+    std::vector<double> us((size_t)4 * nl, 0.0);
+    for (int l = 0; l < nl; l++) {
+        const ReleaseBase::Level &V = b.levels[l];
+        ReleaseLevel &L = in.levels[l];
+        L.nbig = V.nbig; L.max_cols = V.max_cols; L.max_trail = V.max_trail; L.has_syrk = V.has_syrk;
+        L.window_us = V.syrk_flops / kSyrkFlopsPerUs;
+        L.cost_ratio = syrk_window_cost_ratio(V.max_cols, V.nbig);
+        us[4 * l + 0] = V.inv_flops / kInvFlopsPerUs;
+        us[4 * l + 1] = 2.0 * V.rows * nr / kLevelDoublesPerUs;
+        us[4 * l + 2] = (V.prod_doubles + 2.0 * (V.rows - V.upd_rows) * nr) / kLevelDoublesPerUs;
+        us[4 * l + 3] = (V.upd_doubles + 2.0 * V.upd_rows * nr) / kLevelDoublesPerUs;
+    }
+    in.pieces = release_piece_list(nl, b.task_level, true, us.data());
+    in.ntasks = b.ntasks;
+    if (chunk_tasks && b.ntasks > 0) {
+        for (size_t g = 0; g < b.task_group_doubles.size(); g++)
+            in.task_group_us.push_back((b.task_group_doubles[g] + 2.0 * b.task_group_rows[g] * nr) / kTaskDoublesPerUs);
+    }
+    return in;
+}
+
+ReleasePlan plan_forward_release(const ReleaseInput &in, bool use_windows) {
+    const int nl = (int)in.levels.size();
+    ReleasePlan P;
+    P.record_factored.assign((size_t)std::max(nl, 1), 0);
+    P.record_syrk_start.assign((size_t)std::max(nl, 1), 0);
+    const int gate = std::min(std::max(in.gate_level, 0), std::max(nl - 1, 0));
+    std::vector<int> win;
+    for (int l = 0; use_windows && l < nl; l++)
+        if (release_window_eligible(in.levels[l])) win.push_back(l);
+    const int nw = (int)win.size();
+    const int keep_from = nw > 0 ? win[0] + kReleaseTopLevels : 0;
+    size_t cur = 0;
+    double rem = nw > 0 ? in.levels[win[0]].window_us : 0.0;
+    bool used = false;
+    std::vector<char> win_used((size_t)nw, 0);
+    auto seek = [&](int need, double us) {
+        while (cur < (size_t)nw && (win[cur] <= need || (used && rem < us))) {
+            cur++; used = false;
+            if (cur < (size_t)nw) rem = in.levels[win[cur]].window_us;
+        }
+        return cur < (size_t)nw;
+    };
+    auto take = [&](double us) { rem -= us; used = true; win_used[cur] = 1; };
+    for (const ReleasePieceIn &pc : in.pieces) {
+        const int need = pc.kind == kRelTransposeIn ? -1 : std::min(std::max(pc.level, 0), std::max(nl - 1, 0));
+        ReleasePiece out{pc.kind, pc.level, 0, 0, need < 0 ? kWaitNone : kWaitFactored, need < 0 ? -1 : std::max(need, gate), true};
+        if (pc.kind == kRelTasks) {
+            const int G = (int)in.task_group_us.size();
+            int g = 0;
+            while (g < G) {
+                out.wait = kWaitFactored; out.wait_level = std::max(need, gate);
+                int g1 = G;
+                if (need < keep_from && seek(need, in.task_group_us[g] * std::min(kTaskRangeMinGroups, G - g))) {
+                    double acc = 0;
+                    g1 = g;
+                    while (g1 < G && (g1 - g < kTaskRangeMinGroups || acc + in.task_group_us[g1] <= rem)) acc += in.task_group_us[g1++];
+                    if (G - g1 < kTaskRangeMinGroups) { for (; g1 < G; g1++) acc += in.task_group_us[g1]; }
+                    out.wait = kWaitSyrkStart; out.wait_level = win[cur];
+                    take(acc);
+                }
+                out.t0 = 8 * g; out.t1 = std::min(8 * g1, in.ntasks);
+                P.pieces.push_back(out);
+                P.task_ranges++;
+                g = g1;
+            }
+            if (G == 0) { out.t0 = 0; out.t1 = in.ntasks; P.pieces.push_back(out); P.task_ranges++; }
+            continue;
+        }
+        if (pc.kind != kRelInverse && pc.kind != kRelTransposeIn && need < keep_from && seek(need, pc.us)) {
+            out.wait = kWaitSyrkStart; out.wait_level = win[cur];
+            take(pc.us);
+        }
+        P.pieces.push_back(out);
+    }
+    int fmax = -1, smax = -1;
+    for (ReleasePiece &p : P.pieces) {
+        if (p.wait == kWaitNone) { p.enqueue_wait = false; continue; }
+        const bool implied = p.wait == kWaitFactored ? p.wait_level <= fmax : p.wait_level <= smax;
+        p.enqueue_wait = !implied;
+        if (implied) continue;
+        if (p.wait == kWaitFactored) { fmax = p.wait_level; smax = std::max(smax, p.wait_level); P.record_factored[p.wait_level] = 1; }
+        else { smax = p.wait_level; fmax = std::max(fmax, p.wait_level - 1); P.record_syrk_start[p.wait_level] = 1; }
+    }
+    for (char u : win_used) P.windows_used += u;
+    return P;
+}
+
+}
diff --git a/gaussianmarkovrandomfields.jl_amd/csrc/device_plan.h b/gaussianmarkovrandomfields.jl_amd/csrc/device_plan.h
--- a/gaussianmarkovrandomfields.jl_amd/csrc/device_plan.h
+++ b/gaussianmarkovrandomfields.jl_amd/csrc/device_plan.h
@@ -203,6 +203,58 @@
 Launch choose_bwd_gemm(int nfronts, int max_cols, int blk, int cap);
 Launch choose_bwd_wave(int nfronts, int max_cols, int nr, bool split_k);
 Launch choose_permute(int n, int nr);
+
+constexpr int kSyrkWindowMinCols = 128;
+constexpr double kChainCostRatio = 0.4, kMidLevelCostRatio = 1.0;
+constexpr int kReleaseTopLevels = 2;
+constexpr int kTaskRangeMinGroups = 16;
+enum ReleaseKind { kRelTransposeIn, kRelDtile, kRelTasks, kRelInverse, kRelAssemble, kRelProduct, kRelUpdate };
+enum ReleaseWait { kWaitNone, kWaitFactored, kWaitSyrkStart };
+struct ReleaseLevel {
+    int nbig = 0, max_cols = 0, max_trail = 0;
+    bool has_syrk = false;
+    double window_us = 0;
+    double cost_ratio = 1.0;
+};
+struct ReleasePieceIn { int kind, level; double us; };
+struct ReleaseInput {
+    std::vector<ReleaseLevel> levels;
+    int gate_level = 0;
+    std::vector<ReleasePieceIn> pieces;
+    int ntasks = 0;
+    std::vector<double> task_group_us;
+};
+struct ReleasePiece {
+    int kind, level;
+    int t0, t1;
+    int wait, wait_level;
+    bool enqueue_wait;
+};
+struct ReleasePlan {
+    std::vector<ReleasePiece> pieces;
+    std::vector<char> record_factored, record_syrk_start;
+    int task_ranges = 0, windows_used = 0;
+};
+double syrk_window_cost_ratio(int max_cols, int nbig);
+bool release_window_eligible(const ReleaseLevel &L);
+ReleasePlan plan_forward_release(const ReleaseInput &in, bool use_windows = true);
+std::vector<ReleasePieceIn> release_piece_list(int nlevels, int task_level, bool tasks, const double *level_us );
+
+struct ReleaseBase {
+    struct Level {
+        int nbig = 0, max_cols = 0, max_trail = 0;
+        bool has_syrk = false;
+        double syrk_flops = 0;
+        double inv_flops = 0;
+        double rows = 0, prod_doubles = 0, upd_doubles = 0, upd_rows = 0;
+    };
+    std::vector<Level> levels;
+    int gate_level = 0, task_level = 0, ntasks = 0;
+    std::vector<double> task_group_doubles, task_group_rows;
+};
+constexpr double kSyrkFlopsPerUs = 47e6, kInvFlopsPerUs = 20e6;
+constexpr double kTaskDoublesPerUs = 4.0e5, kLevelDoublesPerUs = 2.5e5;
+ReleaseInput release_input(const ReleaseBase &b, int nr, bool chunk_tasks);
 
 struct PlanOptions {
     bool syrk_xcd = true;
@@ -241,6 +293,7 @@
     double syrk_flops = 0;
     long long sum_trail = 0, l_size = 0, nq = 0;
     int nswt = 0, nswc = 0;
+    ReleaseBase release;
 };
 
 DevicePlan build_device_plan(const Symbolic &S, const PlanOptions &o);
diff --git a/gaussianmarkovrandomfields.jl_amd/csrc/gmrfx_api.cpp b/gaussianmarkovrandomfields.jl_amd/csrc/gmrfx_api.cpp
--- a/gaussianmarkovrandomfields.jl_amd/csrc/gmrfx_api.cpp
+++ b/gaussianmarkovrandomfields.jl_amd/csrc/gmrfx_api.cpp
@@ -295,6 +295,65 @@
     const gmrfx::HostIoPlan p = gmrfx::host_io_plan_dir(n, nrhs, download);
     plan[0] = p.cols_per; plan[1] = p.ppc; plan[2] = p.rows_per; plan[3] = p.slot_doubles; plan[4] = p.nsl; plan[5] = p.reserve;
     return GMRFX_OK;
+}
+static int32_t flatten_release_plan(const gmrfx::ReleasePlan &P, int64_t cap, int32_t *pieces, int64_t *count) {
+    *count = (int64_t)P.pieces.size();
+    if (!pieces) return GMRFX_OK;
+    if (cap < *count) return GMRFX_ERR_INVALID_ARG;
+    for (size_t k = 0; k < P.pieces.size(); k++) {
+        const gmrfx::ReleasePiece &p = P.pieces[k];
+        const int32_t v[7] = {p.kind, p.level, p.t0, p.t1, p.wait, p.wait_level, (int32_t)p.enqueue_wait};
+        std::copy(v, v + 7, pieces + 7 * k);
+    }
+    return GMRFX_OK;
+}
+extern "C" int32_t gmrfx_release_plan_synthetic(int64_t nlevels, const int32_t *level_tab, const double *window_us, const double *cost_ratio,
+                                                const double *level_us, int32_t task_level, int32_t gate_level, int64_t ntasks, double task_us,
+                                                int32_t use_windows, int64_t cap, int32_t *pieces, int64_t *count) {
+    if (nlevels < 0 || nlevels > (1 << 20) || ntasks < 0 || ntasks > (1 << 28) || !count || (nlevels > 0 && (!level_tab || !window_us || !cost_ratio)))
+        return GMRFX_ERR_INVALID_ARG;
+    try {
+        gmrfx::ReleaseInput in;
+        in.levels.resize((size_t)nlevels);
+        for (int64_t l = 0; l < nlevels; l++) {
+            gmrfx::ReleaseLevel &L = in.levels[l];
+            L.nbig = level_tab[4 * l]; L.max_cols = level_tab[4 * l + 1]; L.max_trail = level_tab[4 * l + 2]; L.has_syrk = level_tab[4 * l + 3] != 0;
+            L.window_us = window_us[l]; L.cost_ratio = cost_ratio[l];
+        }
+        in.gate_level = gate_level;
+        in.pieces = gmrfx::release_piece_list((int)nlevels, task_level, true, level_us);
+        in.ntasks = (int)ntasks;
+        in.task_group_us.assign((size_t)((ntasks + 7) / 8), 0.0);
+        for (int64_t t = 0; t < ntasks; t++) in.task_group_us[t / 8] += task_us;
+        return flatten_release_plan(gmrfx::plan_forward_release(in, use_windows != 0), cap, pieces, count);
+    } catch (...) { return GMRFX_ERR_ALLOC; }
+}
+extern "C" int32_t gmrfx_release_plan(gmrfx_handle *h, int64_t nrhs, int32_t all_windows, int64_t cap, int32_t *pieces, int64_t *count, int64_t *summary) {
+    return guarded(h, [&]() -> int32_t {
+        if (!count || nrhs <= 0) throw std::invalid_argument("release_plan: count is null or nrhs <= 0");
+        const gmrfx::EnvKnobs env = gmrfx::read_env_knobs();
+        const gmrfx::DevicePlan P = gmrfx::build_device_plan(h->S, gmrfx::PlanOptions{env.syrk_xcd});
+        const int nr = (int)std::min<int64_t>(nrhs, 64);
+        gmrfx::ReleaseInput in = gmrfx::release_input(P.release, nr, nr > env.wave_max_nr);
+        int64_t shape = 0;
+        for (gmrfx::ReleaseLevel &L : in.levels) {
+            gmrfx::ReleaseLevel probe = L;
+            probe.cost_ratio = 0;
+            if (!gmrfx::release_window_eligible(probe)) continue;
+            shape++;
+            if (all_windows) L.cost_ratio = 0;
+        }
+        const gmrfx::ReleasePlan R = gmrfx::plan_forward_release(in);
+        if (summary) { summary[0] = shape; summary[1] = R.windows_used; summary[2] = R.task_ranges; summary[3] = in.gate_level; summary[4] = (int64_t)in.levels.size(); }
+        return flatten_release_plan(R, cap, pieces, count);
+    });
+}
+extern "C" int32_t gmrfx_debug_release(gmrfx_handle *h, int32_t task_ranges, int32_t force_windows) {
+    return guarded(h, [&]() -> int32_t {
+        if (int32_t e = need_device(h, false)) return e;
+        h->D->set_test_release(task_ranges, force_windows != 0);
+        return GMRFX_OK;
+    });
 }
 extern "C" int32_t gmrfx_set_stream(gmrfx_handle *h, void *hip_stream, int32_t use_external, int32_t async_phases) {
     return guarded(h, [&]() -> int32_t {
diff --git a/gaussianmarkovrandomfields.jl_amd/gmrfx/_lib.py b/gaussianmarkovrandomfields.jl_amd/gmrfx/_lib.py
--- a/gaussianmarkovrandomfields.jl_amd/gmrfx/_lib.py
+++ b/gaussianmarkovrandomfields.jl_amd/gmrfx/_lib.py
@@ -75,6 +75,7 @@
     "gmrfx_batch_constraints_correct", "gmrfx_batch_constraints_correct_dev", "gmrfx_batch_constraints_var", "gmrfx_batch_sample",
     "gmrfx_batch_sample_dev", "gmrfx_batch_constrained_logpdf_dev",
     "gmrfx_rbmc_var", "gmrfx_rbmc_var_dev", "gmrfx_rbmc_plan",
+    "gmrfx_release_plan_synthetic", "gmrfx_release_plan", "gmrfx_debug_release",
 ]
 
 
@@ -195,6 +196,9 @@
         L.gmrfx_rbmc_var.argtypes = [vp, vp, vp, i64, i64, i32, vp]
         L.gmrfx_rbmc_var_dev.argtypes = [vp, vp, vp, i64, i64, i32, vp]
         L.gmrfx_rbmc_plan.argtypes = [vp, i32, i32, vp, vp, vp, vp, vp]
+        L.gmrfx_release_plan_synthetic.argtypes = [i64, vp, vp, vp, vp, i32, i32, i64, dbl, i32, i64, vp, C.POINTER(i64)]
+        L.gmrfx_release_plan.argtypes = [vp, i64, i32, i64, vp, C.POINTER(i64), vp]
+        L.gmrfx_debug_release.argtypes = [vp, i32, i32]
         for nm in EXPORTS[2:]:
             if nm not in ("gmrfx_destroy", "gmrfx_device_ptr"):
                 getattr(L, nm).restype = i32
diff --git a/include/gmrfx.h b/include/gmrfx.h
--- a/include/gmrfx.h
+++ b/include/gmrfx.h
@@ -107,6 +107,11 @@
 int32_t gmrfx_logdet_partial(gmrfx_handle *h, double *out);
 
 int32_t gmrfx_host_io_plan(int64_t n, int64_t nrhs, int32_t download, int64_t *plan );
+int32_t gmrfx_release_plan_synthetic(int64_t nlevels, const int32_t *level_tab , const double *window_us, const double *cost_ratio,
+                                     const double *level_us , int32_t task_level, int32_t gate_level, int64_t ntasks,
+                                     double task_us, int32_t use_windows, int64_t cap, int32_t *pieces, int64_t *count);
+int32_t gmrfx_release_plan(gmrfx_handle *h, int64_t nrhs, int32_t all_windows, int64_t cap, int32_t *pieces, int64_t *count, int64_t *summary );
+int32_t gmrfx_debug_release(gmrfx_handle *h, int32_t task_ranges, int32_t force_windows);
 
 int32_t gmrfx_solve(gmrfx_handle *h, const double *B, int64_t ldb, int64_t nrhs, double *X, int64_t ldx);
 int32_t gmrfx_solve_dev(gmrfx_handle *h, const double *d_B, int64_t ldb, int64_t nrhs, double *d_X, int64_t ldx);
```

Result: no change. 83.16 million DoF/s (median of 4 runs) (+1.0%).
